# zaiisao/ConTEXTure-NeRF

Measured on AMD Instinct MI355X. Metric: UNet denoise steps/sec (CFG-batched SD2-depth UNet eval + PLMS update), higher is better.
Workload: dtype f16; 1 GPU; BASELINE configs[1]: 1 view @768^2 (latent 96^2), 50 PLMS steps (51 UNet evals), SD2-depth UNet fp16, CFG batch 2, guidance 10, random-init weights; mesh substitution napoleon.obj -> n/a for this stage (denoise loop only); latent=96, cfg_batch=2, ctx_len=77, views_per_rank=1, parallelism=view-shard x1

## Files before the change

### contexture-nerf_amd/_lib.py

```python
import ctypes as C
import os
import torch

_HERE = os.path.dirname(os.path.abspath(__file__))
LIB_PATH = os.path.join(_HERE, "libctxnerf.so")

_vp, _i32, _i64, _f32 = C.c_void_p, C.c_int32, C.c_int64, C.c_float

SIGNATURES = {
    "ctx_version": (_i32, []),
    "ctx_last_error": (C.c_char_p, []),
    "ctx_device_check": (_i32, []),
    "ctx_prepare_vertices": (_i32, [_vp, _vp, _vp, _vp, _i32, _i32, _i32, _vp, _vp, _vp, _vp, _vp]),
    "ctx_rasterize_ws_bytes": (_i64, [_i32, _i32, _i32, _i32]),
    "ctx_rasterize_fwd": (_i32, [_i32, _i32, _vp, _vp, _vp, _i32, _i32, _i32, _f32, _f32, _vp, _vp, _vp, _i64, _vp]),
    "ctx_rasterize_fused": (_i32, [_i32, _i32, _vp, _vp, _vp, _i32, _vp, _i32, _i32, _f32, _f32, _vp, _vp, _vp, _vp, _vp, _i64, _vp]),
    "ctx_normalize_depth_ws_bytes": (_i64, [_i32]),
    "ctx_normalize_depth": (_i32, [_vp, _i32, _i32, _vp, _vp, _vp, _vp]),
    "ctx_texture_mapping_fwd": (_i32, [_vp, _vp, _i32, _i32, _i32, _i32, _i32, _i32, _vp, _vp, _vp]),
    "ctx_texture_mapping_bwd": (_i32, [_vp, _vp, _i32, _i32, _i32, _i32, _vp, _vp, _vp]),
    "ctx_texmap_bwd_plan_bytes": (_i64, [_i32, _i32, _i32]),
    "ctx_texmap_bwd_plan": (_i32, [_vp, _vp, _i32, _i32, _i32, _vp, _vp]),
    "ctx_texture_mapping_bwd_binned_ws_bytes": (_i64, [_i32, _i32]),
    "ctx_texture_mapping_bwd_binned": (_i32, [_vp, _vp, _vp, _i32, _i32, _i32, _i32, _vp, _vp, _vp, _vp]),
# ... 59 lines not shown
    "ctx_hashtex_fwd": (_i32, [_vp, _vp, _i64, _i32, _vp, _i32, _i32, _i32, _vp, _vp, _vp]),
    "ctx_hashtex_bwd_ws_bytes": (_i64, [_i32, _i32, _i32]),
    "ctx_hashtex_bwd": (_i32, [_vp, _vp, _i64, _i32, _vp, _i32, _i32, _i32, _vp, _i32, _vp, _vp, _vp]),
    "ctx_texture_head_fwd": (_i32, [_vp, _vp, _i64, _i64, _i32, _vp, _vp]),
    "ctx_texture_head_bwd": (_i32, [_vp, _vp, _vp, _vp, _i64, _i64, _i32, _vp, _vp]),
    "ctx_adam_multi": (_i32, [_vp, _vp, _vp, _vp, _vp, _i32, _f32, _f32, _f32, _f32, _f32, _f32, _f32, _i32, _vp]),
    "ctx_table_adam": (_i32, [_vp, _vp, _vp, _i64, _vp, _i64, _i32, _f32, _f32, _f32, _f32, _f32, _f32, _f32, _i32, _vp]),
    "ctx_weighted_sum_packed": (_i32, [_vp, _vp, _vp, _i64, _i64, _i32, _vp, _vp]),
    "ctx_texel_rays": (_i32, [_vp, _vp, _vp, _vp, _vp, _vp, _i64, _i32, _i32, _i32, _i32, _f32, _vp, _vp, _vp, _vp]),
    "ctx_bake_resolve": (_i32, [_vp, _vp, _vp, _vp, _i64, _i32, _i32, _f32, _i32, _vp, _vp]),
    "ctx_unet_create": (_vp, [_vp]),
    "ctx_unet_destroy": (None, [_vp]),
    "ctx_unet_param_count": (_i32, [_vp]),
    "ctx_unet_param_name": (C.c_char_p, [_vp, _i32]),
    "ctx_unet_param_shape": (_i32, [_vp, _i32, _vp]),
    "ctx_unet_weight_bytes": (_i64, [_vp]),
    "ctx_unet_workspace_bytes": (_i64, [_vp, _i32, _i32, _i32, _i32]),
    "ctx_unet_bind": (_i32, [_vp, _vp, _vp, _i64]),
    "ctx_unet_derived_bytes": (_i64, [_vp]),
    "ctx_unet_bind_derived": (_i32, [_vp, _vp, _i64]),
    "ctx_unet_set_param": (_i32, [_vp, _i32, _vp, _vp]),
    "ctx_unet_forward": (_i32, [_vp, _vp, _vp, _vp, _i32, _i32, _i32, _i32, _vp, _vp]),
    "ctx_controlnet_create": (_vp, [_vp, _i32]),
    "ctx_controlnet_residual_bytes": (_i64, [_vp, _i32, _i32, _i32]),
    "ctx_controlnet_cond_cache_bytes": (_i64, [_vp, _i32, _i32, _i32]),
    "ctx_controlnet_forward": (_i32, [_vp, _vp, _vp, _vp, _vp, _vp, _i32, _i32, _i32, _i32, _i32, _vp, _vp]),
    "ctx_unet_set_residuals": (_i32, [_vp, _vp, C.c_float]),
    "ctx_unet_ref_bank_bytes": (_i64, [_vp, _i32, _i32, _i32]),
    "ctx_unet_workspace_bytes_ref": (_i64, [_vp, _i32, _i32, _i32, _i32, _i32, _i32]),
    "ctx_unet_forward_ref": (_i32, [_vp, _vp, _vp, _vp, _i32, _i32, _i32, _i32, _i32, _vp, _i32, _vp, _vp]),
    "ctx_unet_set_residual_fp32": (_i32, [_vp, _i32]),
    "ctx_unet_stats": (_i32, [_vp, _i32, _vp, _vp]),
    "ctx_unet_gn_epilogue_counts": (_i32, [_vp, _vp, _vp]),
    "ctx_unet_set_taps": (_i32, [_vp, _vp, _i64]),
    "ctx_unet_tap_count": (_i32, [_vp]),
    "ctx_unet_tap_info": (_i32, [_vp, _i32, _vp, _vp, _vp]),
    "ctx_vae_create": (_vp, [_vp]),
    "ctx_vae_destroy": (None, [_vp]),
    "ctx_vae_param_count": (_i32, [_vp]),
    "ctx_vae_param_name": (C.c_char_p, [_vp, _i32]),
    "ctx_vae_param_shape": (_i32, [_vp, _i32, _vp]),
    "ctx_vae_weight_bytes": (_i64, [_vp]),
    "ctx_vae_workspace_bytes": (_i64, [_vp, _i32, _i32, _i32]),
    "ctx_vae_bind": (_i32, [_vp, _vp, _vp, _i64]),
    "ctx_vae_derived_bytes": (_i64, [_vp]),
    "ctx_vae_bind_derived": (_i32, [_vp, _vp, _i64]),
    "ctx_vae_set_param": (_i32, [_vp, _i32, _vp, _vp]),
    "ctx_vae_decode": (_i32, [_vp, _vp, _i32, _i32, _i32, _vp, _vp]),
    "ctx_vae_decoder_param_count": (_i32, [_vp]),
    "ctx_vae_encode_workspace_bytes": (_i64, [_vp, _i32, _i32, _i32]),
    "ctx_vae_encode": (_i32, [_vp, _vp, _i32, _i32, _i32, _vp, _vp]),
    "ctx_vae_flops": (C.c_double, [_vp]),
    "ctx_vae_encode_train_workspace_bytes": (_i64, [_vp, _i32, _i32, _i32]),
    "ctx_vae_encode_train": (_i32, [_vp, _vp, _i32, _i32, _i32, _vp, _vp]),
    "ctx_vae_encode_bwd": (_i32, [_vp, _vp, _f32, _vp, _vp]),
    "ctx_gemm_f16": (_i32, [_vp, _vp, _vp, _vp, _i32, _i32, _i32, _vp, _vp]),
    "ctx_conv3x3_f16": (_i32, [_vp, _vp, _vp, _vp, _vp, _i32, _i32, _i32, _i32, _i32, _i32, _i32, _vp, _vp]),
    "ctx_conv3x3_seg_f16": (_i32, [_vp, _vp, _vp, _vp, _vp, _vp, _i32, _i32, _i32, _i32, _i32, _vp, _vp, _i32, _i32, _vp, _vp, _i32, _i32,
                                   _vp, _i32, _vp, _vp]),
    "ctx_conv3x3_gn_f16": (_i32, [_vp, _vp, _vp, _vp, _vp, _vp, _i32, _i32, _i32, _i32, _i32, _vp, _i32, _i32, _i32, _vp, _vp, _vp, _vp]),
    "ctx_gemm_last_kernel": (None, [_vp, _vp]),
    "ctx_conv3x3_geom_f16": (_i32, [_vp, _vp, _vp, _vp, _i32, _i32, _i32, _i32, _i32, _i32, _i32, _i32, _i32, _vp, _i32, _vp, _vp]),
    "ctx_pack_conv3_dgrad_f16": (_i32, [_vp, _i32, _i32, _i32, _vp, _vp]),
    "ctx_pack_conv3_phase_f16": (_i32, [_vp, _i32, _i32, _vp, _vp]),
    "ctx_conv3x3_phase_f16": (_i32, [_vp, _vp, _vp, _vp, _vp, _i32, _i32, _i32, _i32, _i32, _vp, _i32, _vp, _vp]),
    "ctx_pack_mat_dgrad_f16": (_i32, [_vp, _i32, _i32, _i32, _i32, _vp, _vp]),
    "ctx_groupnorm_bwd_ws_bytes": (_i64, [_i32, _i32]),
    "ctx_groupnorm_bwd_f16": (_i32, [_vp, _vp, _vp, _vp, _vp, _i32, _i32, _i32, _i32, _f32, _i32, _vp, _vp, _vp]),
    "ctx_softmax_rows_f16": (_i32, [_vp, _i32, _i32, _f32, _vp, _vp]),
    "ctx_softmax_bwd_rows_f16": (_i32, [_vp, _vp, _i32, _i32, _f32, _vp, _vp]),
    "ctx_quant_bwd_f16": (_i32, [_vp, _vp, _i32, _i32, _i64, _f32, _vp, _vp]),
    "ctx_conv_in_bwd_f16": (_i32, [_vp, _vp, _i32, _i32, _i32, _i32, _i32, _f32, _vp, _vp]),
    "ctx_conv_in_f16": (_i32, [_vp, _vp, _vp, _i32, _i32, _i32, _i32, _i32, _vp, _vp]),
    "ctx_conv_out_f16": (_i32, [_vp, _vp, _vp, _i32, _i32, _i32, _i32, _i32, _vp, _vp]),
    "ctx_gemv_f16": (_i32, [_vp, _vp, _vp, _i32, _i32, _i32, _i32, _i32, _vp, _vp]),
    "ctx_time_embed_f16": (_i32, [_vp, _i32, _i32, _vp, _vp]),
    "ctx_transpose_v_f16": (_i32, [_vp, _i32, _i32, _i32, _i32, _i32, _vp, _vp]),
    "ctx_concat_f16": (_i32, [_vp, _vp, _i64, _i32, _i32, _vp, _vp]),
    "ctx_concat_f32": (_i32, [_vp, _vp, _i64, _i32, _i32, _vp, _vp]),
    "ctx_f32_to_f16": (_i32, [_vp, _i64, _vp, _vp]),
    "ctx_f16_to_f32": (_i32, [_vp, _i64, _vp, _vp]),
    "ctx_conv_small_f16": (_i32, [_vp, _vp, _vp, _vp, _i32, _i32, _i32, _i32, _i32, _i32, _i32, _vp, _vp]),
    "ctx_add_scaled_f16": (_i32, [_vp, _vp, _f32, _i64, _vp]),
    "ctx_pointwise_f32": (_i32, [_vp, _vp, _vp, _i32, _i32, _i64, _i32, _vp, _vp]),
    "ctx_pack_fwd_f16": (_i32, [_vp, _i32, _i32, _i32, _vp, _vp]),
    "ctx_groupnorm_f16": (_i32, [_vp, _vp, _vp, _i32, _i32, _i32, _i32, _f32, _i32, _vp, _vp, _vp]),
    "ctx_groupnorm2_f16": (_i32, [_vp, _vp, _i32, _vp, _vp, _i32, _i32, _i32, _i32, _f32, _i32, _vp, _vp, _vp]),
    "ctx_groupnorm_apply_f16": (_i32, [_vp, _vp, _i32, _vp, _vp, _i32, _i32, _i32, _i32, _f32, _i32, _vp, _vp]),
    "ctx_groupnorm_slabs_f16": (_i32, [_vp, _i32, _vp, _vp, _vp, _i32, _vp, _vp, _i32, _i32, _i32, _i32, _f32, _i32, _vp, _vp]),
    "ctx_layernorm_f16": (_i32, [_vp, _vp, _vp, _i64, _i32, _f32, _vp, _vp]),
    "ctx_attention_ws_bytes": (_i64, [_i32, _i32, _i32]),
    "ctx_attention_f16": (_i32, [_vp, _vp, _vp, _i32, _i32, _i32, _i32, _i32, _i32, _f32, _vp, _i32, _vp, _vp]),
    "ctx_groupnorm_ws_bytes": (_i64, [_i32, _i32]),
    "ctx_geglu_f16": (_i32, [_vp, _i64, _i32, _vp, _vp]),
    "ctx_profile_begin": (_i32, []),
    "ctx_profile_end": (_i32, [_i32, _vp, _vp]),
    "ctx_bench_gemm": (C.c_float, [_vp, _vp, _vp, _vp, _i32, _i32, _i32, _vp, _i32, _i32, _i32, _i32, _i32, _i32, _vp, _i32, _i32, _vp]),
    "ctx_gemm_tune": (None, [_i32, _i32]),
    "ctx_attention_tune": (None, [_i32, _i32, _i32, _f32]),
    "ctx_probe_mfma": (_i32, [_i32, _vp, _vp, _vp, _vp]),
    "ctx_probe_stage": (C.c_float, [_i32, _i32, _i32, _i32, _i32, _vp, _vp, _vp]),
    "ctx_cfg_plms_step": (_i32, [_vp, _i64, _f32, _vp, _i32, _vp, _f32, _f32, _i32, _vp, _vp, _vp]),
}


class CtxError(RuntimeError):
    pass


# ... 48 lines not shown
```

### contexture-nerf_amd/csrc/attention.hip

```cpp
#include "gemm_common.h"
#include <math.h>

#define AT_KB 64
#define AT_KROW 72
#define AT_VROW 68


struct AttnArgs {
    const f16 *Q, *K, *V;
    f16 *O;
    int Sq, Skv, heads;
    int q_stride, kv_stride, o_stride;
    float scale_log2e;
    float lazy;
};



typedef short at_s16x4 __attribute__((__vector_size__(4 * sizeof(short))));
__device__ __forceinline__ f16x4 at_tr16(const f16 *p)
{
    at_s16x4 v = __builtin_amdgcn_ds_read_tr16_b64_v4i16((__attribute__((address_space(3))) at_s16x4 *)p);
    return __builtin_bit_cast(f16x4, v);
}
struct AtNoIssue { __device__ __forceinline__ void operator()(int) const {} };
template <bool MASK, int NISSUE = 0, class Issue = AtNoIssue>
__device__ __forceinline__ void attn_tile(const f16 *__restrict__ Ks, const f16 *__restrict__ Vs, int k0, int Skv, int r, int h,
                                          int swz, int vlane, int vfq, float c, const f16x8 (&qf)[4], f32x16 (&o)[2], f32x16 &ls,
                                          float &m_run, float lazy, Issue iss = Issue())
{
    f32x16 s[2];
#pragma unroll
    for (int kb = 0; kb < 2; ++kb) {
#pragma unroll
        for (int q = 0; q < 16; ++q) s[kb][q] = 0.f;
        const f16 *kr = Ks + (kb * 32 + r) * 64;
#pragma unroll
        for (int ks = 0; ks < 4; ++ks) {
            f16x8 kf = *(const f16x8 *)(kr + ((2 * ks + h) ^ swz) * 8);
            s[kb] = __builtin_amdgcn_mfma_f32_32x32x16_f16(kf, qf[ks], s[kb], 0, 0, 0);
            if (kb * 4 + ks < NISSUE) iss(kb * 4 + ks);
        }
    }
    if (MASK) {
#pragma unroll
        for (int kb = 0; kb < 2; ++kb)
#pragma unroll
// ... 29 lines not shown
#pragma unroll
        for (int d = 0; d < 2; ++d)
#pragma unroll
            for (int q = 0; q < 16; ++q) asm volatile("v_mul_f32 %0, %0, %1" : "+v"(o[d][q]) : "v"(alpha));
    }
    m_run = m_new;
    const f16x8 ones = {1, 1, 1, 1, 1, 1, 1, 1};
#pragma unroll
    for (int kb = 0; kb < 2; ++kb)
#pragma unroll
        for (int st = 0; st < 2; ++st) {
            f16x8 pf;
#pragma unroll
            for (int j = 0; j < 8; ++j) pf[j] = (f16)s[kb][8 * st + j];
            const f16 *vk = Vs + (32 * kb + 16 * st + 4 * h) * 64 + vlane;
#pragma unroll
            for (int d = 0; d < 2; ++d) {
                const int co = ((4 * d) ^ vfq) * 8;
                f16x4 v0 = at_tr16(vk + co), v1 = at_tr16(vk + 8 * 64 + co);
                f16x8 vf = __builtin_shufflevector(v0, v1, 0, 1, 2, 3, 4, 5, 6, 7);
                o[d] = __builtin_amdgcn_mfma_f32_32x32x16_f16(vf, pf, o[d], 0, 0, 0);
            }
            ls = __builtin_amdgcn_mfma_f32_32x32x16_f16(ones, pf, ls, 0, 0, 0);
        }
}

template <int AT_NS, int NW, bool SPREAD = true>
__global__ __launch_bounds__(64 * NW, NW == 8 ? 4 : 1) void k_attention_dma(AttnArgs a)
{
    __shared__ __attribute__((aligned(16))) f16 ring[AT_NS * 2 * 64 * 64];
    const int tid = threadIdx.x, lane = tid & 63, wave = __builtin_amdgcn_readfirstlane(tid >> 6);
    const int r = lane & 31, h = lane >> 5;
    const int b = blockIdx.z, hd = blockIdx.y;
    const int q0 = blockIdx.x * (32 * NW) + wave * 32;
    const int qrow = q0 + r;
    const bool qok = qrow < a.Sq;
    constexpr int PI = 8 / NW;
    constexpr int G = 2 * PI;

    f16x8 qf[4];
    const f16x8 zero8 = {0, 0, 0, 0, 0, 0, 0, 0};
    {
        const f16 *qp = a.Q + ((size_t)b * a.Sq + (qok ? qrow : 0)) * a.q_stride + hd * 64 + 8 * h;
#pragma unroll
        for (int ks = 0; ks < 4; ++ks) qf[ks] = qok ? *(const f16x8 *)(qp + ks * 16) : zero8;
    }
    f32x16 o[2];
#pragma unroll
    for (int d = 0; d < 2; ++d)
#pragma unroll
        for (int q = 0; q < 16; ++q) o[d][q] = 0.f;
    f32x16 ls;
#pragma unroll
    for (int q = 0; q < 16; ++q) ls[q] = 0.f;
    float m_run = -INFINITY;

    const int ntiles = (a.Skv + AT_KB - 1) / AT_KB;
    const int lr = lane >> 3, pc = lane & 7;
    const f16 *kp[PI], *vp[PI];
    int krow[PI];
#pragma unroll
    for (int i = 0; i < PI; ++i) {
        int row = 8 * (wave + NW * i) + lr;
        int lc = (pc ^ ((row >> 1) & 7)) * 8;
        krow[i] = row;
        kp[i] = a.K + ((size_t)b * a.Skv + row) * a.kv_stride + hd * 64 + lc;
// ... 53 lines not shown
            attn_tile<false>(Ks, Ks + 64 * 64, t * AT_KB, a.Skv, r, h, swz, vlane, vfq, c, qf, o, ls, m_run, a.lazy);
        }
        slot = slot + 1 == AT_NS ? 0 : slot + 1;
    }
    for (; t < nfull; ++t) {
        const int newer = issued - 1 - t;
        if (AT_NS >= 4 && newer >= 2) asm volatile("s_waitcnt vmcnt(%0)" ::"n"(2 * G) : "memory");
        else if (newer >= 1) asm volatile("s_waitcnt vmcnt(%0)" ::"n"(G) : "memory");
        else asm volatile("s_waitcnt vmcnt(0)" ::: "memory");
        __builtin_amdgcn_sched_barrier(0);
        ctx_barrier();
        if (issued < ntiles) issue(slot == 0 ? AT_NS - 1 : slot - 1);
        const f16 *Ks = ring + slot * (2 * 64 * 64);
        attn_tile<false>(Ks, Ks + 64 * 64, t * AT_KB, a.Skv, r, h, swz, vlane, vfq, c, qf, o, ls, m_run, a.lazy);
        slot = slot + 1 == AT_NS ? 0 : slot + 1;
    }
    if (nfull < ntiles) {
        asm volatile("s_waitcnt vmcnt(0)" ::: "memory");
        ctx_barrier();
        const f16 *Ks = ring + slot * (2 * 64 * 64);
        attn_tile<true>(Ks, Ks + 64 * 64, nfull * AT_KB, a.Skv, r, h, swz, vlane, vfq, c, qf, o, ls, m_run, a.lazy);
    }
    if (qok) {
        float inv = 1.0f / ls[0];
        f16 *op = a.O + ((size_t)b * a.Sq + qrow) * a.o_stride + hd * 64;
#pragma unroll
        for (int d = 0; d < 2; ++d)
#pragma unroll
            for (int g = 0; g < 4; ++g) {
                f16x4 v;
#pragma unroll
                for (int j = 0; j < 4; ++j) v[j] = (f16)(o[d][4 * g + j] * inv);
                *(f16x4 *)(op + d * 32 + 8 * g + 4 * h) = v;
            }
    }
}

template <int NS, int NW, bool SPREAD = true>
static void attn_launch(const AttnArgs &a, int B, bool report, hipStream_t s)
{
    constexpr auto kern = k_attention_dma<NS, NW, SPREAD>;
    if (report) {
        int nb = 0;
        hipFuncAttributes fa;
        (void)hipOccupancyMaxActiveBlocksPerMultiprocessor(&nb, kern, 64 * NW, 0);
        (void)hipFuncGetAttributes(&fa, (const void *)kern);
        fprintf(stderr, "[ctx] attention: %d blocks/CU by the occupancy API, %d VGPRs, %zu B static LDS\n", nb, fa.numRegs, fa.sharedSizeBytes);
    }
    ctx_launch<kern>(1, dim3(cdiv(a.Sq, 32 * NW), a.heads, B), dim3(64 * NW), 0, s, a);
}

struct AttnTune { int ns, nw8, spread; float lazy; };
static AttnTune g_attn_force = {-1, -1, -1, -1.f};
static const AttnTune &attn_tune_env()
{
    static const AttnTune env = [] {
        AttnTune t;
        t.ns = ctx_env_int("CTX_ATTN_NS", 3);
        t.nw8 = ctx_env_int("CTX_ATTN_NW8", -1);
        t.spread = ctx_env_int("CTX_ATTN_SPREAD", 1);
        const char *e = getenv("CTX_ATTN_LAZY");
        t.lazy = e ? (float)atof(e) : 8.0f;
        if (!(t.lazy >= 0.f && t.lazy <= 12.f)) t.lazy = 8.0f;
        return t;
    }();
    return env;
}

extern "C" void ctx_attention_tune(int32_t ns, int32_t nw8, int32_t spread, float lazy)
{
    g_attn_force.ns = ns; g_attn_force.nw8 = nw8; g_attn_force.spread = spread; g_attn_force.lazy = lazy;
}

int ctx_attention_core(const f16 *Q, const f16 *K, const f16 *V, int B, int Sq, int Skv, int heads, int q_stride,
                       int kv_stride, float scale, f16 *O, int o_stride, hipStream_t s)
{
    AttnArgs a;
    a.Q = Q; a.K = K; a.V = V; a.O = O; a.Sq = Sq; a.Skv = Skv; a.heads = heads;
    a.q_stride = q_stride; a.kv_stride = kv_stride; a.o_stride = o_stride;
    a.scale_log2e = scale * 1.4426950408889634f;
    const AttnTune &tu = attn_tune_env();
    const float lazy = g_attn_force.lazy >= 0.f ? g_attn_force.lazy : tu.lazy;
    a.lazy = lazy >= 0.f && lazy <= 12.f ? lazy : 8.0f;
    const int ns = g_attn_force.ns >= 0 ? g_attn_force.ns : tu.ns;
    const int nw8 = g_attn_force.nw8 >= 0 ? g_attn_force.nw8 : tu.nw8;
    const bool w8 = nw8 == 1 || (nw8 < 0 && Sq >= 1024 && Sq < 4096 && Skv >= 1024);
    const int spread = g_attn_force.spread >= 0 ? g_attn_force.spread : tu.spread;
    static int dbg = -1;
    bool report = false;
    if (dbg < 0) { dbg = ctx_env_int("CTX_ATTN_DEBUG", 0); report = dbg != 0; }
    if (w8) {
        if (ns == 2) attn_launch<2, 8>(a, B, report, s); else if (ns == 4) attn_launch<4, 8>(a, B, report, s);
        else if (spread) attn_launch<3, 8>(a, B, report, s); else attn_launch<3, 8, false>(a, B, report, s);
    } else {
        if (ns == 2) attn_launch<2, 4>(a, B, report, s); else if (ns == 4) attn_launch<4, 4>(a, B, report, s);
        else if (spread) attn_launch<3, 4>(a, B, report, s); else attn_launch<3, 4, false>(a, B, report, s);
    }
    hipError_t e = hipGetLastError();
    if (e != hipSuccess) {
        ctx_set_error("attention launch failed: %s", hipGetErrorString(e));
        return CTX_E_LAUNCH;
    }
    return CTX_OK;
}

extern "C" int64_t ctx_attention_ws_bytes(int32_t B, int32_t Skv, int32_t heads)
{
    (void)B; (void)Skv; (void)heads;
    return 256;
}
// ... 14 lines not shown
```

### contexture-nerf_amd/csrc/common.h

```cpp
#pragma once
#include <hip/hip_runtime.h>
#include <stdint.h>
#include <stdio.h>
#include <stdlib.h>
#include <stdarg.h>
#include "../../include/ctx_nerf.h"

void ctx_set_error(const char *fmt, ...);

#define CTX_REQUIRE(cond, ...)                 \
    do {                                       \
        if (!(cond)) {                         \
            ctx_set_error(__VA_ARGS__);        \
            return CTX_E_ARG;                  \
        }                                      \
    } while (0)

#define CTX_CHECK_LAUNCH(name)                                                     \
    do {                                                                           \
        hipError_t e__ = hipGetLastError();                                        \
        if (e__ != hipSuccess) {                                                   \
            ctx_set_error("%s: launch failed: %s", name, hipGetErrorString(e__)); \
            return CTX_E_LAUNCH;                                                   \
        }                                                                          \
// ... 1 lines not shown

static inline int64_t cdiv64(int64_t a, int64_t b) { return (a + b - 1) / b; }
static inline int cdiv(int a, int b) { return (a + b - 1) / b; }
static inline unsigned capped_blocks(int64_t items, int per_block, int64_t cap)
{
    const int64_t nb = cdiv64(items, per_block);
    return (unsigned)(nb < cap ? nb : cap);
}
static inline int ctx_env_int(const char *name, int dflt)
{
    const char *e = getenv(name);
    return e ? atoi(e) : dflt;
}
#define CTX_BOOL_GO(flag, B_, ...)                                 \
    do {                                                           \
        if (flag) { constexpr bool B_ = true; __VA_ARGS__; }       \
        else { constexpr bool B_ = false; __VA_ARGS__; }           \
    } while (0)

typedef _Float16 f16;
typedef f16 f16x8 __attribute__((ext_vector_type(8)));
typedef f16 f16x4 __attribute__((ext_vector_type(4)));
typedef f16 f16x2 __attribute__((ext_vector_type(2)));
typedef float f32x16 __attribute__((ext_vector_type(16)));
typedef float f32x4 __attribute__((ext_vector_type(4)));

__device__ __forceinline__ void ctx_barrier()
{
    asm volatile("" ::: "memory");
    __builtin_amdgcn_s_barrier();
    asm volatile("" ::: "memory");
}

__device__ __forceinline__ float wave_sum(float v)
{
#pragma unroll
    for (int o = 32; o > 0; o >>= 1) v += __shfl_xor(v, o, 64);
    return v;
}
__device__ __forceinline__ float sum8_dpp(float v)
{
    v += __builtin_bit_cast(float, __builtin_amdgcn_update_dpp(0, __builtin_bit_cast(int, v), 0xB1, 0xf, 0xf, true));
    v += __builtin_bit_cast(float, __builtin_amdgcn_update_dpp(0, __builtin_bit_cast(int, v), 0x4E, 0xf, 0xf, true));
    v += __builtin_bit_cast(float, __builtin_amdgcn_update_dpp(0, __builtin_bit_cast(int, v), 0x141, 0xf, 0xf, true));
    return v;
}
__device__ __forceinline__ float wave_sum_dpp(float v)
{
    v = sum8_dpp(v);
    v += __builtin_bit_cast(float, __builtin_amdgcn_update_dpp(0, __builtin_bit_cast(int, v), 0x140, 0xf, 0xf, true));
    const int vi = __builtin_bit_cast(int, v);
    float r0 = __builtin_bit_cast(float, __builtin_amdgcn_readlane(vi, 0)), r1 = __builtin_bit_cast(float, __builtin_amdgcn_readlane(vi, 16));
    float r2 = __builtin_bit_cast(float, __builtin_amdgcn_readlane(vi, 32)), r3 = __builtin_bit_cast(float, __builtin_amdgcn_readlane(vi, 48));
    return (r0 + r1) + (r2 + r3);
}
__device__ __forceinline__ float wave_max(float v)
{
#pragma unroll
    for (int o = 32; o > 0; o >>= 1) v = fmaxf(v, __shfl_xor(v, o, 64));
    return v;
}
__device__ __forceinline__ float wave_min(float v)
{
#pragma unroll
    for (int o = 32; o > 0; o >>= 1) v = fminf(v, __shfl_xor(v, o, 64));
    return v;
// ... 2 lines not shown
```

### contexture-nerf_amd/csrc/elementwise.hip

```cpp
#include "common.h"
#include "kernels.h"
#include <math.h>

__global__ __launch_bounds__(256) void k_geglu(const f16 *__restrict__ h, int64_t M, int C4, f16 *__restrict__ y)
{
    const int c8n = C4 / 8;
    const int64_t total = M * c8n;
    for (int64_t i = (int64_t)blockIdx.x * 256 + threadIdx.x; i < total; i += (int64_t)gridDim.x * 256) {
        int64_t m = i / c8n;
        int c8 = (int)(i % c8n);
        f16x8 a = *(const f16x8 *)(h + m * 2 * C4 + c8 * 8);
        f16x8 g = *(const f16x8 *)(h + m * 2 * C4 + C4 + c8 * 8);
        f16x8 o;
#pragma unroll
        for (int j = 0; j < 8; ++j) {
            float gf = (float)g[j];
            o[j] = (f16)((float)a[j] * (0.5f * gf * (1.0f + erff(gf * 0.70710678118654752f))));
        }
        *(f16x8 *)(y + m * C4 + c8 * 8) = o;
    }
}

extern "C" int32_t ctx_geglu_f16(const void *h, int64_t M, int32_t C4, void *y, ctx_stream_t stream)
{
// ... 57 lines not shown
                "transpose_v: need Sp %% 8 == 0, Sp >= S, ld %% 8 == 0, ld >= 64 heads (B=%d S=%d ld=%d heads=%d Sp=%d)", B, S, ld, heads, Sp);
    hipLaunchKernelGGL(k_transpose_v, dim3(cdiv(Sp, 64), heads, B), dim3(256), 0, s, v, S, ld, heads, Sp, vt);
    CTX_CHECK_LAUNCH("transpose_v");
    return CTX_OK;
}

__global__ __launch_bounds__(256) void k_f32_to_f16(const float *__restrict__ x, int64_t n, f16 *__restrict__ y)
{
    for (int64_t i = (int64_t)blockIdx.x * 256 + threadIdx.x; i < n; i += (int64_t)gridDim.x * 256) y[i] = (f16)x[i];
}
__global__ __launch_bounds__(256) void k_f16_to_f32(const f16 *__restrict__ x, int64_t n8, float *__restrict__ y)
{
    for (int64_t i = (int64_t)blockIdx.x * 256 + threadIdx.x; i < n8; i += (int64_t)gridDim.x * 256) {
        const f16x8 v = *(const f16x8 *)(x + i * 8);
        f32x4 a = {(float)v[0], (float)v[1], (float)v[2], (float)v[3]}, b = {(float)v[4], (float)v[5], (float)v[6], (float)v[7]};
        *(f32x4 *)(y + i * 8) = a; *(f32x4 *)(y + i * 8 + 4) = b;
    }
}
int ctx_f16_to_f32_core(const f16 *x, int64_t n, float *y, hipStream_t s)
{
    CTX_REQUIRE(x && y && n > 0 && n % 8 == 0, "f16_to_f32: n=%lld is not a positive multiple of 8", (long long)n);
    hipLaunchKernelGGL(k_f16_to_f32, dim3(capped_blocks(n / 8, 256, 4096)), dim3(256), 0, s, x, n / 8, y);
    CTX_CHECK_LAUNCH("f16_to_f32");
    return CTX_OK;
}
int ctx_f32_to_f16_core(const float *x, int64_t n, f16 *y, hipStream_t s)
{
    CTX_REQUIRE(x && y && n > 0, "f32_to_f16: null pointer or n=%lld < 1", (long long)n);
    hipLaunchKernelGGL(k_f32_to_f16, dim3(capped_blocks(n, 256, 2048)), dim3(256), 0, s, x, n, y);
    CTX_CHECK_LAUNCH("f32_to_f16");
    return CTX_OK;
}

__global__ void k_time_embed(const float *__restrict__ t, int B, int dim, f16 *__restrict__ out)
{
    int i = blockIdx.x * blockDim.x + threadIdx.x;
    int half = dim / 2;
    if (i >= half) return;
    float fr = expf(-9.210340371976184f * (float)i / (float)half);
    float a = t[0] * fr;
    float c = cosf(a), sn = sinf(a);
    for (int b = 0; b < B; ++b) {
        out[(size_t)b * dim + i] = (f16)c;
        out[(size_t)b * dim + half + i] = (f16)sn;
    }
}
int ctx_time_embed_core(const float *t, int B, int dim, f16 *out, hipStream_t s)
{
    CTX_REQUIRE(t && out && B > 0 && dim >= 2 && dim % 2 == 0, "time_embed: unsupported B=%d dim=%d", B, dim);
    hipLaunchKernelGGL(k_time_embed, dim3(cdiv(dim / 2, 64)), dim3(64), 0, s, t, B, dim, out);
    CTX_CHECK_LAUNCH("time_embed");
    return CTX_OK;
}

#define CI_SPLIT 16
template <int CP, int CX>
__global__ __launch_bounds__(256) void k_conv_in(const float *__restrict__ x, const f16 *__restrict__ w,
                                                 const f16 *__restrict__ bias, int B, int Cin, int H, int W, int Cout,
                                                 f16 *__restrict__ y)
{
    extern __shared__ __attribute__((aligned(16))) float s_w[];
    constexpr int WR = 9 * CP, WX = 9 * CX;
    const int o8n = Cout / 8;
    const int o8_per = (o8n + CI_SPLIT - 1) / CI_SPLIT;
    const int o8_0 = blockIdx.y * o8_per, o8_1 = min(o8n, o8_0 + o8_per);
    const int no = (o8_1 - o8_0) * 8;
    for (int i = threadIdx.x; i < no * WX; i += 256) {
        const int o = i / WX, r = i - o * WX, t = r / CX, c = r - t * CX;
        s_w[i] = (float)w[(size_t)(o8_0 * 8 + o) * WR + t * CP + c];
    }
    __syncthreads();
    const int64_t npix = (int64_t)B * H * W;
    const int64_t pix0 = (int64_t)blockIdx.x * 256;
    const int64_t pix = pix0 + threadIdx.x;
    const bool live = pix < npix;
    const int64_t pq = live ? pix : npix - 1;
    int b = (int)(pq / (H * W)), p = (int)(pq % (H * W));
    int oy = p / W, ox = p % W;
    float in[9][CX];
#pragma unroll
    for (int t = 0; t < 9; ++t) {
        int iy = oy + t / 3 - 1, ix = ox + t % 3 - 1;
        bool ok = iy >= 0 && iy < H && ix >= 0 && ix < W;
#pragma unroll
        for (int c = 0; c < CX; ++c)
            in[t][c] = (ok && c < Cin) ? (float)(f16)x[(((size_t)b * Cin + c) * H + iy) * W + ix] : 0.f;
    }
    f16 *patch = (f16 *)(s_w + no * WX);
    for (int g0 = o8_0; g0 < o8_1; g0 += 8) {
        const int ng = min(8, o8_1 - g0);
        for (int gi = 0; gi < ng; ++gi) {
            const int o8 = g0 + gi;
            f16x8 o;
#pragma unroll
            for (int j = 0; j < 8; ++j) {
                const float *wr = s_w + ((o8 - o8_0) * 8 + j) * WX;
                float acc = (float)bias[o8 * 8 + j];
#pragma unroll
                for (int t = 0; t < 9; ++t)
#pragma unroll
                    for (int c = 0; c < CX; ++c) acc += in[t][c] * wr[t * CX + c];
                o[j] = (f16)acc;
            }
            *(f16x8 *)(patch + threadIdx.x * 72 + gi * 8) = o;
        }
        __syncthreads();
        for (int ch = threadIdx.x; ch < 256 * ng; ch += 256) {
            const int px = ch / ng, gi = ch - px * ng;
            if (pix0 + px < npix) *(f16x8 *)(y + (pix0 + px) * Cout + (g0 + gi) * 8) = *(const f16x8 *)(patch + px * 72 + gi * 8);
        }
        __syncthreads();
    }
}
int ctx_conv_in_core(const float *x, const f16 *w, const f16 *bias, int B, int Cin, int H, int W, int Cout, f16 *y, hipStream_t s)
{
    CTX_REQUIRE(x && w && bias && y && Cout > 0 && Cout % 8 == 0, "conv_in: unsupported Cout=%d", Cout);
    CTX_REQUIRE(Cin >= 1 && Cin <= 16, "conv_in: need 1 <= Cin <= 16 (Cin=%d)", Cin);
    CTX_REQUIRE(B > 0 && H > 0 && W > 0 && (int64_t)H * W < (1ll << 31), "conv_in: unsupported grid B=%d H=%d W=%d", B, H, W);
    int64_t npix = (int64_t)B * H * W;
    int o8_per = (Cout / 8 + CI_SPLIT - 1) / CI_SPLIT;
    const int cx = Cin <= 3 ? 3 : Cin <= 5 ? Cin : Cin <= 8 ? 8 : Cin == 9 ? 9 : 16;
    CTX_REQUIRE((size_t)o8_per * 8 * 9 * cx * sizeof(float) + 256 * 72 * sizeof(f16) <= 64 * 1024,
                "conv_in: the weight slice of Cout=%d at Cin=%d does not fit the LDS", Cout, Cin);
    const dim3 grid((unsigned)cdiv64(npix, 256), CI_SPLIT);
#define CI_GO(CP_, CX_) hipLaunchKernelGGL((k_conv_in<CP_, CX_>), grid, dim3(256), (size_t)o8_per * 8 * 9 * CX_ * sizeof(float) + 256 * 72 * sizeof(f16), s, x, w, bias, B, Cin, H, W, Cout, y)
    if (Cin <= 3) CI_GO(8, 3);
    else if (Cin == 4) CI_GO(8, 4);
    else if (Cin == 5) CI_GO(8, 5);
    else if (Cin <= 8) CI_GO(8, 8);
    else if (Cin == 9) CI_GO(16, 9);
    else CI_GO(16, 16);
#undef CI_GO
    CTX_CHECK_LAUNCH("conv_in");
    return CTX_OK;
}

template <int NU, bool WF32>
__global__ __launch_bounds__(256) void k_conv_out(const f16 *__restrict__ x, const f16 *__restrict__ w,
                                                  const f16 *__restrict__ bias, int B, int H, int W, int C, int Cout,
                                                  float *__restrict__ out)
{
    extern __shared__ __attribute__((aligned(16))) char s_cw_raw[];
    f16 *s_cw = (f16 *)s_cw_raw;
    float *s_cf = (float *)s_cw_raw;
    const int nwt = Cout * 9 * C;
    if (WF32) {
        for (int i = threadIdx.x * 8; i < nwt; i += 256 * 8) {
            const f16x8 v = *(const f16x8 *)(w + i);
#pragma unroll
            for (int j = 0; j < 8; ++j) s_cf[i + j] = (float)v[j];
        }
    } else {
        for (int i = threadIdx.x * 8; i < nwt; i += 256 * 8) *(f16x8 *)(s_cw + i) = *(const f16x8 *)(w + i);
    }
    __syncthreads();
    const int lane = threadIdx.x & 63;
    const int c8n = C / 8, nitems = 9 * c8n;
    const int64_t npix = (int64_t)B * H * W;
// ... 112 lines not shown
                                     const float *coef4, float sample_coeff, float eps_coeff, int32_t mode,
                                     float *cur_sample_ws, float *x, ctx_stream_t stream)
{
    CTX_REQUIRE(eps_pair && ets && coef4 && x && n > 0 && head >= 0 && head < 4, "cfg_plms_step: bad args");
    CTX_REQUIRE(mode == 0 || cur_sample_ws, "cfg_plms_step: mode %d needs cur_sample_ws", mode);
    hipLaunchKernelGGL(k_cfg_plms, dim3(capped_blocks(n, 256, 2048)), dim3(256), 0, (hipStream_t)stream, eps_pair, n, guidance, ets, head,
                       coef4[0], coef4[1], coef4[2], coef4[3], sample_coeff, eps_coeff, mode, cur_sample_ws, x);
    CTX_CHECK_LAUNCH("cfg_plms_step");
    return CTX_OK;
}

extern "C" int32_t ctx_concat_f16(const void *a, const void *b, int64_t M, int32_t Ca, int32_t Cb, void *y, ctx_stream_t stream)
{
    return ctx_concat_core((const f16 *)a, (const f16 *)b, M, Ca, Cb, (f16 *)y, (hipStream_t)stream);
}
extern "C" int32_t ctx_concat_f32(const float *a, const float *b, int64_t M, int32_t Ca, int32_t Cb, float *y, ctx_stream_t stream)
{
    CTX_REQUIRE(Ca > 0 && Cb > 0 && Ca <= (1 << 29) && Cb <= (1 << 29), "concat_f32: unsupported Ca=%d Cb=%d", Ca, Cb);
    return ctx_concat32_core(a, b, M, Ca, Cb, y, (hipStream_t)stream);
}
extern "C" int32_t ctx_transpose_v_f16(const void *v, int32_t B, int32_t S, int32_t ld, int32_t heads, int32_t Sp, void *vt, ctx_stream_t stream)
{
    CTX_REQUIRE(B <= 65535 && heads <= 65535, "transpose_v: B=%d / heads=%d exceed the grid", B, heads);
    return ctx_transpose_v_core((const f16 *)v, B, S, ld, heads, Sp, (f16 *)vt, (hipStream_t)stream);
}
extern "C" int32_t ctx_f32_to_f16(const float *x, int64_t n, void *y, ctx_stream_t stream)
{
    return ctx_f32_to_f16_core(x, n, (f16 *)y, (hipStream_t)stream);
}
extern "C" int32_t ctx_f16_to_f32(const void *x, int64_t n, float *y, ctx_stream_t stream)
{
    return ctx_f16_to_f32_core((const f16 *)x, n, y, (hipStream_t)stream);
}
extern "C" int32_t ctx_time_embed_f16(const float *t, int32_t B, int32_t dim, void *out, ctx_stream_t stream)
{
    return ctx_time_embed_core(t, B, dim, (f16 *)out, (hipStream_t)stream);
}
extern "C" int32_t ctx_conv_in_f16(const float *x, const void *w_pack, const void *bias, int32_t B, int32_t Cin, int32_t H, int32_t W, int32_t Cout,
                                   void *y, ctx_stream_t stream)
{
    return ctx_conv_in_core(x, (const f16 *)w_pack, (const f16 *)bias, B, Cin, H, W, Cout, (f16 *)y, (hipStream_t)stream);
}
extern "C" int32_t ctx_conv_out_f16(const void *x, const void *w, const void *bias, int32_t B, int32_t H, int32_t W, int32_t C, int32_t Cout,
                                    float *out, ctx_stream_t stream)
{
    return ctx_conv_out_core((const f16 *)x, (const f16 *)w, (const f16 *)bias, B, H, W, C, Cout, out, (hipStream_t)stream);
}
```

### contexture-nerf_amd/csrc/engine.h

```cpp
#pragma once
#include "common.h"
#include "kernels.h"
#include <string>
#include <vector>

enum PackKind { PK_COPY = 0, PK_CONV3 = 1, PK_CONVIN = 2, PK_GEGLU_W = 3, PK_GEGLU_B = 4 };

struct Param {
    std::string name;
    int ndim;
    int64_t shape[4];
    int kind;
    size_t dst;
    int a, b;
    int kind2 = 0; size_t dst2 = 0; int pad2 = 0, ld2 = 0, col2 = 0;
    int kind3 = 0; size_t dst3 = 0;
};

struct Engine {
    const char *tag = "";
    std::vector<Param> params;
    size_t wtop = 0;
    size_t dtop = 0;
    f16 *D = nullptr;
    f16 *W = nullptr;
    char *ws = nullptr;
    size_t ws_cap = 0;
    size_t top = 0, peak = 0;
    bool dry = false;
    hipStream_t s = nullptr;
    int rc = 0;
    int64_t launches[3] = {0, 0, 0};
    double flops[3] = {0, 0, 0};

    struct GnTag { const void *x = nullptr; int B = 0, HW = 0, C = 0, groups = 0, NS = 0; } gn_tag;
    int64_t gn_from_producer = 0, gn_from_slabs = 0;

    size_t walloc(size_t n) { size_t o = wtop; wtop += (n + 127) / 128 * 128; return o; }
    size_t add(const std::string &name, std::vector<int64_t> shp, int kind, size_t dst, int a = 0, int b = 0)
    {
        Param p; p.name = name; p.ndim = (int)shp.size(); p.kind = kind; p.dst = dst; p.a = a; p.b = b;
        for (int i = 0; i < 4; ++i) p.shape[i] = i < p.ndim ? shp[i] : 1;
        params.push_back(p);
        return dst;
    }
    void derive_phase()
    {
        Param &p = params.back();
        if (!ctx_conv3_phase_ok(p.b, p.a, 1, 1, 0, 0)) return;
        p.kind3 = 1; p.dst3 = dtop; dtop += ((size_t)16 * p.a * p.b + 127) / 128 * 128;
    }
    const f16 *phase_pack(const f16 *Wt) const
    {
        if (!D || !W) return nullptr;
        for (const Param &p : params)
            if (p.kind3 == 1 && W + p.dst == Wt) return D + p.dst3;
        return nullptr;
    }
    size_t vec(const std::string &name, int n) { return add(name, {n}, PK_COPY, walloc(n)); }
    size_t lin(const std::string &name, int out, int in) { return add(name, {out, in}, PK_COPY, walloc((size_t)out * in)); }

    void *alloc(size_t bytes)
    {
        size_t o = (top + 255) / 256 * 256;
        top = o + bytes;
        if (top > peak) peak = top;
        if (!dry && top > ws_cap) { rc = CTX_E_STATE; ctx_set_error("%s: workspace too small (%zu > %zu)", tag, top, ws_cap); return ws; }
        return dry ? nullptr : (void *)(ws + o);
    }
    f16 *allocH(size_t n) { return (f16 *)alloc(n * 2); }

    void begin()
    {
        top = 0; peak = 0; rc = 0; gn_tag = GnTag(); gn_from_producer = 0; gn_from_slabs = 0;
        for (int k = 0; k < 3; ++k) { launches[k] = 0; flops[k] = 0; }
    }
    void note(int klass, double fl, int n = 1) { launches[klass] += n; flops[klass] += fl; }
    bool live() const { return !dry && rc == 0; }
    void copy(void *dst, const void *src, size_t bytes) { if (live()) (void)hipMemcpyAsync(dst, src, bytes, hipMemcpyDeviceToDevice, s); }
    void copy2d(void *dst, size_t dpitch, const void *src, size_t spitch, size_t width, size_t rows)
    { if (live()) (void)hipMemcpy2DAsync(dst, dpitch, src, spitch, width, rows, hipMemcpyDeviceToDevice, s); }
};

#define ENGINE_RUN(e, expr) do { if ((e)->live()) { int r__ = (expr); if (r__ != 0) (e)->rc = r__; } } while (0)
#define ENGINE_LAUNCH(e, kernel, grid, block, lds, ...) do { if ((e)->live()) hipLaunchKernelGGL(kernel, grid, block, lds, (e)->s, __VA_ARGS__); } while (0)

struct GnReq { float *part = nullptr; int groups = 0, HW = 0; };
void engine_linear(Engine &e, const f16 *X, const f16 *Wt, const f16 *bias, const void *res, int M, int N, int K, void *out, int ldc = 0,
                   int epi = 0, bool res32 = false, bool out32 = false, const GnReq *gn = nullptr);
struct ConvGeom { int stride = 1, ups = 0, poff = 0, zins = 0; };
struct ConvSegs { int n = 0; const f16 *x[2] = {nullptr, nullptr}; const f16 *w[2] = {nullptr, nullptr}; int C[2] = {0, 0}, ldw[2] = {0, 0}; const f16 *bias2 = nullptr; };
void engine_conv3(Engine &e, const f16 *x, const f16 *Wt, const f16 *bias, const void *res, int B, int H, int W, int Cin, int Cout, void *out,
                  ConvGeom g = ConvGeom(), const f16 *rowbias = nullptr, int ldrb = 0, bool res32 = false, bool out32 = false,
                  const ConvSegs *segs = nullptr, const GnReq *gn = nullptr, GnSlabs *slabs = nullptr);
int engine_conv3_split(int B, int H, int W, int Cin, int Cout);

template <class F> int engine_dry_run(Engine *e, F run)
{
    const bool was = e->dry;
    e->dry = true; const int rc = run(); e->dry = was;
    return rc;
}
inline int64_t engine_workspace_need(const Engine *e) { return (int64_t)e->peak + 4096; }
int engine_finish(Engine *e, const char *who);

int32_t engine_param_count(const Engine *e);
const char *engine_param_name(const Engine *e, int32_t i);
// ... 8 lines not shown
```

### contexture-nerf_amd/csrc/engine.hip

```cpp
#include "engine.h"

int32_t engine_param_count(const Engine *e) { return e ? (int32_t)e->params.size() : 0; }
const char *engine_param_name(const Engine *e, int32_t i)
{
    return (e && i >= 0 && i < (int)e->params.size()) ? e->params[i].name.c_str() : "";
}
int32_t engine_param_shape(const Engine *e, int32_t i, int64_t shape4[4])
{
    if (!e || i < 0 || i >= (int)e->params.size()) return 0;
    for (int k = 0; k < 4; ++k) shape4[k] = e->params[i].shape[k];
    return e->params[i].ndim;
}
int64_t engine_weight_bytes(const Engine *e) { return e ? (int64_t)e->wtop * 2 + 256 : 0; }

int32_t engine_bind(Engine *e, void *weights, void *workspace, int64_t workspace_bytes, const char *who)
{
    CTX_REQUIRE(e && weights && workspace && workspace_bytes > 0, "%s: bad args", who);
    CTX_REQUIRE(((uintptr_t)weights & 255) == 0 && ((uintptr_t)workspace & 255) == 0, "%s: blobs must be 256-byte aligned", who);
    e->W = (f16 *)weights; e->ws = (char *)workspace; e->ws_cap = (size_t)workspace_bytes;
    return CTX_OK;
}

int64_t engine_derived_bytes(const Engine *e) { return e && e->dtop ? (int64_t)e->dtop * 2 + 256 : 0; }
int32_t engine_bind_derived(Engine *e, void *derived, int64_t bytes, const char *who)
{
    CTX_REQUIRE(e, "%s: bad args", who);
    if (!derived) { e->D = nullptr; return CTX_OK; }
    CTX_REQUIRE(e->dtop > 0, "%s: this engine derives nothing", who);
    CTX_REQUIRE(bytes >= engine_derived_bytes(e) && ((uintptr_t)derived & 255) == 0, "%s: the derived blob needs %lld bytes, 256-byte aligned", who,
                (long long)engine_derived_bytes(e));
    e->D = (f16 *)derived;
    return CTX_OK;
}

static void engine_gemm(Engine &e, GemmArgs &a, bool conv, const ConvSegs *segs = nullptr, const GnReq *gn = nullptr, GnSlabs *slabs = nullptr,
                        const f16 *phase = nullptr)
{
    e.note(0, 2.0 * a.M * a.N * a.K);
    size_t mark = e.top;
    if (phase) ctx_conv3_phase(a, phase);
    ctx_gemm_plan(a, conv);
    if (segs && segs->n) {
        int kseg = 0;
        a.nseg = segs->n; a.bias2 = segs->bias2;
        for (int i = 0; i < segs->n; ++i) {
            a.segX[i] = segs->x[i]; a.segW[i] = segs->w[i]; a.segC[i] = segs->C[i]; a.segLdw[i] = segs->ldw[i];
            kseg += segs->C[i];
        }
        a.K += kseg;
        e.note(0, 2.0 * a.M * a.N * kseg);
    }
    if (a.zins) a.use8 = 0;
    if (a.splitk > 1) a.part = (float *)e.alloc((size_t)a.splitk * a.M * a.N * 4);
    if (gn && gn->part && gn->groups > 0 && a.N % gn->groups == 0) { a.gn_part = gn->part; a.gn_cg = a.N / gn->groups; a.gn_hw = gn->HW; }
    if (slabs) {
        a.keep_slabs = 1;
        *slabs = GnSlabs{a.part, a.splitk, (size_t)a.M * a.N, a.bias, a.bias2, a.rowbias, a.ldrb};
    }
    ENGINE_RUN(&e, ctx_gemm_dispatch(a, conv, e.s));
    if (e.live() && a.gn_part) e.gn_tag = Engine::GnTag{a.out, a.M / a.gn_hw, a.gn_hw, a.N, gn->groups, a.gn_ns};
    if (!slabs) e.top = mark;
}

int engine_conv3_split(int B, int H, int W, int Cin, int Cout)
{
    GemmArgs a = {};
    a.Ho = H; a.Wo = W; a.M = B * H * W; a.N = Cout; a.K = 9 * Cin; a.H = H; a.W = W; a.Cin = Cin; a.stride = 1;
    ctx_gemm_plan(a, true);
    return (a.splitk > 1 && a.splitk <= a.K / 64) ? a.splitk : 1;
}

void engine_linear(Engine &e, const f16 *X, const f16 *Wt, const f16 *bias, const void *res, int M, int N, int K, void *out, int ldc, int epi,
                   bool res32, bool out32, const GnReq *gn)
{
    GemmArgs a = {};
    a.X = X; a.Wt = Wt; a.bias = bias; a.residual = (const f16 *)res; a.out = (f16 *)out;
    a.M = M; a.N = N; a.K = K; a.ldc = ldc ? ldc : epi == 1 ? N / 2 : N; a.ldr = N; a.rows_per_batch = 1; a.ldrb = N; a.epi = epi;
    a.res32 = res32; a.out32 = out32;
    engine_gemm(e, a, false, nullptr, gn);
}

void engine_conv3(Engine &e, const f16 *x, const f16 *Wt, const f16 *bias, const void *res, int B, int H, int W, int Cin, int Cout, void *out,
                  ConvGeom g, const f16 *rowbias, int ldrb, bool res32, bool out32, const ConvSegs *segs, const GnReq *gn, GnSlabs *slabs)
{
    GemmArgs a = {};
    ctx_conv3_problem(a, B, H, W, Cin, Cout, g.stride, g.ups, g.poff, g.zins);
    a.X = x; a.Wt = Wt; a.bias = bias; a.rowbias = rowbias; a.residual = (const f16 *)res; a.out = (f16 *)out;
    a.ldrb = ldrb;
    a.res32 = res32; a.out32 = out32;
    const f16 *phase = nullptr;
    if (g.ups && ctx_conv3_phase_ok(Cin, Cout, g.stride, g.ups, g.poff, g.zins) && !res && !rowbias && !segs && !gn && !slabs && !res32 && !out32 &&
        !ctx_conv3_phase_loses(a.M, Cout, Cin))
// ... 157 lines not shown
```

### contexture-nerf_amd/csrc/gemm.hip

```cpp
#include "gemm_common.h"

template <int MI, int NI, bool PH = false>
__device__ __forceinline__ void gemm_epilogue(const GemmArgs &a, f32x16 (&acc)[MI][NI], int mw, int nw, int r, int h, const ConvPhase &ph)
{
#pragma unroll
    for (int mi = 0; mi < MI; ++mi) {
        int m = mw + mi * 32 + r;
        if (m >= ph.M) continue;
        const int mo = PH ? conv_phase_row(a, ph, m) : m;
        int bidx = a.rowbias ? m / a.rows_per_batch : 0;
        if (a.epi == 1) {
            if constexpr (NI == 2) {
                int fbase = nw / 2;
#pragma unroll
                for (int g = 0; g < 4; ++g) {
                    int nn = nw + 8 * g + 4 * h;
                    if (nn >= a.N) continue;
                    f16x4 o;
#pragma unroll
                    for (int j = 0; j < 4; ++j) {
                        float xv = acc[mi][0][4 * g + j], gv = acc[mi][1][4 * g + j];
                        if (a.bias) { xv += (float)a.bias[nn + j]; gv += (float)a.bias[nn + 32 + j]; }
                        o[j] = geglu(xv, gv);
                    }
// ... 33 lines not shown
            for (int g = 0; g < 4; ++g)
                *(f32x4 *)(stage + r * RS + ni * 32 + 8 * g + 4 * h) = acc4(acc[mi][ni], g);
#pragma unroll
        for (int p = 0; p < 32 / RPP; ++p) {
            const int row = RPP * p + prow;
            const int m = mw + mi * 32 + row;
            f32x4 v0 = *(const f32x4 *)(stage + row * RS + c8), v1 = *(const f32x4 *)(stage + row * RS + c8 + 4);
            if (m < ph.M && n < a.N) {
                float v[8] = {v0[0], v0[1], v0[2], v0[3], v1[0], v1[1], v1[2], v1[3]};
                add8(v, bs);
                if (a.bias2) add8(v, *(const f16x8 *)(a.bias2 + n));
                store8<true>(a, v, PH ? conv_phase_row(a, ph, m) : m, n);
            }
        }
    }
}

template <int WM, int WN, int MI, int NI, bool CONV, int NS, int PKT, bool PH = false>
__global__ __launch_bounds__(64 * WM * WN) void k_gemm_pipe(GemmArgs a)
{
    constexpr int BM = 32 * MI * WM, BN = 32 * NI * WN, NW = WM * WN;
    constexpr int RP = 512 / PKT;
    constexpr int LPR = PKT / 8;
    constexpr int XI = BM / (RP * NW), WI = BN / (RP * NW);
    static_assert(XI >= 1 && WI >= 1, "tile too small for the wave count");
    constexpr int G = XI + WI;
    constexpr int STAGE = (BM + BN) * PKT;
    extern __shared__ __attribute__((aligned(16))) f16 smem[];

    const int tid = threadIdx.x, lane = tid & 63, wave = __builtin_amdgcn_readfirstlane(tid >> 6);
    const int r = lane & 31, h = lane >> 5;
    const int wm = wave / WN, wn = wave % WN;
    const GemmTile t = gemm_tile(a, blockIdx.x, PKT, BM, BN);
    static_assert(!PH || CONV, "the phase form is a convolution");
    const ConvPhase ph = PH ? conv_phase_tile(a, t.tile_m, BM) : ConvPhase{0, 0, 0, t.m0, a.M};
    const int slice = t.slice, tile_m = t.tile_m, tile_n = t.tile_n, m0 = ph.m0, n0 = t.n0, kbeg = t.kbeg, nk = t.nk;
    const int ldw = CONV ? (PH ? 4 : 9) * a.Cin : a.K;
    const f16 *const Wt = PH ? a.Wt + (size_t)ph.ph * a.N * ldw : a.Wt;
    const int lr = lane / LPR, pc = lane % LPR;

    const f16 *xp[XI], *wp[WI];
    int xst[XI], wst[WI];
    int xoff[XI], xoy[XI], xox[XI];
    bool xok[XI];
#pragma unroll
    for (int i = 0; i < XI; ++i) {
        int row = RP * (wave + NW * i) + lr;
        int m = m0 + row;
        const int lc = (pc ^ (PKT == 32 ? ((row >> 2) & 3) : ((row >> 1) & 7))) * 8;
        xok[i] = m < ph.M;
        if (CONV) {
            conv_pixel(a, m, lc, xoy[i], xox[i], xoff[i]);
            xp[i] = ctx_zero_page; xst[i] = 0;
        } else {
            xoff[i] = 0; xoy[i] = 0; xox[i] = 0;
            xp[i] = xok[i] ? a.X + (size_t)m * a.K + kbeg * PKT + lc : ctx_zero_page;
            xst[i] = xok[i] ? PKT : 0;
        }
    }
#pragma unroll
    for (int i = 0; i < WI; ++i) {
        int row = RP * (wave + NW * i) + lr;
        bool ok = (n0 + row) < a.N;
        wp[i] = ok ? Wt + (size_t)(n0 + row) * ldw + kbeg * PKT + ((pc ^ (PKT == 32 ? ((row >> 2) & 3) : ((row >> 1) & 7))) * 8) : ctx_zero_page;
        wst[i] = ok ? PKT : 0;
    }
// ... 703 lines not shown
```

### contexture-nerf_amd/csrc/gemm144.hip

```cpp
#include "gemm_common.h"
#include <type_traits>

#define G144_BM 144
#define G144_BN 160
#define G144_STAGE ((G144_BM + G144_BN) * 64)

template <int WM, int WN, bool CONV, int NS, int VAR, int UPS = 0, int BMB = 9, bool GNP = false>
__global__ __launch_bounds__(64 * WM * WN) void k_gemm144(GemmArgs a)
{
    constexpr int NW = WM * WN, MI = BMB / WM, NI = 10 / WN;
    constexpr int BM = 16 * BMB, NPX = BM / 8;
    constexpr int NP = NPX + 20;
    constexpr int STAGE = (BM + G144_BN) * 64;
    static_assert(NPX % 2 == 0, "the K segments' chunk swizzle takes a weight piece's parity from its slot");
    static_assert(BMB % WM == 0 && (BMB == 9 || (BMB == 18 && VAR == 0)), "288-row tiles: lockstep schedule only");
    constexpr int SL = (NP + NW - 1) / NW;
    static_assert(9 % WM == 0 && 10 % WN == 0, "wave grid must divide 9 x 10 blocks");
    extern __shared__ __attribute__((aligned(16))) f16 smem[];
    const int tid = threadIdx.x, lane = tid & 63, wave = __builtin_amdgcn_readfirstlane(tid >> 6);
    const int wm = wave / WN, wn = wave % WN;
    const int r16 = lane & 15, kg = lane >> 4;

    const GemmTile tl = gemm_tile(a, blockIdx.x, 64, BM, G144_BN);
    constexpr bool PH = UPS == 2;
    static_assert(!PH || (CONV && !GNP), "the phase form is a convolution without GroupNorm partials");
    const ConvPhase ph = PH ? conv_phase_tile(a, tl.tile_m, BM) : ConvPhase{0, 0, 0, tl.m0, a.M};
    const int slice = tl.slice, m0 = ph.m0, n0 = tl.n0, kbeg = tl.kbeg, nk = tl.nk;
    const int ldw = CONV ? (PH ? 4 : 9) * a.Cin : a.K;
    const f16 *const Wt = PH ? a.Wt + (size_t)ph.ph * a.N * ldw : a.Wt;

    const int prow = lane >> 3, pc = lane & 7;
    constexpr bool FAST = CONV && UPS != 1;
    constexpr int NTAP = PH ? 4 : 9;
    const f16 *pp[SL], *xcen[SL];
    int pst[SL], xoff[SL], xoy[SL], xox[SL], xlc[SL], xval[SL];
    bool xok[SL];
    const f16 *const zp = ctx_zero_page;
    const bool full = wave + NW * (SL - 1) < NP;
#pragma unroll
    for (int i = 0; i < SL; ++i) {
        const int p = wave + NW * i;
        const bool isx = p < NPX, live = p < NP;
        const int s = isx ? 8 * p + prow : 8 * (p - NPX) + prow;
        xlc[i] = (pc ^ ((s >> 1) & 7)) * 8;
        xoff[i] = 0; xoy[i] = 0; xox[i] = 0;
        if (isx) {
            const int m = m0 + s;
            xok[i] = m < ph.M;
            if (CONV) {
                conv_pixel(a, xok[i] ? m : 0, xlc[i], xoy[i], xox[i], xoff[i]);
                pp[i] = zp; pst[i] = 0;
                if (FAST) {
                    xcen[i] = a.X + (size_t)xoff[i] + (size_t)(xoy[i] * a.W + xox[i]) * a.Cin;
                    int v = 0;
#pragma unroll
                    for (int t = 0; t < NTAP; ++t) {
                        const int iy = xoy[i] + (PH ? conv_phase_dy(ph, t) : t / 3 - 1 + a.poff), ix = xox[i] + (PH ? conv_phase_dx(ph, t) : t % 3 - 1 + a.poff);
// ... 458 lines not shown
```

### contexture-nerf_amd/csrc/kernels.h

```cpp
#pragma once
#include "common.h"

struct GemmArgs {
    const f16 *X;
    const f16 *Wt;
    const f16 *bias;
    const f16 *rowbias;
    const f16 *residual;
    f16 *out;
    int M, N, K;
    int ldc, ldr;
    int rows_per_batch;
    int ldrb;
    int epi;
    int H, W, Cin, Ho, Wo, stride, ups;
    int poff;
    int res32, out32;
    int zins;
    int phase;
    int ntm, ntn;
    int splitk;
    float *part;
    int pk;
    int krot;
    int tile, use8;
    int stage_epi;
    int mfast;
    int nseg;
    const f16 *segX[2];
    const f16 *segW[2];
    int segC[2], segLdw[2];
    const f16 *bias2;
    float *gn_part;
    int gn_cg, gn_hw;
    int gn_ns;
    int keep_slabs;
};
#define CTX_GN_MAX_SLOTS 128
#define CTX_GEMM_MAX_SEG 2

static inline void ctx_conv3_problem(GemmArgs &a, int B, int H, int W, int Cin, int Cout, int stride, int ups, int poff, int zins)
{
    a.Ho = ((H << ups) - 1) / stride + 1; a.Wo = ((W << ups) - 1) / stride + 1;
    a.M = B * a.Ho * a.Wo; a.N = Cout; a.K = 9 * Cin; a.ldc = Cout; a.ldr = Cout; a.rows_per_batch = a.Ho * a.Wo;
    a.H = H; a.W = W; a.Cin = Cin; a.stride = stride; a.ups = ups; a.poff = poff; a.zins = zins;
}

static inline void ctx_conv3_phase(GemmArgs &a, const f16 *wp)
{
    a.phase = 1; a.Wt = wp; a.K = 4 * a.Cin;
}
static inline int ctx_conv3_phase_ok(int Cin, int Cout, int stride, int ups, int poff, int zins)
{
    return ups == 1 && stride == 1 && poff == 0 && !zins && Cin % 64 == 0 && Cout % 8 == 0;
}
static inline int ctx_conv3_phase_loses(int M, int Cout, int Cin) { return 0; }

int ctx_gemm_dispatch(GemmArgs &a, bool conv, hipStream_t s);
int ctx_gemm8_try(GemmArgs &a, bool conv, bool force, hipStream_t s);
int ctx_conv_halo_try(GemmArgs &a, int ni, hipStream_t s);
int ctx_gemm144_try(GemmArgs &a, bool conv, int form, hipStream_t s);
int ctx_gemm_pick_split(int M, int N, int K, int epi);
void ctx_gemm_plan(GemmArgs &a, bool conv);
int ctx_gemv_core(const f16 *x, const f16 *w, const f16 *bias, int Bm, int N, int K, int silu_in, int silu_out, f16 *out, hipStream_t s);
int ctx_concat_core(const f16 *a, const f16 *b, int64_t M, int Ca, int Cb, f16 *y, hipStream_t s);
int ctx_transpose_v_core(const f16 *v, int B, int S, int ld, int heads, int Sp, f16 *vt, hipStream_t s);
int ctx_f32_to_f16_core(const float *x, int64_t n, f16 *y, hipStream_t s);
int ctx_time_embed_core(const float *t, int B, int dim, f16 *out, hipStream_t s);
int ctx_conv_in_core(const float *x, const f16 *w, const f16 *bias, int B, int Cin, int H, int W, int Cout, f16 *y, hipStream_t s);
int ctx_conv_out_core(const f16 *x, const f16 *w, const f16 *bias, int B, int H, int W, int C, int Cout, float *out, hipStream_t s);
int ctx_attention_core(const f16 *Q, const f16 *K, const f16 *V, int B, int Sq, int Skv, int heads, int q_stride,
                       int kv_stride, float scale, f16 *O, int o_stride, hipStream_t s);
extern "C" int64_t ctx_groupnorm_ws_bytes(int32_t B, int32_t groups);
int ctx_groupnorm_any(const void *x, int x32, const void *gamma, const void *beta, int B, int HW, int C, int groups, float eps, int silu,
                      void *y, void *stats_ws, hipStream_t stream, const void *x2 = nullptr, int Ca = 0);
int ctx_groupnorm_two_pass(int HW, int C, int groups);
int ctx_groupnorm_apply(const void *x, const float *part, int NS, const void *gamma, const void *beta, int B, int HW, int C, int groups, float eps,
                        int silu, void *y, hipStream_t stream);
struct GnSlabs { const float *part; int S; size_t MN; const f16 *bias, *bias2, *rowbias; int ldrb; };
int ctx_groupnorm_slabs(const GnSlabs &sl, const void *gamma, const void *beta, int B, int HW, int C, int groups, float eps, int silu, void *y,
                        hipStream_t stream);
int ctx_layernorm_any(const void *x, int x32, const void *gamma, const void *beta, int64_t rows, int C, float eps, void *y, hipStream_t stream);
int ctx_concat32_core(const float *a, const float *b, int64_t M, int Ca, int Cb, float *y, hipStream_t s);
int ctx_f16_to_f32_core(const f16 *x, int64_t n, float *y, hipStream_t s);
int ctx_conv_small_core(const float *x32, const f16 *x16, const f16 *w, const f16 *bias, int B, int H, int W, int Cin, int Cout, int stride, int silu,
                        f16 *y, hipStream_t s);
int ctx_add_scaled_core(f16 *dst, const f16 *src, float scale, int64_t n, hipStream_t s);
int ctx_pointwise_core(const void *x, const f16 *w, const f16 *b, int B, int C, int64_t HW, bool nhwc16, float *y, hipStream_t s);

bool ctx_prof_on(void);
void ctx_prof_events(int klass, hipEvent_t *a, hipEvent_t *b);
```

### contexture-nerf_amd/csrc/norm.hip

```cpp
#include "common.h"
#include "kernels.h"
#include <math.h>


struct Wide8 {
    float v[8];
    __device__ __forceinline__ float get(int j) const { return v[j]; }
};
template <bool X32> struct Raw8;
template <> struct Raw8<false> {
    f16x8 a;
    __device__ __forceinline__ float get(int j) const { return (float)a[j]; }
    __device__ __forceinline__ Wide8 widen() const
    {
        Wide8 r;
#pragma unroll
        for (int j = 0; j < 8; ++j) r.v[j] = (float)a[j];
        return r;
    }
};
template <> struct Raw8<true> {
    f32x4 a, b;
    __device__ __forceinline__ float get(int j) const { return j < 4 ? a[j] : b[j - 4]; }
    __device__ __forceinline__ Wide8 widen() const
    {
        Wide8 r;
#pragma unroll
        for (int j = 0; j < 4; ++j) { r.v[j] = a[j]; r.v[4 + j] = b[j]; }
        return r;
    }
};
template <bool X32>
__device__ __forceinline__ Raw8<X32> ldraw(const void *base, size_t elem)
{
    Raw8<X32> r;
    if constexpr (X32) { r.a = *(const f32x4 *)((const float *)base + elem); r.b = *(const f32x4 *)((const float *)base + elem + 4); }
    else r.a = *(const f16x8 *)((const f16 *)base + elem);
    return r;
}

struct GnSrc { const void *p; int cs, col; };
__device__ __forceinline__ GnSrc gn_src(const void *x, const void *x2, int Ca, int C, int ch)
{
    if (!x2) return {x, C, ch};
    return ch < Ca ? GnSrc{x, Ca, ch} : GnSrc{x2, C - Ca, ch - Ca};
}

#define GN_MAX_GROUPS 64
#define GN_MAX_SPLITS CTX_GN_MAX_SLOTS
#define GN_MAX_C 4096
#define GN_U 4
#define GN_AU 6
#define GN_FOLD 8

template <bool X32>
__global__ __launch_bounds__(1024) void k_gn_stats(const void *__restrict__ x, const void *__restrict__ x2, int Ca, int HW, int C, int G,
                                                   int NS, int PL, float *__restrict__ part)
{
    extern __shared__ float s_part[];
    const int c8n = C / 8;
    const int b = blockIdx.y, sp = blockIdx.x;
    const int c8 = threadIdx.x % c8n, pl = threadIdx.x / c8n;
    const int per = (HW + NS - 1) / NS;
    const int p0 = sp * per, p1 = min(HW, p0 + per);
    float s[8], q[8];
#pragma unroll
    for (int j = 0; j < 8; ++j) { s[j] = 0.f; q[j] = 0.f; }
    const GnSrc src = gn_src(x, x2, Ca, C, c8 * 8);
    const size_t base = ((size_t)b * HW) * src.cs + src.col;
    for (int p = p0 + pl; p < p1; p += PL * GN_U) {
        Wide8 v[GN_U];
#pragma unroll
        for (int u = 0; u < GN_U; ++u) v[u] = ldraw<X32>(src.p, base + (size_t)min(p + u * PL, p1 - 1) * src.cs).widen();
#pragma unroll
        for (int u = 0; u < GN_U; ++u) {
            const bool live = p + u * PL < p1;
#pragma unroll
            for (int j = 0; j < 8; ++j) { float f = live ? v[u].get(j) : 0.f; s[j] += f; q[j] += f * f; }
        }
    }
#pragma unroll
    for (int j = 0; j < 8; ++j) {
        s_part[((size_t)pl * C + c8 * 8 + j) * 2 + 0] = s[j];
        s_part[((size_t)pl * C + c8 * 8 + j) * 2 + 1] = q[j];
    }
    __syncthreads();
    float *s_ch = s_part + (size_t)PL * C * 2;
    const int na = max(1, (int)blockDim.x / C);
    for (int it = threadIdx.x; it < C * na; it += blockDim.x) {
        const int a = it / C, c = it - a * C;
        float ss = 0.f, qq = 0.f;
// ... 28 lines not shown
}

__device__ __forceinline__ float2 gn_mean_rstd(float sum, float sumsq, float n, float eps)
{
    const float mean = sum / n;
    return make_float2(mean, rsqrtf(fmaxf(sumsq / n - mean * mean, 0.f) + eps));
}
template <class MR>
__device__ __forceinline__ void gn_scale_shift(MR mr, f16x8 ga, f16x8 be, float (&sa)[8], float (&sh)[8])
{
#pragma unroll
    for (int j = 0; j < 8; ++j) {
        const float2 m = mr(j);
        sa[j] = m.y * (float)ga[j];
        sh[j] = (float)be[j] - m.x * sa[j];
    }
}
template <class V8>
__device__ __forceinline__ void gn_store(const V8 &v, const float (&sa)[8], const float (&sh)[8], int silu, f16 *dst)
{
    f16x8 o;
#pragma unroll
    for (int j = 0; j < 8; ++j) {
        float t = v.get(j) * sa[j] + sh[j];
        if (silu) t = t * __builtin_amdgcn_rcpf(1.0f + __builtin_amdgcn_exp2f(-1.4426950408889634f * t));
        o[j] = (f16)t;
    }
    *(f16x8 *)dst = o;
}

template <bool X32>
__global__ __launch_bounds__(512) void k_gn_apply(const void *__restrict__ x, const void *__restrict__ x2, int Ca, const float *__restrict__ part,
                                                  const f16 *__restrict__ gamma, const f16 *__restrict__ beta, int HW, int C,
                                                  int G, int NS, int PL, float eps, int silu, f16 *__restrict__ y)
{
    constexpr int AU = GN_AU;
    __shared__ float s_mean[GN_MAX_GROUPS], s_rstd[GN_MAX_GROUPS];
    const int b = blockIdx.y;
    const int c8n = C / 8;
    const int c8 = threadIdx.x % c8n, pl = threadIdx.x / c8n;
    const int p0 = blockIdx.x * (PL * AU);
    const GnSrc src = gn_src(x, x2, Ca, C, c8 * 8);
    const size_t xb = (size_t)b * HW * src.cs + src.col;
    f16 *yb = y + (size_t)b * HW * C + c8 * 8;
    Raw8<X32> v[AU];
#pragma unroll
    for (int u = 0; u < AU; ++u) v[u] = ldraw<X32>(src.p, xb + (size_t)min(p0 + u * PL + pl, HW - 1) * src.cs);
    const f16x8 ga = *(const f16x8 *)(gamma + c8 * 8), be = *(const f16x8 *)(beta + c8 * 8);
    if (threadIdx.x < 256) {
        const int lpg = min(256 / G, 64);
        const int gi = threadIdx.x / lpg, l = threadIdx.x % lpg;
        const int g = min(gi, G - 1);
        float s = 0.f, q = 0.f;
        for (int k0 = 0; k0 < NS; k0 += GN_FOLD * lpg) {
            float2 pv[GN_FOLD];
#pragma unroll
            for (int k = 0; k < GN_FOLD; ++k)
                pv[k] = *(const float2 *)(part + (((size_t)b * NS + min(k0 + k * lpg + l, NS - 1)) * G + g) * 2);
#pragma unroll
            for (int k = 0; k < GN_FOLD; ++k)
                if (k0 + k * lpg + l < NS) { s += pv[k].x; q += pv[k].y; }
        }
        for (int o = lpg >> 1; o > 0; o >>= 1) { s += __shfl_xor(s, o, 64); q += __shfl_xor(q, o, 64); }
        if (l == 0 && gi < G) {
            const float2 m = gn_mean_rstd(s, q, (float)HW * (float)(C / G), eps);
            s_mean[g] = m.x;
            s_rstd[g] = m.y;
        }
    }
    __syncthreads();
    const int cg = C / G;
    float sa[8], sh[8];
    gn_scale_shift([&](int j) { const int gg = (c8 * 8 + j) / cg; return make_float2(s_mean[gg], s_rstd[gg]); }, ga, be, sa, sh);
#pragma unroll
    for (int u = 0; u < AU; ++u) {
        const int p = p0 + u * PL + pl;
        if (p < HW) gn_store(v[u], sa, sh, silu, yb + (size_t)p * C);
    }
}

#define GN_FT 512
#define GN_FU 12
__device__ __forceinline__ Wide8 gn_slab_chunk(const GnSlabs &sl, size_t m, int b, int C, int ch)
{
    const float *row = sl.part + m * C + ch;
    f32x4 lo = *(const f32x4 *)row, hi = *(const f32x4 *)(row + 4);
    for (int s = 1; s < sl.S; ++s) { lo += *(const f32x4 *)(row + s * sl.MN); hi += *(const f32x4 *)(row + s * sl.MN + 4); }
    Wide8 r;
#pragma unroll
    for (int j = 0; j < 4; ++j) { r.v[j] = lo[j]; r.v[4 + j] = hi[j]; }
    if (sl.bias) { const f16x8 t = *(const f16x8 *)(sl.bias + ch);
#pragma unroll
        for (int j = 0; j < 8; ++j) r.v[j] += (float)t[j]; }
    if (sl.bias2) { const f16x8 t = *(const f16x8 *)(sl.bias2 + ch);
#pragma unroll
        for (int j = 0; j < 8; ++j) r.v[j] += (float)t[j]; }
    if (sl.rowbias) { const f16x8 t = *(const f16x8 *)(sl.rowbias + (size_t)b * sl.ldrb + ch);
#pragma unroll
        for (int j = 0; j < 8; ++j) r.v[j] += (float)t[j]; }
#pragma unroll
    for (int j = 0; j < 8; ++j) r.v[j] = (float)(f16)r.v[j];
    return r;
}
template <bool X32, bool SLAB = false>
__global__ __launch_bounds__(GN_FT) void k_gn_fused(const void *__restrict__ x, const void *__restrict__ x2, int Ca, const f16 *__restrict__ gamma,
                                                    const f16 *__restrict__ beta, int HW, int C, int G, int PLF, float eps, int silu,
                                                    f16 *__restrict__ y, GnSlabs sl)
{
    __shared__ float s_red[2][GN_FT / 64];
    const int g = blockIdx.x, b = blockIdx.y;
    const int cg = C / G, cpg = cg / 8;
    const int c = threadIdx.x % cpg, pl = threadIdx.x / cpg;
    const bool act = pl < PLF;
    const GnSrc src = gn_src(x, x2, Ca, C, g * cg + c * 8);
    const size_t xb = (size_t)b * HW * src.cs + src.col;
    f16 *yb = y + (size_t)b * HW * C + g * cg + c * 8;
    const f16x8 ga = *(const f16x8 *)(gamma + g * cg + c * 8), be = *(const f16x8 *)(beta + g * cg + c * 8);
    Wide8 v[GN_FU];
#pragma unroll
    for (int u = 0; u < GN_FU; ++u) {
        if constexpr (SLAB) v[u] = gn_slab_chunk(sl, (size_t)b * HW + min(pl + PLF * u, HW - 1), b, C, g * cg + c * 8);
        else v[u] = ldraw<X32>(src.p, xb + (size_t)min(pl + PLF * u, HW - 1) * src.cs).widen();
    }
    float s = 0.f, q = 0.f;
#pragma unroll
    for (int u = 0; u < GN_FU; ++u)
        if (act && pl + PLF * u < HW) {
#pragma unroll
            for (int j = 0; j < 8; ++j) { float f = v[u].get(j); s += f; q += f * f; }
        }
    s = wave_sum_dpp(s); q = wave_sum_dpp(q);
    const int wave = threadIdx.x >> 6;
    if ((threadIdx.x & 63) == 0) { s_red[0][wave] = s; s_red[1][wave] = q; }
    __syncthreads();
    float ss = 0.f, qq = 0.f;
    const int nw = ((int)blockDim.x + 63) >> 6;
    for (int w = 0; w < nw; ++w) { ss += s_red[0][w]; qq += s_red[1][w]; }
    const float2 m = gn_mean_rstd(ss, qq, (float)HW * (float)cg, eps);
    float sa[8], sh[8];
    gn_scale_shift([&](int) { return m; }, ga, be, sa, sh);
#pragma unroll
    for (int u = 0; u < GN_FU; ++u) {
        const int p = pl + PLF * u;
        if (act && p < HW) gn_store(v[u], sa, sh, silu, yb + (size_t)p * C);
    }
}

static bool gn_shape_ok(int B, int HW, int C, int groups)
{
    return B > 0 && HW > 0 && groups > 0 && C % 8 == 0 && C % groups == 0 && groups <= GN_MAX_GROUPS && C <= GN_MAX_C && 256 % groups == 0 &&
           (256 / groups & (256 / groups - 1)) == 0;
}
static int gn_one_kernel_lanes(int HW, int C, int groups)
{
    static const int fuse = ctx_env_int("CTX_GN_FUSED", 1);
    const int cg = C / groups, cpg = cg / 8;
    const int plf = cg % 8 == 0 ? GN_FT / cpg : 0;
    return (fuse && plf > 0 && cpg <= GN_FT && (HW + plf - 1) / plf <= GN_FU) ? plf : 0;
}
static void gn_launch_apply(const void *x, int x32, const void *x2, int Ca, const float *part, int NS, const void *gamma, const void *beta, int B, int HW,
                            int C, int groups, float eps, int silu, void *y, hipStream_t stream)
{
    const int c8n = C / 8;
    const int apl = (256 + c8n - 1) / c8n;
    const int athreads = c8n * apl;
    const int nb = (HW + apl * GN_AU - 1) / (apl * GN_AU);
    CTX_BOOL_GO(x32, X, hipLaunchKernelGGL(k_gn_apply<X>, dim3(nb, B), dim3(athreads), 0, stream, x, x2, Ca, part, (const f16 *)gamma, (const f16 *)beta, HW, C,
                                           groups, NS, apl, eps, silu, (f16 *)y));
}

extern "C" int64_t ctx_groupnorm_ws_bytes(int32_t B, int32_t groups)
{
    return ((int64_t)B * GN_MAX_SPLITS * groups * 2 + (int64_t)B * 2 * GN_MAX_C) * 4;
}

extern "C" int32_t ctx_groupnorm_f16(const void *x, const void *gamma, const void *beta, int32_t B, int32_t HW, int32_t C,
                                     int32_t groups, float eps, int32_t silu, void *y, void *stats_ws, ctx_stream_t stream)
{
    return ctx_groupnorm_any(x, 0, gamma, beta, B, HW, C, groups, eps, silu, y, stats_ws, (hipStream_t)stream);
}

extern "C" int32_t ctx_groupnorm2_f16(const void *xa, const void *xb, int32_t Ca, const void *gamma, const void *beta, int32_t B, int32_t HW,
                                      int32_t C, int32_t groups, float eps, int32_t silu, void *y, void *stats_ws, ctx_stream_t stream)
{
    CTX_REQUIRE(xb, "groupnorm2: null pointer");
    return ctx_groupnorm_any(xa, 0, gamma, beta, B, HW, C, groups, eps, silu, y, stats_ws, (hipStream_t)stream, xb, Ca);
}

extern "C" int32_t ctx_groupnorm_apply_f16(const void *x, const void *part, int32_t slots, const void *gamma, const void *beta, int32_t B, int32_t HW,
                                           int32_t C, int32_t groups, float eps, int32_t silu, void *y, ctx_stream_t stream)
{
    return ctx_groupnorm_apply(x, (const float *)part, slots, gamma, beta, B, HW, C, groups, eps, silu, y, (hipStream_t)stream);
}

extern "C" int32_t ctx_groupnorm_slabs_f16(const void *part, int32_t splitk, const void *bias, const void *bias2, const void *rowbias, int32_t ldrb,
                                           const void *gamma, const void *beta, int32_t B, int32_t HW, int32_t C, int32_t groups, float eps,
                                           int32_t silu, void *y, ctx_stream_t stream)
{
    const GnSlabs sl = {(const float *)part, splitk, (size_t)B * HW * C, (const f16 *)bias, (const f16 *)bias2, (const f16 *)rowbias, ldrb};
    return ctx_groupnorm_slabs(sl, gamma, beta, B, HW, C, groups, eps, silu, y, (hipStream_t)stream);
}

int ctx_groupnorm_any(const void *x, int x32, const void *gamma, const void *beta, int B, int HW, int C, int groups, float eps, int silu,
                      void *y, void *stats_ws, hipStream_t stream, const void *x2, int Ca)
{
    CTX_REQUIRE(x && gamma && beta && y && stats_ws, "groupnorm: null pointer");
    CTX_REQUIRE(!x2 || (Ca > 0 && Ca < C && Ca % 8 == 0), "groupnorm: two sources need 0 < Ca < C in whole 8-channel columns (Ca=%d C=%d)", Ca, C);
    CTX_REQUIRE(gn_shape_ok(B, HW, C, groups), "groupnorm: unsupported B=%d HW=%d C=%d groups=%d", B, HW, C, groups);
    if (const int plf = gn_one_kernel_lanes(HW, C, groups); plf && (!x2 || Ca % (C / groups) == 0)) {
        const int thr = (C / groups / 8 * plf + 63) / 64 * 64;
        CTX_BOOL_GO(x32, X, hipLaunchKernelGGL(k_gn_fused<X>, dim3(groups, B), dim3(thr), 0, stream, x, x2, Ca, (const f16 *)gamma, (const f16 *)beta, HW, C,
                                               groups, plf, eps, silu, (f16 *)y, GnSlabs{}));
        CTX_CHECK_LAUNCH("groupnorm");
        return CTX_OK;
    }
    int c8n = C / 8;
    int PL = 1024 / c8n;
    if (PL < 1) PL = 1;
    if (PL > HW) PL = HW;
    int threads = c8n * PL;
    int NS = min(GN_MAX_SPLITS, max(1, HW / PL));
    {
        static const int ns_env = ctx_env_int("CTX_GN_NS", 0);
        const int64_t sample_bytes = (int64_t)HW * C * (x32 ? 4 : 2);
        const int by_size = (int)min((int64_t)GN_MAX_SPLITS, sample_bytes / (384 * 1024));
        const int want = ns_env > 0 ? ns_env : max(16, max(by_size, (64 + B - 1) / B));
        NS = min(NS, want);
    }
    float *part = (float *)stats_ws;
    const int na = threads / C > 1 ? threads / C : 1;
    size_t lds = (size_t)(PL + na) * C * 2 * sizeof(float);
    static bool attr = false;
    if (!attr) {
        (void)hipFuncSetAttribute((const void *)k_gn_stats<false>, hipFuncAttributeMaxDynamicSharedMemorySize, 80 * 1024);
        (void)hipFuncSetAttribute((const void *)k_gn_stats<true>, hipFuncAttributeMaxDynamicSharedMemorySize, 80 * 1024);
        attr = true;
    }
    CTX_BOOL_GO(x32, X, hipLaunchKernelGGL(k_gn_stats<X>, dim3(NS, B), dim3(threads), lds, stream, x, x2, Ca, HW, C, groups, NS, PL, part));
    gn_launch_apply(x, x32, x2, Ca, part, NS, gamma, beta, B, HW, C, groups, eps, silu, y, stream);
    CTX_CHECK_LAUNCH("groupnorm");
    return CTX_OK;
}

int ctx_groupnorm_two_pass(int HW, int C, int groups) { return gn_one_kernel_lanes(HW, C, groups) == 0; }

int ctx_groupnorm_apply(const void *x, const float *part, int NS, const void *gamma, const void *beta, int B, int HW, int C, int groups, float eps,
                        int silu, void *y, hipStream_t stream)
{
    CTX_REQUIRE(x && part && gamma && beta && y, "groupnorm apply: null pointer");
    CTX_REQUIRE(gn_shape_ok(B, HW, C, groups) && NS >= 1 && NS <= GN_MAX_SPLITS, "groupnorm apply: unsupported B=%d HW=%d C=%d groups=%d NS=%d", B, HW, C, groups, NS);
    gn_launch_apply(x, 0, nullptr, 0, part, NS, gamma, beta, B, HW, C, groups, eps, silu, y, stream);
    CTX_CHECK_LAUNCH("groupnorm apply");
    return CTX_OK;
}

int ctx_groupnorm_slabs(const GnSlabs &sl, const void *gamma, const void *beta, int B, int HW, int C, int groups, float eps, int silu, void *y,
                        hipStream_t stream)
{
    CTX_REQUIRE(sl.part && sl.S >= 1 && gamma && beta && y, "groupnorm slabs: bad arguments");
    const int plf = gn_shape_ok(B, HW, C, groups) ? gn_one_kernel_lanes(HW, C, groups) : 0;
    CTX_REQUIRE(plf > 0 && (!sl.rowbias || sl.ldrb % 8 == 0), "groupnorm slabs: B=%d HW=%d C=%d groups=%d does not take the one-kernel form", B, HW, C, groups);
    const int thr = (C / groups / 8 * plf + 63) / 64 * 64;
    hipLaunchKernelGGL((k_gn_fused<false, true>), dim3(groups, B), dim3(thr), 0, stream, (const void *)nullptr, (const void *)nullptr, 0, (const f16 *)gamma,
                       (const f16 *)beta, HW, C, groups, plf, eps, silu, (f16 *)y, sl);
    CTX_CHECK_LAUNCH("groupnorm slabs");
    return CTX_OK;
}

#define GNB_MAX_SPLITS 128

__device__ __forceinline__ float gnb_du(float dy, float u, float gamma, int silu)
{
    if (silu) { const float sg = 1.0f / (1.0f + __expf(-u)); dy *= sg * (1.0f + u * (1.0f - sg)); }
    return dy * gamma;
}
template <int MODE>
__global__ __launch_bounds__(256) void k_gnb_reduce(const f16 *__restrict__ x, const f16 *__restrict__ dy, const f16 *__restrict__ gamma,
                                                    const f16 *__restrict__ beta, const float *__restrict__ mr, int HW, int C, int G, int NS,
                                                    int silu, float *__restrict__ part)
{
    extern __shared__ float sm[];
    const int c8n = C / 8, PL = 256 / c8n;
    const int b = blockIdx.y, sp = blockIdx.x;
    const int c8 = threadIdx.x % c8n, pl = threadIdx.x / c8n;
    const int per = (HW + NS - 1) / NS, p0 = sp * per, p1 = min(HW, p0 + per), cg = C / G;
    float s[8], q[8], a[8], b0[8], ga[8], mu[8], rs[8];
#pragma unroll
    for (int j = 0; j < 8; ++j) {
        s[j] = 0.f; q[j] = 0.f;
        if (MODE == 1) {
            const int c = c8 * 8 + j, g = c / cg;
            mu[j] = mr[((size_t)b * G + g) * 2]; rs[j] = mr[((size_t)b * G + g) * 2 + 1];
            ga[j] = (float)gamma[c]; a[j] = rs[j] * ga[j]; b0[j] = (float)beta[c] - mu[j] * a[j];
        }
    }
    if (pl < PL)
        for (int p = p0 + pl; p < p1; p += PL) {
// ... 70 lines not shown
extern "C" int64_t ctx_groupnorm_bwd_ws_bytes(int32_t B, int32_t groups)
{
    return ((int64_t)B * GNB_MAX_SPLITS * groups * 2 + (int64_t)B * groups * 4) * 4;
}

extern "C" int32_t ctx_groupnorm_bwd_f16(const void *xv, const void *dyv, const void *gammav, const void *betav, const void *addv, int32_t B,
                                         int32_t HW, int32_t C, int32_t groups, float eps, int32_t silu, void *dxv, void *ws, ctx_stream_t stream)
{
    const f16 *x = (const f16 *)xv, *dy = (const f16 *)dyv, *gamma = (const f16 *)gammav, *beta = (const f16 *)betav, *add = (const f16 *)addv;
    f16 *dx = (f16 *)dxv;
    hipStream_t s = (hipStream_t)stream;
    CTX_REQUIRE(x && dy && gamma && beta && dx && ws, "groupnorm backward: null pointer");
    CTX_REQUIRE(B > 0 && HW > 0 && C >= 8 && groups > 0, "groupnorm backward: B=%d HW=%d C=%d groups=%d", B, HW, C, groups);
    const int G = groups, c8n = C / 8;
    CTX_REQUIRE(C % 8 == 0 && 256 % c8n == 0 && C % G == 0, "groupnorm backward: C=%d groups=%d is outside the kernel's envelope", C, G);
    const int PL = 256 / c8n;
    int NS = HW / (PL * 4); if (NS < 1) NS = 1; if (NS > GNB_MAX_SPLITS) NS = GNB_MAX_SPLITS;
    float *part = (float *)ws, *mr = part + (size_t)B * GNB_MAX_SPLITS * G * 2, *cc = mr + (size_t)B * G * 2;
    const size_t lds = ((size_t)PL * C * 2 + (size_t)C * 2) * sizeof(float);
    const float n = (float)HW * (float)(C / G);
    hipLaunchKernelGGL(k_gnb_reduce<0>, dim3(NS, B), dim3(256), lds, s, x, (const f16 *)nullptr, gamma, beta, (const float *)nullptr, HW, C, G, NS, silu, part);
    hipLaunchKernelGGL(k_gnb_finalize<0>, dim3(B), dim3(64), 0, s, part, G, NS, n, eps, mr);
    hipLaunchKernelGGL(k_gnb_reduce<1>, dim3(NS, B), dim3(256), lds, s, x, dy, gamma, beta, mr, HW, C, G, NS, silu, part);
    hipLaunchKernelGGL(k_gnb_finalize<1>, dim3(B), dim3(64), 0, s, part, G, NS, n, 0.f, cc);
    hipLaunchKernelGGL(k_gnb_apply, dim3(capped_blocks((int64_t)HW * c8n, 256, 2048), B), dim3(256), 0, s, x, dy, gamma, beta, mr, cc, add, HW, C, G, silu, dx);
    CTX_CHECK_LAUNCH("groupnorm backward");
    return CTX_OK;
}

__device__ __forceinline__ f16 ln_norm(float x, float mean, float rstd, f16 ga, f16 be) { return (f16)((x - mean) * rstd * (float)ga + (float)be); }
template <int KC, int R, bool X32>
__global__ __launch_bounds__(256) void k_layernorm(const void *__restrict__ x, const f16 *__restrict__ gamma,
                                                   const f16 *__restrict__ beta, int64_t rows, int C, float eps,
                                                   f16 *__restrict__ y)
{
    const int lane = threadIdx.x & 63;
    const int c8n = C / 8;
    const int64_t wave = ((int64_t)blockIdx.x * 256 + threadIdx.x) >> 6;
    const int64_t row0 = wave * R;
    if (row0 >= rows) return;
    Wide8 v[R][KC];
#pragma unroll
    for (int rr = 0; rr < R; ++rr)
#pragma unroll
        for (int k = 0; k < KC; ++k) {
            int c8 = lane + 64 * k;
            const int64_t rw = row0 + rr < rows ? row0 + rr : rows - 1;
            v[rr][k] = ldraw<X32>(x, (size_t)(rw * C + min(c8, c8n - 1) * 8)).widen();
            if (c8 >= c8n) v[rr][k] = Wide8{};
        }
    f16x8 ga[KC], be[KC];
#pragma unroll
    for (int k = 0; k < KC; ++k) {
        int c8 = lane + 64 * k;
        ga[k] = *(const f16x8 *)(gamma + min(c8, c8n - 1) * 8);
        be[k] = *(const f16x8 *)(beta + min(c8, c8n - 1) * 8);
    }
#pragma unroll
    for (int rr = 0; rr < R; ++rr) {
        if (row0 + rr >= rows) break;
        float s = 0.f;
#pragma unroll
        for (int k = 0; k < KC; ++k)
#pragma unroll
            for (int j = 0; j < 8; ++j) s += v[rr][k].get(j);
        float mean = wave_sum_dpp(s) / (float)C;
        float q = 0.f;
#pragma unroll
        for (int k = 0; k < KC; ++k) {
            int c8 = lane + 64 * k;
            if (c8 < c8n) {
#pragma unroll
                for (int j = 0; j < 8; ++j) { float d = v[rr][k].get(j) - mean; q += d * d; }
            }
        }
        float rstd = rsqrtf(wave_sum_dpp(q) / (float)C + eps);
        f16 *yr = y + (row0 + rr) * C;
#pragma unroll
        for (int k = 0; k < KC; ++k) {
            int c8 = lane + 64 * k;
            if (c8 < c8n) {
                f16x8 o;
#pragma unroll
                for (int j = 0; j < 8; ++j) o[j] = ln_norm(v[rr][k].get(j), mean, rstd, ga[k][j], be[k][j]);
                *(f16x8 *)(yr + c8 * 8) = o;
            }
        }
    }
}

template <int KC>
__global__ __launch_bounds__(256) void k_layernorm_g8(const f16 *__restrict__ x, const f16 *__restrict__ gamma, const f16 *__restrict__ beta,
                                                      int64_t rows, float eps, f16 *__restrict__ y)
{
    constexpr int C = 64 * KC;
    const int lane = threadIdx.x & 63, s = lane & 7, rw = lane >> 3;
    const int64_t wave = ((int64_t)blockIdx.x * 256 + threadIdx.x) >> 6;
    const int64_t row = wave * 8 + rw;
    const bool live = row < rows;
    const f16 *xr = x + (live ? row : rows - 1) * C + s * 8;
    Raw8<false> v[KC];
#pragma unroll
    for (int k = 0; k < KC; ++k) v[k] = ldraw<false>(xr, k * 64);
    f16x8 ga[KC], be[KC];
#pragma unroll
    for (int k = 0; k < KC; ++k) {
        ga[k] = *(const f16x8 *)(gamma + k * 64 + s * 8);
        be[k] = *(const f16x8 *)(beta + k * 64 + s * 8);
    }
    float sum = 0.f;
#pragma unroll
    for (int k = 0; k < KC; ++k)
#pragma unroll
        for (int j = 0; j < 8; ++j) sum += v[k].get(j);
    const float mean = sum8_dpp(sum) / (float)C;
    float q = 0.f;
#pragma unroll
    for (int k = 0; k < KC; ++k)
#pragma unroll
        for (int j = 0; j < 8; ++j) { const float d = v[k].get(j) - mean; q += d * d; }
    const float rstd = rsqrtf(sum8_dpp(q) / (float)C + eps);
    if (!live) return;
    f16 *yr = y + row * C + s * 8;
#pragma unroll
    for (int k = 0; k < KC; ++k) {
        f16x8 o;
#pragma unroll
        for (int j = 0; j < 8; ++j) o[j] = ln_norm(v[k].get(j), mean, rstd, ga[k][j], be[k][j]);
        *(f16x8 *)(yr + k * 64) = o;
    }
}

extern "C" int32_t ctx_layernorm_f16(const void *x, const void *gamma, const void *beta, int64_t rows, int32_t C, float eps,
                                     void *y, ctx_stream_t stream)
{
    return ctx_layernorm_any(x, 0, gamma, beta, rows, C, eps, y, (hipStream_t)stream);
}

int ctx_layernorm_any(const void *x, int x32, const void *gamma, const void *beta, int64_t rows, int C, float eps, void *y, hipStream_t stream)
{
    CTX_REQUIRE(x && gamma && beta && y && rows > 0 && C % 8 == 0 && C <= 2048, "layernorm: unsupported rows=%lld C=%d", (long long)rows, C);
    {
        static const int g8 = ctx_env_int("CTX_LN_G8", 1);
        if (g8 && !x32 && C % 64 == 0 && C <= 640 && rows >= 64) {
            const unsigned nb = (unsigned)cdiv64(cdiv64(rows, 8), 4);
#define LN_G8(KC_) case KC_: hipLaunchKernelGGL(k_layernorm_g8<KC_>, dim3(nb), dim3(256), 0, stream, (const f16 *)x, (const f16 *)gamma, (const f16 *)beta, rows, eps, (f16 *)y); break
            switch (C / 64) {
                LN_G8(1); LN_G8(2); LN_G8(3); LN_G8(4); LN_G8(5); LN_G8(6); LN_G8(7); LN_G8(8); LN_G8(9); LN_G8(10);
            }
#undef LN_G8
            CTX_CHECK_LAUNCH("layernorm");
            return CTX_OK;
        }
    }
    const int kc = (C / 8 + 63) / 64;
#define LN_GO(KC_, R_) CTX_BOOL_GO(x32, X, hipLaunchKernelGGL((k_layernorm<KC_, R_, X>), dim3((unsigned)cdiv64(cdiv64(rows, R_), 4)), dim3(256), 0, stream, x, \
                                                          (const f16 *)gamma, (const f16 *)beta, rows, C, eps, (f16 *)y))
    const bool many = rows >= 8192;
    if (kc == 1) { if (many) LN_GO(1, 4); else LN_GO(1, 1); }
    else if (kc == 2) { if (many) LN_GO(2, 2); else LN_GO(2, 1); }
    else if (kc == 3) LN_GO(3, 1);
    else LN_GO(4, 1);
#undef LN_GO
    CTX_CHECK_LAUNCH("layernorm");
    return CTX_OK;
}
```

### contexture-nerf_amd/csrc/unet.hip

```cpp
#include "engine.h"
#include <string.h>

struct ResP {
    int cin, cout;
    size_t n1g, n1b, c1w, c1b, n2g, n2b, c2w, c2b, scw, scb;
    int temb_row;
};
struct TrP {
    int C, heads;
    size_t ng, nb, piw, pib, l1g, l1b, qkv, o1w, o1b, l2g, l2b, q2, kv2, o2w, o2b, l3g, l3b, f1w, f1b, f2w, f2b, pow_, pob;
    int kv_row;
};
struct LevelP {
    std::vector<ResP> res;
    std::vector<TrP> tr;
    bool has_attn = false, has_sampler = false;
    size_t sw = 0, sb = 0;
    int sc = 0;
};

struct ctx_unet : Engine {
    ctx_unet_config_t cfg;
    size_t ciw, cib, t1w, t1b, t2w, t2b, tpw, tpb, cng, cnb, cow, cob;
    int temb_dim = 0, temb_rows = 0;
    size_t kvw = 0;
    int kv_rows_total = 0, kv_rows = 0;
    std::vector<LevelP> down, up;
    LevelP mid;
    struct RefSlot { size_t off; int tokens, C, rows; };
    int ref_mode = 0;
    f16 *ref_bank = nullptr;
    size_t ref_cursor = 0;
    int ref_k = 0, ref_row0 = 0;
    std::vector<RefSlot> ref_slots;
    bool is_controlnet = false;
    int cond_channels = 3;
    struct CondConv { size_t w, b; int cin, cout, stride; };
    std::vector<CondConv> cond_convs;
    std::vector<size_t> zc_w, zc_b;
    std::vector<int> zc_c;
    size_t zm_w = 0, zm_b = 0;
    const float *cn_cond = nullptr;
    f16 *cn_cache = nullptr;
    bool cn_cache_valid = false;
    f16 *cn_out = nullptr;
    const f16 *add_res = nullptr;
    float add_scale = 1.0f;
    bool res32 = false;
    void *allocS(size_t n) { return alloc(n * (res32 ? 4 : 2)); }
    struct Tap { size_t off; int rows, C; };
    f16 *tap_buf = nullptr;
    size_t tap_cap = 0, tap_cursor = 0;
    std::vector<Tap> taps;
    void tap(const void *x, int rows, int C)
    {
        if (!tap_buf || res32) return;
        const size_t n = (size_t)rows * C;
        Tap t = {tap_cursor, rows, C};
        taps.push_back(t);
        if (tap_cursor + n <= tap_cap) copy(tap_buf + tap_cursor, x, n * 2);
        tap_cursor += n;
    }
};

static void add_resnet(ctx_unet *u, const std::string &p, int cin, int cout, ResP &r)
{
    r.cin = cin; r.cout = cout;
    r.n1g = u->vec(p + ".norm1.weight", cin); r.n1b = u->vec(p + ".norm1.bias", cin);
    r.c1w = u->add(p + ".conv1.weight", {cout, cin, 3, 3}, PK_CONV3, u->walloc((size_t)cout * cin * 9), cout, cin);
    r.c1b = u->vec(p + ".conv1.bias", cout);
    r.temb_row = u->temb_rows;
    u->add(p + ".time_emb_proj.weight", {cout, u->temb_dim}, PK_COPY, u->tpw + (size_t)u->temb_rows * u->temb_dim);
    u->add(p + ".time_emb_proj.bias", {cout}, PK_COPY, u->tpb + u->temb_rows);
    u->temb_rows += cout;
    r.n2g = u->vec(p + ".norm2.weight", cout); r.n2b = u->vec(p + ".norm2.bias", cout);
    r.c2w = u->add(p + ".conv2.weight", {cout, cout, 3, 3}, PK_CONV3, u->walloc((size_t)cout * cout * 9), cout, cout);
    r.c2b = u->vec(p + ".conv2.bias", cout);
    if (cin != cout) {
        r.scw = u->add(p + ".conv_shortcut.weight", {cout, cin, 1, 1}, PK_COPY, u->walloc((size_t)cout * cin));
        r.scb = u->vec(p + ".conv_shortcut.bias", cout);
    } else r.scw = r.scb = 0;
}

static void add_transformer(ctx_unet *u, const std::string &p, int C, int heads, TrP &t)
{
    int cd = u->cfg.cross_attention_dim;
    t.C = C; t.heads = heads;
    t.ng = u->vec(p + ".norm.weight", C); t.nb = u->vec(p + ".norm.bias", C);
    t.piw = u->lin(p + ".proj_in.weight", C, C); t.pib = u->vec(p + ".proj_in.bias", C);
    std::string b = p + ".transformer_blocks.0";
    t.l1g = u->vec(b + ".norm1.weight", C); t.l1b = u->vec(b + ".norm1.bias", C);
    t.qkv = u->walloc((size_t)3 * C * C);
    u->add(b + ".attn1.to_q.weight", {C, C}, PK_COPY, t.qkv);
    u->add(b + ".attn1.to_k.weight", {C, C}, PK_COPY, t.qkv + (size_t)C * C);
    u->add(b + ".attn1.to_v.weight", {C, C}, PK_COPY, t.qkv + (size_t)2 * C * C);
    t.o1w = u->lin(b + ".attn1.to_out.0.weight", C, C); t.o1b = u->vec(b + ".attn1.to_out.0.bias", C);
    t.l2g = u->vec(b + ".norm2.weight", C); t.l2b = u->vec(b + ".norm2.bias", C);
    t.q2 = u->lin(b + ".attn2.to_q.weight", C, C);
    t.kv_row = u->kv_rows;
    t.kv2 = u->kvw + (size_t)u->kv_rows * cd;
    u->kv_rows += 2 * C;
    u->add(b + ".attn2.to_k.weight", {C, cd}, PK_COPY, t.kv2);
    u->add(b + ".attn2.to_v.weight", {C, cd}, PK_COPY, t.kv2 + (size_t)C * cd);
    t.o2w = u->lin(b + ".attn2.to_out.0.weight", C, C); t.o2b = u->vec(b + ".attn2.to_out.0.bias", C);
    t.l3g = u->vec(b + ".norm3.weight", C); t.l3b = u->vec(b + ".norm3.bias", C);
    t.f1w = u->add(b + ".ff.net.0.proj.weight", {8 * C, C}, PK_GEGLU_W, u->walloc((size_t)8 * C * C), 4 * C, C);
    t.f1b = u->add(b + ".ff.net.0.proj.bias", {8 * C}, PK_GEGLU_B, u->walloc((size_t)8 * C), 4 * C, 0);
    t.f2w = u->lin(b + ".ff.net.2.weight", C, 4 * C); t.f2b = u->vec(b + ".ff.net.2.bias", C);
    t.pow_ = u->lin(p + ".proj_out.weight", C, C); t.pob = u->vec(p + ".proj_out.bias", C);
}

static ctx_unet_t *unet_create_impl(const ctx_unet_config_t *cfg, bool controlnet, int cond_channels)
{
    if (!cfg || cfg->n_levels < 1 || cfg->n_levels > 4 || cfg->in_channels > 16 || cfg->out_channels > 4 ||
        cfg->groups > 64 || cfg->layers_per_block < 1 || cfg->layers_per_block > 4 || cfg->cross_attention_dim % 64) {
        ctx_set_error("unet_create: unsupported config");
        return nullptr;
    }
    for (int i = 0; i < cfg->n_levels; ++i)
        if (cfg->block_out_channels[i] % 64 || cfg->block_out_channels[i] % cfg->groups || cfg->heads[i] * 64 != cfg->block_out_channels[i]) {
            ctx_set_error("unet_create: level %d: channels %d must be a multiple of 64 and of groups, with head_dim 64 (heads=%d)",
                          i, cfg->block_out_channels[i], cfg->heads[i]);
            return nullptr;
        }
    ctx_unet *u = new ctx_unet();
    u->tag = "unet";
    u->cfg = *cfg;
    const int n = cfg->n_levels, lpb = cfg->layers_per_block;
    const int *ch = cfg->block_out_channels;
    u->temb_dim = ch[0] * 4;
    int rows = 0;
    u->is_controlnet = controlnet; u->cond_channels = cond_channels;
    for (int i = 0; i < n; ++i) rows += lpb * ch[i];
    rows += 2 * ch[n - 1];
    if (!controlnet)
        for (int i = 0; i < n; ++i) rows += (lpb + 1) * ch[n - 1 - i];
    u->tpw = u->walloc((size_t)rows * u->temb_dim);
    u->tpb = u->walloc(rows);
    {
        int kvr = 2 * ch[n - 1];
        for (int i = 0; i < n; ++i) {
            if (cfg->down_attn[i]) kvr += lpb * 2 * ch[i];
            if (cfg->up_attn[i] && !controlnet) kvr += (lpb + 1) * 2 * ch[n - 1 - i];
        }
        u->kv_rows_total = kvr;
        u->kvw = u->walloc((size_t)kvr * cfg->cross_attention_dim);
    }

    u->ciw = u->add("conv_in.weight", {ch[0], cfg->in_channels, 3, 3}, PK_CONVIN, u->walloc((size_t)ch[0] * 9 * (cfg->in_channels > 8 ? 16 : 8)), ch[0],
                    cfg->in_channels);
    u->cib = u->vec("conv_in.bias", ch[0]);
    u->t1w = u->lin("time_embedding.linear_1.weight", u->temb_dim, ch[0]); u->t1b = u->vec("time_embedding.linear_1.bias", u->temb_dim);
    u->t2w = u->lin("time_embedding.linear_2.weight", u->temb_dim, u->temb_dim); u->t2b = u->vec("time_embedding.linear_2.bias", u->temb_dim);
    u->down.resize(n);
    int out = ch[0];
    for (int i = 0; i < n; ++i) {
        LevelP &L = u->down[i];
        int cin = out; out = ch[i];
        std::string p = "down_blocks." + std::to_string(i);
// ... 206 lines not shown

static int gn_epi_mode(void)
{
    static const int m = ctx_env_int("CTX_GN_EPI", 2);
    return m;
}
static GnReq gn_request(ctx_unet *u, void *stats, int HW, int C, bool want)
{
    GnReq r;
    if (want && (gn_epi_mode() == 1 || gn_epi_mode() == 2) && !u->res32 && C % u->cfg.groups == 0 && ctx_groupnorm_two_pass(HW, C, u->cfg.groups)) {
        r.part = (float *)stats; r.groups = u->cfg.groups; r.HW = HW;
    }
    return r;
}

static void op_gemm(ctx_unet *u, const f16 *X, size_t w, size_t bias, bool has_bias, const void *res, int M, int N, int K, void *out,
                    int epi = 0, bool res_s = false, bool out_s = false, const GnReq *gn = nullptr)
{
    engine_linear(*u, X, u->W + w, has_bias ? u->W + bias : nullptr, res, M, N, K, out, 0, epi, u->res32 && res_s && res, u->res32 && out_s, gn);
}
static void op_conv(ctx_unet *u, const f16 *x, size_t w, size_t bias, const f16 *rowbias, int ldrb, const void *res, int B, int H,
                    int W, int Cin, int Cout, int stride, int ups, void *out, bool res_s = false, bool out_s = false, const ConvSegs *segs = nullptr,
                    const GnReq *gn = nullptr, GnSlabs *slabs = nullptr)
{
    engine_conv3(*u, x, u->W + w, u->W + bias, res, B, H, W, Cin, Cout, out, ConvGeom{stride, ups}, rowbias, ldrb, u->res32 && res_s && res,
                 u->res32 && out_s, segs, gn, slabs);
}
static void op_gn(ctx_unet *u, const void *x, size_t g, size_t b, int B, int HW, int C, float eps, int silu, f16 *y, void *stats, bool x_s = true,
                  const void *x2 = nullptr, int Ca = 0)
{
    u->note(2, 0, 2);
    const Engine::GnTag t = u->gn_tag;
    u->gn_tag = Engine::GnTag();
    if (t.x && t.x == x && !x2 && !(u->res32 && x_s) && t.B == B && t.HW == HW && t.C == C && t.groups == u->cfg.groups) {
        ++u->gn_from_producer;
        RUN(ctx_groupnorm_apply(x, (const float *)stats, t.NS, u->W + g, u->W + b, B, HW, C, u->cfg.groups, eps, silu, y, u->s));
        return;
    }
    RUN(ctx_groupnorm_any(x, (u->res32 && x_s) ? 1 : 0, u->W + g, u->W + b, B, HW, C, u->cfg.groups, eps, silu, y, stats, u->s, x2, Ca));
}
static void op_ln(ctx_unet *u, const void *x, size_t g, size_t b, int64_t rows, int C, f16 *y)
{
    u->note(2, 0);
    RUN(ctx_layernorm_any(x, u->res32 ? 1 : 0, u->W + g, u->W + b, rows, C, 1e-5f, y, u->s));
}
static const f16 *op_as16(ctx_unet *u, const void *x, size_t n)
{
    if (!u->res32) return (const f16 *)x;
    f16 *c = u->allocH(n);
    u->note(2, 0);
    RUN(ctx_f32_to_f16_core((const float *)x, (int64_t)n, c, u->s));
    return c;
}
static void op_attn(ctx_unet *u, const f16 *Q, const f16 *K, const f16 *V, int B, int Sq, int Skv, int heads, int qs, int kvs, f16 *O)
{
    u->note(1, 4.0 * B * heads * (double)Sq * Skv * 64);
    RUN(ctx_attention_core(Q, K, V, B, Sq, Skv, heads, qs, kvs, 0.125f, O, heads * 64, u->s));
}

struct FwdCtx {
    int B, L;
    const f16 *tproj;
    const f16 *ctx16;
    const f16 *kv_all;
    void *gn_stats;
};

static int resnet_fold_mode(void)
{
    static const int m = ctx_env_int("CTX_RESNET_FOLD", 1);
    return m;
}
static bool resnet_fold_loses(int M, int cin, int cout) { return M == 4608 && cin == 320 && cout == 640; }

static void *run_resnet(ctx_unet *u, const FwdCtx &f, const ResP &r, const void *x, int H, int W, void *out, bool gn_next, const void *x2 = nullptr,
                        int Ca = 0)
{
    const int B = f.B, HW = H * W, M = B * HW;
    size_t mark = u->top;
    const int mode = u->res32 ? 0 : resnet_fold_mode();
    const bool pair = Ca > 0;
    const int Cb = r.cin - Ca;
    const bool segs_ok = r.cout % 32 == 0 && (pair ? (Ca % 32 == 0 && Cb % 32 == 0) : r.cin % 32 == 0);
    const bool fold = mode == 1 && r.cin != r.cout && segs_ok && !resnet_fold_loses(M, r.cin, r.cout);
    const bool gn_pair = pair && mode != 0 && Ca % 8 == 0;
    const void *xin = x;
    if (pair) {
        u->note(2, 0);
        if (!gn_pair || !fold) {
            void *cat = u->allocS((size_t)M * r.cin);
// ... 22 lines not shown
    } else {
        f16 *h = u->allocH((size_t)M * r.cout);
        const GnReq rq = gn_request(u, f.gn_stats, HW, r.cout, true);
        op_conv(u, t1, r.c1w, r.c1b, trow, u->temb_rows, nullptr, B, H, W, r.cin, r.cout, 1, 0, h, false, false, nullptr, &rq);
        t2 = u->allocH((size_t)M * r.cout);
        op_gn(u, h, r.n2g, r.n2b, B, HW, r.cout, u->cfg.norm_eps, 1, t2, f.gn_stats, false);
    }
    const GnReq rq2 = gn_request(u, f.gn_stats, HW, r.cout, gn_next);
    if (fold) {
        ConvSegs sg;
        sg.n = pair ? 2 : 1; sg.bias2 = u->W + r.scb;
        sg.x[0] = (const f16 *)x; sg.w[0] = u->W + r.scw; sg.C[0] = pair ? Ca : r.cin; sg.ldw[0] = r.cin;
        if (pair) { sg.x[1] = (const f16 *)x2; sg.w[1] = u->W + r.scw + Ca; sg.C[1] = Cb; sg.ldw[1] = r.cin; }
        op_conv(u, t2, r.c2w, r.c2b, nullptr, 0, nullptr, B, H, W, r.cout, r.cout, 1, 0, out, true, true, &sg, &rq2);
        u->top = mark;
        return out;
    }
    const void *sc = xin;
    if (r.cin != r.cout) {
        void *s2 = u->allocS((size_t)M * r.cout);
        op_gemm(u, op_as16(u, xin, (size_t)M * r.cin), r.scw, r.scb, true, nullptr, M, r.cout, r.cin, s2, 0, false, true);
        sc = s2;
    }
    op_conv(u, t2, r.c2w, r.c2b, nullptr, 0, sc, B, H, W, r.cout, r.cout, 1, 0, out, true, true, nullptr, &rq2);
    u->top = mark;
    return out;
}

static void *run_transformer(ctx_unet *u, const FwdCtx &f, const TrP &t, const void *x, int H, int W, void *out, bool gn_next)
{
    const int B = f.B, S = H * W, M = B * S, C = t.C, cd = u->cfg.cross_attention_dim;
    size_t mark = u->top;
    f16 *g = u->allocH((size_t)M * C);
    op_gn(u, x, t.ng, t.nb, B, S, C, 1e-6f, 0, g, f.gn_stats);
    void *h0 = u->allocS((size_t)M * C);
    op_gemm(u, g, t.piw, t.pib, true, nullptr, M, C, C, h0, 0, false, true);
    f16 *l = g;
    op_ln(u, h0, t.l1g, t.l1b, M, C, l);
    f16 *a = nullptr;
    if (u->ref_mode == 2) {
        if (u->ref_k >= (int)u->ref_slots.size() || u->ref_slots[u->ref_k].C != C ||
            u->ref_slots[u->ref_k].rows != B - u->ref_row0) {
            u->rc = CTX_E_STATE;
            ctx_set_error("unet: the reference bank does not match this pass (run the 'w' pass on the condition latent first; layer %d)", u->ref_k);
            u->top = mark;
            return out;
        }
        const ctx_unet::RefSlot sl = u->ref_slots[u->ref_k++];
        f16 *q = u->allocH((size_t)M * C);
        op_gemm(u, l, t.qkv, 0, false, nullptr, M, C, C, q);
        a = u->allocH((size_t)M * C);
        f16 *kv = u->allocH((size_t)(S + sl.tokens) * 2 * C);
        for (int b = 0; b < B; ++b) {
            const int Sr = b >= u->ref_row0 ? sl.tokens : 0;
            op_gemm(u, l ? l + (size_t)b * S * C : nullptr, t.qkv + (size_t)C * C, 0, false, nullptr, S, 2 * C, C, kv);
            if (Sr)
                op_gemm(u, u->ref_bank ? u->ref_bank + sl.off + (size_t)(b - u->ref_row0) * sl.tokens * C : nullptr,
                        t.qkv + (size_t)C * C, 0, false, nullptr, Sr, 2 * C, C, kv ? kv + (size_t)S * 2 * C : nullptr);
            op_attn(u, q ? q + (size_t)b * S * C : nullptr, kv, kv ? kv + C : nullptr, 1, S, S + Sr, t.heads, C, 2 * C,
                    a ? a + (size_t)b * S * C : nullptr);
        }
    } else {
        if (u->ref_mode == 1) {
            ctx_unet::RefSlot sl; sl.off = u->ref_cursor; sl.tokens = S; sl.C = C; sl.rows = B;
            u->ref_slots.push_back(sl);
            u->ref_cursor += (size_t)M * C;
            if (u->ref_bank) u->copy(u->ref_bank + sl.off, l, (size_t)M * C * 2);
        }
        f16 *qkv = u->allocH((size_t)M * 3 * C);
        op_gemm(u, l, t.qkv, 0, false, nullptr, M, 3 * C, C, qkv);
        a = u->allocH((size_t)M * C);
        op_attn(u, qkv, qkv + C, qkv + 2 * C, B, S, S, t.heads, 3 * C, 3 * C, a);
    }
    void *h1 = u->allocS((size_t)M * C);
    op_gemm(u, a, t.o1w, t.o1b, true, h0, M, C, C, h1, 0, true, true);
    op_ln(u, h1, t.l2g, t.l2b, M, C, l);
    f16 *q = a;
    op_gemm(u, l, t.q2, 0, false, nullptr, M, C, C, q);
    const f16 *kv = f.kv_all + t.kv_row;
    f16 *a2 = u->allocH((size_t)M * C);
    op_attn(u, q, kv, kv + C, B, S, f.L, t.heads, C, u->kv_rows_total, a2);
    void *h2 = h0;
    op_gemm(u, a2, t.o2w, t.o2b, true, h1, M, C, C, h2, 0, true, true);
    op_ln(u, h2, t.l3g, t.l3b, M, C, l);
    f16 *ff = u->allocH((size_t)M * 4 * C);
    op_gemm(u, l, t.f1w, t.f1b, true, nullptr, M, 8 * C, C, ff, 1);
    void *h3 = h1;
    op_gemm(u, ff, t.f2w, t.f2b, true, h2, M, C, 4 * C, h3, 0, true, true);
    const GnReq rq = gn_request(u, f.gn_stats, S, C, gn_next);
    op_gemm(u, op_as16(u, h3, (size_t)M * C), t.pow_, t.pob, true, x, M, C, C, out, 0, true, true, &rq);
    u->top = mark;
    return out;
}

static int unet_run(ctx_unet *u, const float *sample, const float *timestep, const float *ctx, int B, int H, int W, int L, float *out)
{
    const ctx_unet_config_t &c = u->cfg;
    const int n = c.n_levels, lpb = c.layers_per_block;
    const int *ch = c.block_out_channels;
    u->begin();
    u->ref_k = 0; u->ref_cursor = 0;
    u->taps.clear(); u->tap_cursor = 0;
    if (u->ref_mode == 1) u->ref_slots.clear();
    FwdCtx f; f.B = B; f.L = L;
    f.gn_stats = u->alloc((size_t)ctx_groupnorm_ws_bytes(B, c.groups));
    f16 *te0 = u->allocH((size_t)B * ch[0]);
    u->note(2, 0); RUN(ctx_time_embed_core(timestep, B, ch[0], te0, u->s));
    f16 *te1 = u->allocH((size_t)B * u->temb_dim);
    u->note(2, 2.0 * B * ch[0] * u->temb_dim); RUN(ctx_gemv_core(te0, u->W + u->t1w, u->W + u->t1b, B, u->temb_dim, ch[0], 0, 1, te1, u->s));
    f16 *te2 = u->allocH((size_t)B * u->temb_dim);
    u->note(2, 2.0 * B * u->temb_dim * u->temb_dim); RUN(ctx_gemv_core(te1, u->W + u->t2w, u->W + u->t2b, B, u->temb_dim, u->temb_dim, 0, 1, te2, u->s));
    f16 *tproj = u->allocH((size_t)B * u->temb_rows);
    u->note(2, 2.0 * B * u->temb_rows * u->temb_dim); RUN(ctx_gemv_core(te2, u->W + u->tpw, u->W + u->tpb, B, u->temb_rows, u->temb_dim, 0, 0, tproj, u->s));
    f.tproj = tproj;
    f16 *ctx16 = u->allocH((size_t)B * L * c.cross_attention_dim);
    u->note(2, 0); RUN(ctx_f32_to_f16_core(ctx, (int64_t)B * L * c.cross_attention_dim, ctx16, u->s));
    f.ctx16 = ctx16;
    f16 *kv_all = u->allocH((size_t)B * L * u->kv_rows_total);
    op_gemm(u, ctx16, u->kvw, 0, false, nullptr, B * L, u->kv_rows_total, c.cross_attention_dim, kv_all);
    f.kv_all = kv_all;

    int h = H, w = W;
    if (u->res32 && (u->is_controlnet || u->add_res || u->ref_mode)) {
        ctx_set_error("unet: the fp32 residual-stream mode covers the plain UNet forward only");
        return CTX_E_STATE;
    }
    void *x = u->allocS((size_t)B * h * w * ch[0]);
    {
        size_t m0 = u->top;
        f16 *x16 = u->res32 ? u->allocH((size_t)B * h * w * ch[0]) : (f16 *)x;
        u->note(2, 2.0 * B * h * w * ch[0] * c.in_channels * 9); RUN(ctx_conv_in_core(sample, u->W + u->ciw, u->W + u->cib, B, c.in_channels, h, w, ch[0], x16, u->s));
        if (u->res32) { u->note(2, 0); RUN(ctx_f16_to_f32_core(x16, (int64_t)B * h * w * ch[0], (float *)x, u->s)); u->top = m0; }
    }

    auto add_scaled = [&](f16 *dst, const f16 *src, float scale, size_t n) {
        u->note(2, 0);
        RUN(ctx_add_scaled_core(dst, src, scale, (int64_t)n, u->s));
    };
    if (u->is_controlnet) {
        size_t mark = u->top;
        int eh = 8 * H, ew = 8 * W;
        const f16 *cur16 = nullptr;
        const size_t nconv = u->cond_convs.size();
        for (size_t k = 0; k + 1 < nconv; ++k) {
            const ctx_unet::CondConv &cc = u->cond_convs[k];
            int oh = (eh - 1) / cc.stride + 1, ow = (ew - 1) / cc.stride + 1;
            const bool last = k + 2 == nconv;
            f16 *o = (last && u->cn_cache) ? u->cn_cache : u->allocH((size_t)B * oh * ow * cc.cout);
            if (!u->cn_cache_valid) {
                u->note(2, 2.0 * B * oh * ow * cc.cout * cc.cin * 9);
                RUN(ctx_conv_small_core(k == 0 ? u->cn_cond : nullptr, cur16, u->W + cc.w, u->W + cc.b, B, eh, ew, cc.cin, cc.cout, cc.stride, 1, o, u->s));
            }
            cur16 = o; eh = oh; ew = ow;
        }
        if (eh != h || ew != w) { ctx_set_error("controlnet: conditioning embedding grid %dx%d != latent grid %dx%d", eh, ew, h, w); return CTX_E_ARG; }
        const ctx_unet::CondConv &co = u->cond_convs.back();
        f16 *emb = u->allocH((size_t)B * h * w * ch[0]);
        op_conv(u, cur16, co.w, co.b, nullptr, 0, x, B, h, w, co.cin, ch[0], 1, 0, emb);
        u->copy(x, emb, (size_t)B * h * w * ch[0] * 2);
        u->top = mark;
    }
    struct Skip { void *p; int C, h, w; };
    std::vector<Skip> skips;
    skips.push_back({x, ch[0], h, w});
// ... 71 lines not shown
    for (int i = 0; i < n; ++i) {
        LevelP &Lv = u->up[i];
        for (int j = 0; j <= lpb; ++j) {
            Skip sk = skips.back(); skips.pop_back();
            if (sk.h != h || sk.w != w) { ctx_set_error("unet: skip size mismatch (H, W must be multiples of %d)", 1 << (n - 1)); return CTX_E_ARG; }
            int cin = cur + sk.C, cout = Lv.res[j].cout;
            void *o = u->allocS((size_t)B * h * w * cout);
            size_t mark = u->top;
            if (cin != Lv.res[j].cin) { ctx_set_error("unet: up block input has %d channels, its resnet expects %d", cin, Lv.res[j].cin); return CTX_E_STATE; }
            const bool last = i == n - 1 && j == lpb && !Lv.has_sampler;
            if (Lv.has_attn) {
                void *t = u->allocS((size_t)B * h * w * cout);
                run_resnet(u, f, Lv.res[j], x, h, w, t, true, sk.p, cur);
                u->tap(t, B * h * w, cout);
                run_transformer(u, f, Lv.tr[j], t, h, w, o, last);
            } else run_resnet(u, f, Lv.res[j], x, h, w, o, last, sk.p, cur);
            u->tap(o, B * h * w, cout);
            u->top = mark;
            x = o; cur = cout;
        }
        if (Lv.has_sampler) {
            void *o = u->allocS((size_t)B * (2 * h) * (2 * w) * cur);
            size_t m0 = u->top;
            op_conv(u, op_as16(u, x, (size_t)B * h * w * cur), Lv.sw, Lv.sb, nullptr, 0, nullptr, B, h, w, cur, cur, 1, 1, o, false, true);
            u->top = m0;
            x = o; h *= 2; w *= 2;
            u->tap(x, B * h * w, cur);
        }
    }
    f16 *y = u->allocH((size_t)B * h * w * cur);
    op_gn(u, x, u->cng, u->cnb, B, h * w, cur, c.norm_eps, 1, y, f.gn_stats);
    u->note(2, 2.0 * B * h * w * cur * c.out_channels * 9);
    RUN(ctx_conv_out_core(y, u->W + u->cow, u->W + u->cob, B, h, w, cur, c.out_channels, out, u->s));
    return engine_finish(u, "unet_forward");
}

static int unet_dry(ctx_unet *u, int B, int H, int W, int L)
{
    return engine_dry_run(u, [&] { return unet_run(u, nullptr, nullptr, nullptr, B, H, W, L, nullptr); });
}

static int check_dims(const ctx_unet *u, int B, int H, int W, int L)
{
    int div = 1 << (u->cfg.n_levels - 1);
    if (B < 1 || B > 16 || H < div || W < div || H % div || W % div || L < 1) {
        ctx_set_error("unet: need 1<=B<=16, H,W multiples of %d, ctx_len>=1 (B=%d H=%d W=%d L=%d)", div, B, H, W, L);
        return CTX_E_ARG;
    }
    return 0;
}

extern "C" int64_t ctx_unet_workspace_bytes(const ctx_unet_t *cu, int32_t B, int32_t H, int32_t W, int32_t ctx_len)
{
    ctx_unet *u = const_cast<ctx_unet *>(cu);
    if (!u || check_dims(u, B, H, W, ctx_len)) return -1;
    unet_dry(u, B, H, W, ctx_len);
    return engine_workspace_need(u);
}

extern "C" int32_t ctx_unet_forward(ctx_unet_t *u, const float *sample, const float *timestep, const float *ctx, int32_t B,
                                    int32_t H, int32_t W, int32_t ctx_len, float *out, ctx_stream_t stream)
{
    CTX_REQUIRE(u && sample && timestep && ctx && out, "unet_forward: null pointer");
    CTX_REQUIRE(u->W && u->ws, "unet_forward: ctx_unet_bind() first");
    if (check_dims(u, B, H, W, ctx_len)) return CTX_E_ARG;
    u->s = (hipStream_t)stream;
// ... 71 lines not shown
    CTX_REQUIRE(u->W && u->ws, "unet_forward_ref: ctx_unet_bind() first");
    CTX_REQUIRE(mode == 1 || mode == 2, "unet_forward_ref: mode %d (1 = 'w' park the attn1 inputs, 2 = 'r' attend to them)", mode);
    CTX_REQUIRE(ref_row0 >= 0 && ref_row0 < B, "unet_forward_ref: ref_row0=%d outside [0, B)", ref_row0);
    if (check_dims(u, B, H, W, ctx_len)) return CTX_E_ARG;
    u->s = (hipStream_t)stream;
    u->dry = false;
    u->ref_mode = mode; u->ref_bank = (f16 *)bank; u->ref_row0 = mode == 2 ? ref_row0 : 0;
    int rc = unet_run(u, sample, timestep, ctx, B, H, W, ctx_len, out);
    u->ref_mode = 0; u->ref_bank = nullptr; u->ref_row0 = 0;
    return rc;
}

extern "C" int32_t ctx_unet_set_residual_fp32(ctx_unet_t *u, int32_t on)
{
    CTX_REQUIRE(u, "unet_set_residual_fp32: null handle");
    u->res32 = on != 0;
    return CTX_OK;
}

extern "C" int32_t ctx_unet_set_taps(ctx_unet_t *u, void *buf, int64_t capacity)
{
    CTX_REQUIRE(u && capacity >= 0, "unet_set_taps: bad args");
    u->tap_buf = (f16 *)buf; u->tap_cap = buf ? (size_t)capacity : 0;
    return CTX_OK;
}
extern "C" int32_t ctx_unet_tap_count(const ctx_unet_t *u) { return u ? (int32_t)u->taps.size() : -1; }
extern "C" int32_t ctx_unet_tap_info(const ctx_unet_t *u, int32_t i, int64_t *offset, int32_t *rows, int32_t *channels)
{
    CTX_REQUIRE(u && offset && rows && channels && i >= 0 && i < (int32_t)u->taps.size(), "unet_tap_info: bad args");
    *offset = (int64_t)u->taps[i].off; *rows = u->taps[i].rows; *channels = u->taps[i].C;
    return CTX_OK;
}

extern "C" int32_t ctx_unet_gn_epilogue_counts(const ctx_unet_t *u, int64_t *from_producer, int64_t *from_slabs)
{
    CTX_REQUIRE(u && from_producer && from_slabs, "unet_gn_epilogue_counts: bad args");
    *from_producer = u->gn_from_producer;
    *from_slabs = u->gn_from_slabs;
    return CTX_OK;
}

extern "C" int32_t ctx_unet_stats(const ctx_unet_t *u, int32_t klass, int64_t *launches, double *flops)
{
    CTX_REQUIRE(u && klass >= 0 && klass < 3 && launches && flops, "unet_stats: bad args");
    *launches = u->launches[klass];
    *flops = u->flops[klass];
    return CTX_OK;
}
```

### contexture-nerf_amd/unet.py

```python
import ctypes as C
import math
import torch
from . import _lib as L
from .engine import HipEngine


class UNetConfig(C.Structure):
    _fields_ = [("in_channels", C.c_int32), ("out_channels", C.c_int32), ("n_levels", C.c_int32),
                ("block_out_channels", C.c_int32 * 4), ("heads", C.c_int32 * 4),
                ("down_attn", C.c_int32 * 4), ("up_attn", C.c_int32 * 4), ("layers_per_block", C.c_int32),
                ("cross_attention_dim", C.c_int32), ("groups", C.c_int32), ("norm_eps", C.c_float)]


SD2_DEPTH = dict(in_channels=5, out_channels=4, block_out_channels=(320, 640, 1280, 1280), layers_per_block=2,
                 down_attn=(True, True, True, False), up_attn=(False, True, True, True),
                 cross_attention_dim=1024, heads=(5, 10, 20, 20), groups=32, norm_eps=1e-5)


def _pad4(xs):
    xs = [int(x) for x in xs]
    return (C.c_int32 * 4)(*(xs + [0] * (4 - len(xs))))


class UNet2DConditionModel(HipEngine):
    _prefix = 'ctx_unet'

    def __init__(self, config=None, device="cuda:0", seed=0, init=True):
        super().__init__(dict(SD2_DEPTH if config is None else config), device=device, seed=seed, init=init)

    def _config_struct(self):
        cfg = self.config
        return UNetConfig(cfg['in_channels'], cfg['out_channels'], len(cfg['block_out_channels']),
                          _pad4(cfg['block_out_channels']), _pad4(cfg['heads']), _pad4(cfg['down_attn']),
                          _pad4(cfg['up_attn']), cfg['layers_per_block'], cfg['cross_attention_dim'], cfg['groups'],
                          cfg['norm_eps'])

    def _create_handle(self):
        h = self._lib.ctx_unet_create(C.byref(self._config_struct()))
        if not h:
            raise L.CtxError("ctx_unet_create: " + self._lib.ctx_last_error().decode())
        return h

    def _init_state(self, src=None):
        self.in_channels = self.config['in_channels']
        self._res32 = False
        if src is not None and src._res32:
            self.set_residual_fp32(True)

    def load_state_dict(self, sd, strict=True):
        missing = [n for n in self._names if n not in sd]
        extra = [k for k in sd if k not in self._index]
        if strict and (missing or extra):
            raise L.CtxError(f"load_state_dict: missing {missing[:5]}... ({len(missing)}), unexpected {extra[:5]}... ({len(extra)})")
        self._load(sd)
        return missing, extra

    @staticmethod
    def _init_scale(u, fan):
        b = 1.0 / math.sqrt(fan)
        return u * b

    def workspace_bytes(self, B, H, W, ctx_len):
        n = self._lib.ctx_unet_workspace_bytes(self._h, B, H, W, ctx_len)
        if n < 0:
            raise L.CtxError(self._lib.ctx_last_error().decode())
        return n

    def flops(self, B, H, W, ctx_len):
        self.workspace_bytes(B, H, W, ctx_len)
        out = {}
        for k, name in enumerate(('gemm_conv', 'attention', 'other')):
            n, f = C.c_int64(), C.c_double()
            L.check(self._lib.ctx_unet_stats(self._h, k, C.byref(n), C.byref(f)))
            out[name] = (n.value, f.value)
        return out

    def __call__(self, sample, timestep, encoder_hidden_states=None, down_block_additional_residuals=None,
                 mid_block_additional_residual=None, **kw):
        if down_block_additional_residuals is None:
            return self.forward(sample, timestep, encoder_hidden_states)
        with self.residuals(down_block_additional_residuals):
            return self.forward(sample, timestep, encoder_hidden_states)

    def residuals(self, res):
        unet = self

        class _Scope:
            def __enter__(s):
                if not isinstance(res, ControlResiduals):
                    raise L.CtxError("unet: additional residuals must come from contexture_nerf_amd.unet.ControlNetModel")
                L.check(unet._lib.ctx_unet_set_residuals(unet._h, L.ptr(res.buffer), float(res.scale)))
                unet._ws_key = None

            def __exit__(s, *a):
                L.check(unet._lib.ctx_unet_set_residuals(unet._h, None, 1.0))
                unet._ws_key = None
                return False
        return _Scope()

    def set_residual_fp32(self, on=True):
        L.check(self._lib.ctx_unet_set_residual_fp32(self._h, int(bool(on))))
        self._res32 = bool(on)
        self._ws_key = None
        return self

    def forward_ref(self, sample, timestep, encoder_hidden_states, mode, bank=None, ref_row0=0):
        m = {'w': 1, 'r': 2}.get(mode)
        if m is None:
            raise L.CtxError(f"unet.forward_ref: mode {mode!r} (expected 'w' or 'r')")
        x = L.f32c(sample, self.device)
        ctx = L.f32c(encoder_hidden_states, self.device)
        B, Cin, H, W = x.shape
        if Cin != self.in_channels or ctx.shape[0] != B or ctx.shape[2] != self.config['cross_attention_dim']:
            raise L.CtxError(f"unet.forward_ref: sample {tuple(x.shape)} / encoder_hidden_states {tuple(ctx.shape)} do not fit")
        Lc = ctx.shape[1]
        if m == 1:
            nb = self._lib.ctx_unet_ref_bank_bytes(self._h, B, H, W)
            if nb < 0:
                raise L.CtxError(self._lib.ctx_last_error().decode())
            if bank is None or bank.numel() < nb:
                bank = torch.empty(nb, dtype=torch.uint8, device=self.device)
        elif bank is None:
            raise L.CtxError("unet.forward_ref: mode 'r' needs the bank of a 'w' pass")
        self._reserve(self._lib.ctx_unet_workspace_bytes_ref(self._h, B, H, W, Lc, m, ref_row0 if m == 2 else 0))
        self._ws_key = None
        t = self._timestep(timestep)
        out = torch.empty(B, self.config['out_channels'], H, W, device=self.device)
        L.check(self._lib.ctx_unet_forward_ref(self._h, L.ptr(x, torch.float32, "sample"), L.ptr(t), L.ptr(ctx), B, H, W, Lc, m,
                                               L.ptr(bank), ref_row0, L.ptr(out), L.stream()))
        return {'sample': out}, bank

    def forward(self, sample, timestep, encoder_hidden_states):
        x = L.f32c(sample, self.device)
        ctx = L.f32c(encoder_hidden_states, self.device)
        B, Cin, H, W = x.shape
        if Cin != self.in_channels:
            raise L.CtxError(f"unet: expected {self.in_channels} input channels, got {Cin}")
# ... 80 lines not shown
```

### include/ctx_nerf.h

```cpp
#ifndef CTX_NERF_H
#define CTX_NERF_H
#include <stdint.h>
#ifdef __cplusplus
extern "C" {
#endif

#define CTX_OK 0
#define CTX_E_ARG (-1)
#define CTX_E_LAUNCH (-2)
#define CTX_E_STATE (-3)

typedef void *ctx_stream_t;

int32_t ctx_version(void);
const char *ctx_last_error(void);
int32_t ctx_device_check(void);

int32_t ctx_prepare_vertices(const float *verts, const int64_t *faces, const float *cam,
                             const float *proj3, int32_t B, int32_t V, int32_t F,
                             float *fv_cam, float *fv_img, float *fnorm,
                             void *ws , ctx_stream_t stream);

int64_t ctx_rasterize_ws_bytes(int32_t H, int32_t W, int32_t B, int32_t F);
int32_t ctx_rasterize_fwd(int32_t H, int32_t W, const float *face_z, const float *face_xy,
// ... 197 lines not shown
    int32_t groups;
    float norm_eps;
} ctx_unet_config_t;

ctx_unet_t *ctx_unet_create(const ctx_unet_config_t *cfg);
void ctx_unet_destroy(ctx_unet_t *u);
int32_t ctx_unet_param_count(const ctx_unet_t *u);
const char *ctx_unet_param_name(const ctx_unet_t *u, int32_t i);
int32_t ctx_unet_param_shape(const ctx_unet_t *u, int32_t i, int64_t shape4[4]);
int64_t ctx_unet_weight_bytes(const ctx_unet_t *u);
int64_t ctx_unet_workspace_bytes(const ctx_unet_t *u, int32_t B, int32_t H, int32_t W, int32_t ctx_len);
int32_t ctx_unet_bind(ctx_unet_t *u, void *weights, void *workspace, int64_t workspace_bytes);
int64_t ctx_unet_derived_bytes(const ctx_unet_t *u);
int32_t ctx_unet_bind_derived(ctx_unet_t *u, void *derived, int64_t bytes);
int32_t ctx_unet_set_param(ctx_unet_t *u, int32_t i, const float *src, ctx_stream_t stream);
int32_t ctx_unet_forward(ctx_unet_t *u, const float *sample, const float *timestep, const float *ctx,
                         int32_t B, int32_t H, int32_t W, int32_t ctx_len, float *out, ctx_stream_t stream);
int64_t ctx_unet_ref_bank_bytes(const ctx_unet_t *u, int32_t B, int32_t H, int32_t W);
int64_t ctx_unet_workspace_bytes_ref(const ctx_unet_t *u, int32_t B, int32_t H, int32_t W, int32_t ctx_len, int32_t mode,
                                     int32_t ref_row0);
int32_t ctx_unet_forward_ref(ctx_unet_t *u, const float *sample, const float *timestep, const float *ctx,
                             int32_t B, int32_t H, int32_t W, int32_t ctx_len, int32_t mode, void *bank, int32_t ref_row0,
                             float *out, ctx_stream_t stream);
ctx_unet_t *ctx_controlnet_create(const ctx_unet_config_t *cfg, int32_t cond_channels);
int64_t ctx_controlnet_residual_bytes(const ctx_unet_t *cn, int32_t B, int32_t H, int32_t W);
int64_t ctx_controlnet_cond_cache_bytes(const ctx_unet_t *cn, int32_t B, int32_t H, int32_t W);
int32_t ctx_controlnet_forward(ctx_unet_t *cn, const float *sample, const float *timestep, const float *ctx,
                               const float *cond , void *cond_cache, int32_t cache_valid,
                               int32_t B, int32_t H, int32_t W, int32_t ctx_len, void *residuals, ctx_stream_t stream);
int32_t ctx_unet_set_residuals(ctx_unet_t *u, const void *residuals , float scale);
int32_t ctx_unet_set_residual_fp32(ctx_unet_t *u, int32_t on);
int32_t ctx_unet_stats(const ctx_unet_t *u, int32_t klass, int64_t *launches, double *flops);
int32_t ctx_unet_gn_epilogue_counts(const ctx_unet_t *u, int64_t *from_producer, int64_t *from_slabs);
int32_t ctx_unet_set_taps(ctx_unet_t *u, void *buf, int64_t capacity);
int32_t ctx_unet_tap_count(const ctx_unet_t *u);
int32_t ctx_unet_tap_info(const ctx_unet_t *u, int32_t i, int64_t *offset, int32_t *rows, int32_t *channels);

typedef struct ctx_vae ctx_vae_t;
typedef struct {
    int32_t latent_channels, out_channels;
    int32_t n_levels;
    int32_t block_out_channels[4];
    int32_t layers_per_block;
    int32_t groups;
} ctx_vae_config_t;
ctx_vae_t *ctx_vae_create(const ctx_vae_config_t *cfg);
void ctx_vae_destroy(ctx_vae_t *v);
int32_t ctx_vae_param_count(const ctx_vae_t *v);
const char *ctx_vae_param_name(const ctx_vae_t *v, int32_t i);
int32_t ctx_vae_param_shape(const ctx_vae_t *v, int32_t i, int64_t shape4[4]);
int64_t ctx_vae_weight_bytes(const ctx_vae_t *v);
int64_t ctx_vae_workspace_bytes(const ctx_vae_t *v, int32_t B, int32_t H, int32_t W);
int32_t ctx_vae_bind(ctx_vae_t *v, void *weights, void *workspace, int64_t workspace_bytes);
int64_t ctx_vae_derived_bytes(const ctx_vae_t *v);
int32_t ctx_vae_bind_derived(ctx_vae_t *v, void *derived, int64_t bytes);
int32_t ctx_vae_set_param(ctx_vae_t *v, int32_t i, const float *src, ctx_stream_t stream);
int32_t ctx_vae_decode(ctx_vae_t *v, const float *latents, int32_t B, int32_t H, int32_t W, float *image, ctx_stream_t stream);
int32_t ctx_vae_decoder_param_count(const ctx_vae_t *v);
int64_t ctx_vae_encode_workspace_bytes(const ctx_vae_t *v, int32_t B, int32_t H, int32_t W);
int32_t ctx_vae_encode(ctx_vae_t *v, const float *image, int32_t B, int32_t H, int32_t W, float *moments, ctx_stream_t stream);
double ctx_vae_flops(const ctx_vae_t *v);
int64_t ctx_vae_encode_train_workspace_bytes(const ctx_vae_t *v, int32_t B, int32_t H, int32_t W);
int32_t ctx_vae_encode_train(ctx_vae_t *v, const float *image, int32_t B, int32_t H, int32_t W, float *moments, ctx_stream_t stream);
int32_t ctx_vae_encode_bwd(ctx_vae_t *v, const float *grad_moments, float gscale, float *grad_image, ctx_stream_t stream);

int32_t ctx_gemm_f16(const void *A, const void *Wt, const void *bias, const void *residual,
// ... 3 lines not shown
                        int32_t Cout, int32_t stride, int32_t upsample, void *y, ctx_stream_t stream);
int32_t ctx_conv3x3_seg_f16(const void *x, const void *w, const void *bias, const void *bias2, const void *rowbias,
                            const void *residual, int32_t B, int32_t H, int32_t W, int32_t Cin, int32_t Cout,
                            const void *xa, const void *wa, int32_t Ca, int32_t ldwa, const void *xb, const void *wb,
                            int32_t Cb, int32_t ldwb, void *part, int32_t splitk, void *y, ctx_stream_t stream);
int32_t ctx_conv3x3_gn_f16(const void *x, const void *w, const void *bias, const void *bias2, const void *rowbias,
                           const void *residual, int32_t B, int32_t H, int32_t W, int32_t Cin, int32_t Cout, void *part,
                           int32_t splitk, int32_t keep_slabs, int32_t groups, void *gn_part, int32_t *slots, void *y,
                           ctx_stream_t stream);
void ctx_gemm_last_kernel(int32_t *tile, int32_t *use8);
int32_t ctx_conv3x3_geom_f16(const void *x, const void *w, const void *bias, const void *residual, int32_t B, int32_t H, int32_t W,
                             int32_t Cin, int32_t Cout, int32_t stride, int32_t upsample, int32_t poff, int32_t zins, void *part,
                             int32_t splitk, void *y, ctx_stream_t stream);
int32_t ctx_pack_conv3_phase_f16(const float *src, int32_t Cout, int32_t Cin, void *dst, ctx_stream_t stream);
int32_t ctx_conv3x3_phase_f16(const void *x, const void *wp, const void *bias, const void *rowbias, const void *residual, int32_t B,
                              int32_t H, int32_t W, int32_t Cin, int32_t Cout, void *part, int32_t splitk, void *y, ctx_stream_t stream);
int32_t ctx_pack_conv3_dgrad_f16(const float *src, int32_t Cout, int32_t Cin, int32_t pad, void *dst, ctx_stream_t stream);
int32_t ctx_pack_mat_dgrad_f16(const float *src, int32_t out, int32_t in, int32_t ld, int32_t col, void *dst, ctx_stream_t stream);
int64_t ctx_groupnorm_bwd_ws_bytes(int32_t B, int32_t groups);
int32_t ctx_groupnorm_bwd_f16(const void *x, const void *dy, const void *gamma, const void *beta, const void *add, int32_t B, int32_t HW,
                              int32_t C, int32_t groups, float eps, int32_t silu, void *dx, void *ws, ctx_stream_t stream);
int32_t ctx_softmax_rows_f16(const void *s, int32_t rows, int32_t n, float scale, void *p, ctx_stream_t stream);
int32_t ctx_softmax_bwd_rows_f16(const void *P, const void *dP, int32_t rows, int32_t n, float scale, void *dS, ctx_stream_t stream);
int32_t ctx_quant_bwd_f16(const float *g, const void *w, int32_t B, int32_t C, int64_t HW, float gscale, void *d, ctx_stream_t stream);
int32_t ctx_conv_in_bwd_f16(const void *dy, const void *w_pack, int32_t B, int32_t H, int32_t W, int32_t C, int32_t Cimg, float inv_gscale,
                            float *dimg, ctx_stream_t stream);
int32_t ctx_conv_in_f16(const float *x, const void *w_pack, const void *bias, int32_t B, int32_t Cin, int32_t H, int32_t W, int32_t Cout,
                        void *y, ctx_stream_t stream);
int32_t ctx_conv_out_f16(const void *x, const void *w, const void *bias, int32_t B, int32_t H, int32_t W, int32_t C, int32_t Cout,
                         float *out, ctx_stream_t stream);
int32_t ctx_gemv_f16(const void *x, const void *w, const void *bias, int32_t Bm, int32_t N, int32_t K, int32_t silu_in, int32_t silu_out,
                     void *out, ctx_stream_t stream);
int32_t ctx_time_embed_f16(const float *t, int32_t B, int32_t dim, void *out, ctx_stream_t stream);
int32_t ctx_transpose_v_f16(const void *v, int32_t B, int32_t S, int32_t ld, int32_t heads, int32_t Sp, void *vt, ctx_stream_t stream);
int32_t ctx_concat_f16(const void *a, const void *b, int64_t M, int32_t Ca, int32_t Cb, void *y, ctx_stream_t stream);
int32_t ctx_concat_f32(const float *a, const float *b, int64_t M, int32_t Ca, int32_t Cb, float *y, ctx_stream_t stream);
int32_t ctx_f32_to_f16(const float *x, int64_t n, void *y, ctx_stream_t stream);
int32_t ctx_f16_to_f32(const void *x, int64_t n, float *y, ctx_stream_t stream);
int32_t ctx_conv_small_f16(const float *x32, const void *x16, const void *w, const void *bias, int32_t B, int32_t H, int32_t W, int32_t Cin,
                           int32_t Cout, int32_t stride, int32_t silu, void *y, ctx_stream_t stream);
int32_t ctx_add_scaled_f16(void *dst, const void *src, float scale, int64_t n, ctx_stream_t stream);
int32_t ctx_pointwise_f32(const void *x, const void *w, const void *b, int32_t B, int32_t C, int64_t HW, int32_t nhwc16, float *y,
                          ctx_stream_t stream);
int32_t ctx_pack_fwd_f16(const float *src, int32_t kind, int32_t a, int32_t b, void *dst, ctx_stream_t stream);
int64_t ctx_groupnorm_ws_bytes(int32_t B, int32_t groups);
int32_t ctx_groupnorm_f16(const void *x, const void *gamma, const void *beta, int32_t B, int32_t HW,
                          int32_t C, int32_t groups, float eps, int32_t silu, void *y, void *stats_ws,
                          ctx_stream_t stream);
int32_t ctx_groupnorm2_f16(const void *xa, const void *xb, int32_t Ca, const void *gamma, const void *beta, int32_t B,
                           int32_t HW, int32_t C, int32_t groups, float eps, int32_t silu, void *y, void *stats_ws,
                           ctx_stream_t stream);
int32_t ctx_groupnorm_apply_f16(const void *x, const void *part, int32_t slots, const void *gamma, const void *beta, int32_t B,
                                int32_t HW, int32_t C, int32_t groups, float eps, int32_t silu, void *y, ctx_stream_t stream);
int32_t ctx_groupnorm_slabs_f16(const void *part, int32_t splitk, const void *bias, const void *bias2, const void *rowbias,
                                int32_t ldrb, const void *gamma, const void *beta, int32_t B, int32_t HW, int32_t C,
                                int32_t groups, float eps, int32_t silu, void *y, ctx_stream_t stream);
int32_t ctx_layernorm_f16(const void *x, const void *gamma, const void *beta, int64_t rows, int32_t C,
                          float eps, void *y, ctx_stream_t stream);
int64_t ctx_attention_ws_bytes(int32_t B, int32_t Skv, int32_t heads);
int32_t ctx_attention_f16(const void *Q, const void *K, const void *V, int32_t B, int32_t Sq, int32_t Skv,
                          int32_t heads, int32_t q_stride, int32_t kv_stride, float scale, void *O,
                          int32_t o_stride, void *vt_ws, ctx_stream_t stream);
int32_t ctx_geglu_f16(const void *h, int64_t M, int32_t C4, void *y, ctx_stream_t stream);

int32_t ctx_cfg_plms_step(const float *eps_pair, int64_t n, float guidance, float *ets, int32_t head,
                          const float *coef4, float sample_coeff, float eps_coeff, int32_t mode,
// ... 23 lines not shown
```

Before: 120.7 steps/s.

## Share identical CFG pair rows up to first cross-attention, computing once and duplicating

```diff
diff --git a/contexture-nerf_amd/_lib.py b/contexture-nerf_amd/_lib.py
--- a/contexture-nerf_amd/_lib.py
+++ b/contexture-nerf_amd/_lib.py
@@ -115,6 +115,8 @@
     "ctx_unet_set_residual_fp32": (_i32, [_vp, _i32]),
     "ctx_unet_stats": (_i32, [_vp, _i32, _vp, _vp]),
     "ctx_unet_gn_epilogue_counts": (_i32, [_vp, _vp, _vp]),
+    "ctx_unet_set_pair_share": (_i32, [_vp, _i32]),
+    "ctx_unet_pair_share_ops": (_i32, [_vp]),
     "ctx_unet_set_taps": (_i32, [_vp, _vp, _i64]),
     "ctx_unet_tap_count": (_i32, [_vp]),
     "ctx_unet_tap_info": (_i32, [_vp, _i32, _vp, _vp, _vp]),
@@ -158,6 +160,7 @@
     "ctx_conv_out_f16": (_i32, [_vp, _vp, _vp, _i32, _i32, _i32, _i32, _i32, _vp, _vp]),
     "ctx_gemv_f16": (_i32, [_vp, _vp, _vp, _i32, _i32, _i32, _i32, _i32, _vp, _vp]),
     "ctx_time_embed_f16": (_i32, [_vp, _i32, _i32, _vp, _vp]),
+    "ctx_time_embed_pairs_f16": (_i32, [_vp, _i32, _i32, _vp, _vp, _i64, _vp, _i32, _i32, _vp]),
     "ctx_transpose_v_f16": (_i32, [_vp, _i32, _i32, _i32, _i32, _i32, _vp, _vp]),
     "ctx_concat_f16": (_i32, [_vp, _vp, _i64, _i32, _i32, _vp, _vp]),
     "ctx_concat_f32": (_i32, [_vp, _vp, _i64, _i32, _i32, _vp, _vp]),
diff --git a/contexture-nerf_amd/csrc/attention.hip b/contexture-nerf_amd/csrc/attention.hip
--- a/contexture-nerf_amd/csrc/attention.hip
+++ b/contexture-nerf_amd/csrc/attention.hip
@@ -13,6 +13,8 @@
     int q_stride, kv_stride, o_stride;
     float scale_log2e;
     float lazy;
+    const int *pair;
+    int pair_epoch;
 };
 
 
@@ -108,6 +110,11 @@
     const int tid = threadIdx.x, lane = tid & 63, wave = __builtin_amdgcn_readfirstlane(tid >> 6);
     const int r = lane & 31, h = lane >> 5;
     const int b = blockIdx.z, hd = blockIdx.y;
+    size_t o_twin = 0;
+    if (a.pair && pair_shared(a.pair, a.pair_epoch, b)) {
+        if (b & 1) return;
+        o_twin = (size_t)a.Sq * a.o_stride;
+    }
     const int q0 = blockIdx.x * (32 * NW) + wave * 32;
     const int qrow = q0 + r;
     const bool qok = qrow < a.Sq;
@@ -227,6 +234,7 @@
 #pragma unroll
                 for (int j = 0; j < 4; ++j) v[j] = (f16)(o[d][4 * g + j] * inv);
                 *(f16x4 *)(op + d * 32 + 8 * g + 4 * h) = v;
+                if (o_twin) *(f16x4 *)(op + o_twin + d * 32 + 8 * g + 4 * h) = v;
             }
     }
 }
@@ -268,9 +276,10 @@
 }
 
 int ctx_attention_core(const f16 *Q, const f16 *K, const f16 *V, int B, int Sq, int Skv, int heads, int q_stride,
-                       int kv_stride, float scale, f16 *O, int o_stride, hipStream_t s)
+                       int kv_stride, float scale, f16 *O, int o_stride, hipStream_t s, const PairShare *pair)
 {
     AttnArgs a;
+    a.pair = pair ? pair->mism : nullptr; a.pair_epoch = pair ? pair->epoch : 0;
     a.Q = Q; a.K = K; a.V = V; a.O = O; a.Sq = Sq; a.Skv = Skv; a.heads = heads;
     a.q_stride = q_stride; a.kv_stride = kv_stride; a.o_stride = o_stride;
     a.scale_log2e = scale * 1.4426950408889634f;
diff --git a/contexture-nerf_amd/csrc/common.h b/contexture-nerf_amd/csrc/common.h
--- a/contexture-nerf_amd/csrc/common.h
+++ b/contexture-nerf_amd/csrc/common.h
@@ -57,6 +57,15 @@
     asm volatile("" ::: "memory");
 }
 
+struct PairShare { const int *mism = nullptr; int epoch = 0; int rows = 0; int dup = 0; };
+__device__ __forceinline__ bool pair_shared(const int *mism, int epoch, int b) { return mism[b >> 1] != epoch; }
+__device__ __forceinline__ bool pair_rows_dead(const int *mism, int epoch, unsigned rows, unsigned first, unsigned last)
+{
+    if (!mism) return false;
+    const unsigned b = first / rows;
+    return (b & 1) && last / rows == b && pair_shared(mism, epoch, (int)b);
+}
+
 __device__ __forceinline__ float wave_sum(float v)
 {
 #pragma unroll
diff --git a/contexture-nerf_amd/csrc/elementwise.hip b/contexture-nerf_amd/csrc/elementwise.hip
--- a/contexture-nerf_amd/csrc/elementwise.hip
+++ b/contexture-nerf_amd/csrc/elementwise.hip
@@ -113,9 +113,8 @@
     return CTX_OK;
 }
 
-__global__ void k_time_embed(const float *__restrict__ t, int B, int dim, f16 *__restrict__ out)
-{
-    int i = blockIdx.x * blockDim.x + threadIdx.x;
+__device__ __forceinline__ void time_embed_item(const float *__restrict__ t, int B, int dim, f16 *__restrict__ out, int i)
+{
     int half = dim / 2;
     if (i >= half) return;
     float fr = expf(-9.210340371976184f * (float)i / (float)half);
@@ -126,10 +125,52 @@
         out[(size_t)b * dim + half + i] = (f16)sn;
     }
 }
+__global__ void k_time_embed(const float *__restrict__ t, int B, int dim, f16 *__restrict__ out)
+{
+    time_embed_item(t, B, dim, out, blockIdx.x * blockDim.x + threadIdx.x);
+}
 int ctx_time_embed_core(const float *t, int B, int dim, f16 *out, hipStream_t s)
 {
     CTX_REQUIRE(t && out && B > 0 && dim >= 2 && dim % 2 == 0, "time_embed: unsupported B=%d dim=%d", B, dim);
     hipLaunchKernelGGL(k_time_embed, dim3(cdiv(dim / 2, 64)), dim3(64), 0, s, t, B, dim, out);
+    CTX_CHECK_LAUNCH("time_embed");
+    return CTX_OK;
+}
+
+#define PS_CHUNK 2048
+__global__ __launch_bounds__(64) void k_time_embed_pairs(const float *__restrict__ t, int B, int dim, f16 *__restrict__ out, int nte,
+                                                         const unsigned *__restrict__ sample, int64_t per, int chunks, int *__restrict__ mism,
+                                                         int epoch)
+{
+    if ((int)blockIdx.x < nte) { time_embed_item(t, B, dim, out, blockIdx.x * 64 + threadIdx.x); return; }
+    const int k = blockIdx.x - nte;
+    if (k == 0) {
+        if (threadIdx.x == 0) {
+            if (B & 1) mism[B >> 1] = epoch;
+            if (!chunks)
+                for (int p = 0; p < B / 2; ++p) mism[p] = epoch - 1;
+        }
+        return;
+    }
+    const int p = (k - 1) / chunks, ch = (k - 1) - p * chunks;
+    const unsigned *xa = sample + (int64_t)(2 * p) * per, *xb = xa + per;
+    const int64_t i0 = (int64_t)ch * PS_CHUNK + threadIdx.x;
+    bool ne = false;
+#pragma unroll 8
+    for (int j = 0; j < PS_CHUNK / 64; ++j) {
+        const int64_t i = i0 + 64 * j;
+        if (i < per) ne |= xa[i] != xb[i];
+    }
+    if (__any(ne) && threadIdx.x == 0) mism[p] = epoch;
+}
+int ctx_time_embed_pairs_core(const float *t, int B, int dim, f16 *out, const float *sample, int64_t per, int *mism, int epoch, int forced,
+                              hipStream_t s)
+{
+    CTX_REQUIRE(t && out && B > 0 && dim >= 2 && dim % 2 == 0, "time_embed: unsupported B=%d dim=%d", B, dim);
+    CTX_REQUIRE(sample && mism && per > 0, "time_embed: the pair-sharing words need the sample and a buffer of (B + 1) / 2 words");
+    const int nte = cdiv(dim / 2, 64), chunks = forced ? 0 : (int)cdiv64(per, PS_CHUNK);
+    hipLaunchKernelGGL(k_time_embed_pairs, dim3(nte + 1 + (B / 2) * chunks), dim3(64), 0, s, t, B, dim, out, nte, (const unsigned *)sample, per,
+                       chunks, mism, epoch);
     CTX_CHECK_LAUNCH("time_embed");
     return CTX_OK;
 }
@@ -138,8 +179,9 @@
 template <int CP, int CX>
 __global__ __launch_bounds__(256) void k_conv_in(const float *__restrict__ x, const f16 *__restrict__ w,
                                                  const f16 *__restrict__ bias, int B, int Cin, int H, int W, int Cout,
-                                                 f16 *__restrict__ y)
-{
+                                                 f16 *__restrict__ y, PairShare ps)
+{
+    if (pair_rows_dead(ps.mism, ps.epoch, H * W, blockIdx.x * 256, min((int64_t)(blockIdx.x + 1) * 256, (int64_t)B * H * W) - 1)) return;
     extern __shared__ __attribute__((aligned(16))) float s_w[];
     constexpr int WR = 9 * CP, WX = 9 * CX;
     const int o8n = Cout / 8;
@@ -188,13 +230,28 @@
         __syncthreads();
         for (int ch = threadIdx.x; ch < 256 * ng; ch += 256) {
             const int px = ch / ng, gi = ch - px * ng;
-            if (pix0 + px < npix) *(f16x8 *)(y + (pix0 + px) * Cout + (g0 + gi) * 8) = *(const f16x8 *)(patch + px * 72 + gi * 8);
+            if (pix0 + px < npix) {
+                const int64_t m = pix0 + px;
+                const f16x8 v = *(const f16x8 *)(patch + px * 72 + gi * 8);
+                int64_t twin = 0;
+                bool own = true;
+                if (ps.mism) {
+                    const int sb = (int)(m / (H * W));
+                    if (pair_shared(ps.mism, ps.epoch, sb)) { own = !(sb & 1); twin = (int64_t)H * W; }
+                }
+                if (own) {
+                    *(f16x8 *)(y + m * Cout + (g0 + gi) * 8) = v;
+                    if (twin) *(f16x8 *)(y + (m + twin) * Cout + (g0 + gi) * 8) = v;
+                }
+            }
         }
         __syncthreads();
     }
 }
-int ctx_conv_in_core(const float *x, const f16 *w, const f16 *bias, int B, int Cin, int H, int W, int Cout, f16 *y, hipStream_t s)
-{
+int ctx_conv_in_core(const float *x, const f16 *w, const f16 *bias, int B, int Cin, int H, int W, int Cout, f16 *y, hipStream_t s,
+                     const PairShare *pair)
+{
+    const PairShare ps = pair ? *pair : PairShare();
     CTX_REQUIRE(x && w && bias && y && Cout > 0 && Cout % 8 == 0, "conv_in: unsupported Cout=%d", Cout);
     CTX_REQUIRE(Cin >= 1 && Cin <= 16, "conv_in: need 1 <= Cin <= 16 (Cin=%d)", Cin);
     CTX_REQUIRE(B > 0 && H > 0 && W > 0 && (int64_t)H * W < (1ll << 31), "conv_in: unsupported grid B=%d H=%d W=%d", B, H, W);
@@ -204,7 +261,7 @@
     CTX_REQUIRE((size_t)o8_per * 8 * 9 * cx * sizeof(float) + 256 * 72 * sizeof(f16) <= 64 * 1024,
                 "conv_in: the weight slice of Cout=%d at Cin=%d does not fit the LDS", Cout, Cin);
     const dim3 grid((unsigned)cdiv64(npix, 256), CI_SPLIT);
-#define CI_GO(CP_, CX_) hipLaunchKernelGGL((k_conv_in<CP_, CX_>), grid, dim3(256), (size_t)o8_per * 8 * 9 * CX_ * sizeof(float) + 256 * 72 * sizeof(f16), s, x, w, bias, B, Cin, H, W, Cout, y)
+#define CI_GO(CP_, CX_) hipLaunchKernelGGL((k_conv_in<CP_, CX_>), grid, dim3(256), (size_t)o8_per * 8 * 9 * CX_ * sizeof(float) + 256 * 72 * sizeof(f16), s, x, w, bias, B, Cin, H, W, Cout, y, ps)
     if (Cin <= 3) CI_GO(8, 3);
     else if (Cin == 4) CI_GO(8, 4);
     else if (Cin == 5) CI_GO(8, 5);
@@ -383,6 +440,11 @@
 {
     return ctx_f16_to_f32_core((const f16 *)x, n, y, (hipStream_t)stream);
 }
+extern "C" int32_t ctx_time_embed_pairs_f16(const float *t, int32_t B, int32_t dim, void *out, const float *sample, int64_t per, void *mism,
+                                            int32_t epoch, int32_t forced, ctx_stream_t stream)
+{
+    return ctx_time_embed_pairs_core(t, B, dim, (f16 *)out, sample, per, (int *)mism, epoch, forced, (hipStream_t)stream);
+}
 extern "C" int32_t ctx_time_embed_f16(const float *t, int32_t B, int32_t dim, void *out, ctx_stream_t stream)
 {
     return ctx_time_embed_core(t, B, dim, (f16 *)out, (hipStream_t)stream);
diff --git a/contexture-nerf_amd/csrc/engine.h b/contexture-nerf_amd/csrc/engine.h
--- a/contexture-nerf_amd/csrc/engine.h
+++ b/contexture-nerf_amd/csrc/engine.h
@@ -35,6 +35,8 @@
 
     struct GnTag { const void *x = nullptr; int B = 0, HW = 0, C = 0, groups = 0, NS = 0; } gn_tag;
     int64_t gn_from_producer = 0, gn_from_slabs = 0;
+    PairShare pair;
+    int pair_ops = 0;
 
     size_t walloc(size_t n) { size_t o = wtop; wtop += (n + 127) / 128 * 128; return o; }
     size_t add(const std::string &name, std::vector<int64_t> shp, int kind, size_t dst, int a = 0, int b = 0)
@@ -72,7 +74,7 @@
 
     void begin()
     {
-        top = 0; peak = 0; rc = 0; gn_tag = GnTag(); gn_from_producer = 0; gn_from_slabs = 0;
+        top = 0; peak = 0; rc = 0; gn_tag = GnTag(); gn_from_producer = 0; gn_from_slabs = 0; pair = PairShare(); pair_ops = 0;
         for (int k = 0; k < 3; ++k) { launches[k] = 0; flops[k] = 0; }
     }
     void note(int klass, double fl, int n = 1) { launches[klass] += n; flops[klass] += fl; }
diff --git a/contexture-nerf_amd/csrc/engine.hip b/contexture-nerf_amd/csrc/engine.hip
--- a/contexture-nerf_amd/csrc/engine.hip
+++ b/contexture-nerf_amd/csrc/engine.hip
@@ -53,11 +53,18 @@
     if (a.zins) a.use8 = 0;
     if (a.splitk > 1) a.part = (float *)e.alloc((size_t)a.splitk * a.M * a.N * 4);
     if (gn && gn->part && gn->groups > 0 && a.N % gn->groups == 0) { a.gn_part = gn->part; a.gn_cg = a.N / gn->groups; a.gn_hw = gn->HW; }
+    const bool paired = e.pair.mism && a.splitk <= 1 && !a.phase && e.pair.rows > 0 && a.M % e.pair.rows == 0;
+    if (paired) { a.pair = e.pair.mism; a.pair_epoch = e.pair.epoch; a.pair_rows = e.pair.rows; }
     if (slabs) {
         a.keep_slabs = 1;
         *slabs = GnSlabs{a.part, a.splitk, (size_t)a.M * a.N, a.bias, a.bias2, a.rowbias, a.ldrb};
     }
     ENGINE_RUN(&e, ctx_gemm_dispatch(a, conv, e.s));
+    if (e.live() && paired) {
+        int32_t tile = -1, use8 = -1;
+        ctx_gemm_last_kernel(&tile, &use8);
+        if (use8 == 0 || (use8 >= 4 && use8 <= 8)) ++e.pair_ops;
+    }
     if (e.live() && a.gn_part) e.gn_tag = Engine::GnTag{a.out, a.M / a.gn_hw, a.gn_hw, a.N, gn->groups, a.gn_ns};
     if (!slabs) e.top = mark;
 }
diff --git a/contexture-nerf_amd/csrc/gemm.hip b/contexture-nerf_amd/csrc/gemm.hip
--- a/contexture-nerf_amd/csrc/gemm.hip
+++ b/contexture-nerf_amd/csrc/gemm.hip
@@ -89,6 +89,7 @@
     const int r = lane & 31, h = lane >> 5;
     const int wm = wave / WN, wn = wave % WN;
     const GemmTile t = gemm_tile(a, blockIdx.x, PKT, BM, BN);
+    if (!PH && pair_rows_dead(a.pair, a.pair_epoch, a.pair_rows, t.m0, min(t.m0 + BM, a.M) - 1)) return;
     static_assert(!PH || CONV, "the phase form is a convolution");
     const ConvPhase ph = PH ? conv_phase_tile(a, t.tile_m, BM) : ConvPhase{0, 0, 0, t.m0, a.M};
     const int slice = t.slice, tile_m = t.tile_m, tile_n = t.tile_n, m0 = ph.m0, n0 = t.n0, kbeg = t.kbeg, nk = t.nk;
diff --git a/contexture-nerf_amd/csrc/gemm144.hip b/contexture-nerf_amd/csrc/gemm144.hip
--- a/contexture-nerf_amd/csrc/gemm144.hip
+++ b/contexture-nerf_amd/csrc/gemm144.hip
@@ -23,6 +23,7 @@
 
     const GemmTile tl = gemm_tile(a, blockIdx.x, 64, BM, G144_BN);
     constexpr bool PH = UPS == 2;
+    if (!PH && pair_rows_dead(a.pair, a.pair_epoch, a.pair_rows, tl.m0, min(tl.m0 + BM, a.M) - 1)) return;
     static_assert(!PH || (CONV && !GNP), "the phase form is a convolution without GroupNorm partials");
     const ConvPhase ph = PH ? conv_phase_tile(a, tl.tile_m, BM) : ConvPhase{0, 0, 0, tl.m0, a.M};
     const int slice = tl.slice, m0 = ph.m0, n0 = tl.n0, kbeg = tl.kbeg, nk = tl.nk;
diff --git a/contexture-nerf_amd/csrc/kernels.h b/contexture-nerf_amd/csrc/kernels.h
--- a/contexture-nerf_amd/csrc/kernels.h
+++ b/contexture-nerf_amd/csrc/kernels.h
@@ -35,6 +35,8 @@
     int gn_cg, gn_hw;
     int gn_ns;
     int keep_slabs;
+    const int *pair;
+    int pair_epoch, pair_rows;
 };
 #define CTX_GN_MAX_SLOTS 128
 #define CTX_GEMM_MAX_SEG 2
@@ -67,20 +69,24 @@
 int ctx_transpose_v_core(const f16 *v, int B, int S, int ld, int heads, int Sp, f16 *vt, hipStream_t s);
 int ctx_f32_to_f16_core(const float *x, int64_t n, f16 *y, hipStream_t s);
 int ctx_time_embed_core(const float *t, int B, int dim, f16 *out, hipStream_t s);
-int ctx_conv_in_core(const float *x, const f16 *w, const f16 *bias, int B, int Cin, int H, int W, int Cout, f16 *y, hipStream_t s);
+int ctx_time_embed_pairs_core(const float *t, int B, int dim, f16 *out, const float *sample, int64_t per, int *mism, int epoch, int forced,
+                              hipStream_t s);
+int ctx_conv_in_core(const float *x, const f16 *w, const f16 *bias, int B, int Cin, int H, int W, int Cout, f16 *y, hipStream_t s,
+                     const PairShare *pair = nullptr);
 int ctx_conv_out_core(const f16 *x, const f16 *w, const f16 *bias, int B, int H, int W, int C, int Cout, float *out, hipStream_t s);
 int ctx_attention_core(const f16 *Q, const f16 *K, const f16 *V, int B, int Sq, int Skv, int heads, int q_stride,
-                       int kv_stride, float scale, f16 *O, int o_stride, hipStream_t s);
+                       int kv_stride, float scale, f16 *O, int o_stride, hipStream_t s, const PairShare *pair = nullptr);
 extern "C" int64_t ctx_groupnorm_ws_bytes(int32_t B, int32_t groups);
 int ctx_groupnorm_any(const void *x, int x32, const void *gamma, const void *beta, int B, int HW, int C, int groups, float eps, int silu,
-                      void *y, void *stats_ws, hipStream_t stream, const void *x2 = nullptr, int Ca = 0);
+                      void *y, void *stats_ws, hipStream_t stream, const void *x2 = nullptr, int Ca = 0, const PairShare *pair = nullptr);
 int ctx_groupnorm_two_pass(int HW, int C, int groups);
 int ctx_groupnorm_apply(const void *x, const float *part, int NS, const void *gamma, const void *beta, int B, int HW, int C, int groups, float eps,
-                        int silu, void *y, hipStream_t stream);
+                        int silu, void *y, hipStream_t stream, const PairShare *pair = nullptr);
 struct GnSlabs { const float *part; int S; size_t MN; const f16 *bias, *bias2, *rowbias; int ldrb; };
 int ctx_groupnorm_slabs(const GnSlabs &sl, const void *gamma, const void *beta, int B, int HW, int C, int groups, float eps, int silu, void *y,
                         hipStream_t stream);
-int ctx_layernorm_any(const void *x, int x32, const void *gamma, const void *beta, int64_t rows, int C, float eps, void *y, hipStream_t stream);
+int ctx_layernorm_any(const void *x, int x32, const void *gamma, const void *beta, int64_t rows, int C, float eps, void *y, hipStream_t stream,
+                      const PairShare *pair = nullptr);
 int ctx_concat32_core(const float *a, const float *b, int64_t M, int Ca, int Cb, float *y, hipStream_t s);
 int ctx_f16_to_f32_core(const f16 *x, int64_t n, float *y, hipStream_t s);
 int ctx_conv_small_core(const float *x32, const f16 *x16, const f16 *w, const f16 *bias, int B, int H, int W, int Cin, int Cout, int stride, int silu,
diff --git a/contexture-nerf_amd/csrc/norm.hip b/contexture-nerf_amd/csrc/norm.hip
--- a/contexture-nerf_amd/csrc/norm.hip
+++ b/contexture-nerf_amd/csrc/norm.hip
@@ -39,6 +39,15 @@
     return r;
 }
 
+template <class V8>
+__device__ __forceinline__ void pair_copy(const V8 &v, f16 *dst)
+{
+    f16x8 o;
+#pragma unroll
+    for (int j = 0; j < 8; ++j) o[j] = (f16)v.get(j);
+    *(f16x8 *)dst = o;
+}
+
 struct GnSrc { const void *p; int cs, col; };
 __device__ __forceinline__ GnSrc gn_src(const void *x, const void *x2, int Ca, int C, int ch)
 {
@@ -55,8 +64,9 @@
 
 template <bool X32>
 __global__ __launch_bounds__(1024) void k_gn_stats(const void *__restrict__ x, const void *__restrict__ x2, int Ca, int HW, int C, int G,
-                                                   int NS, int PL, float *__restrict__ part)
-{
+                                                   int NS, int PL, float *__restrict__ part, PairShare ps)
+{
+    if (ps.mism && (blockIdx.y & 1) && pair_shared(ps.mism, ps.epoch, blockIdx.y)) return;
     extern __shared__ float s_part[];
     const int c8n = C / 8;
     const int b = blockIdx.y, sp = blockIdx.x;
@@ -151,8 +161,9 @@
 template <bool X32>
 __global__ __launch_bounds__(512) void k_gn_apply(const void *__restrict__ x, const void *__restrict__ x2, int Ca, const float *__restrict__ part,
                                                   const f16 *__restrict__ gamma, const f16 *__restrict__ beta, int HW, int C,
-                                                  int G, int NS, int PL, float eps, int silu, f16 *__restrict__ y)
-{
+                                                  int G, int NS, int PL, float eps, int silu, f16 *__restrict__ y, PairShare ps)
+{
+    if (ps.mism && (blockIdx.y & 1) && pair_shared(ps.mism, ps.epoch, blockIdx.y)) return;
     constexpr int AU = GN_AU;
     __shared__ float s_mean[GN_MAX_GROUPS], s_rstd[GN_MAX_GROUPS];
     const int b = blockIdx.y;
@@ -162,6 +173,7 @@
     const GnSrc src = gn_src(x, x2, Ca, C, c8 * 8);
     const size_t xb = (size_t)b * HW * src.cs + src.col;
     f16 *yb = y + (size_t)b * HW * C + c8 * 8;
+    f16 *const twin = (!X32 && ps.dup && ps.mism && pair_shared(ps.mism, ps.epoch, b)) ? (f16 *)const_cast<void *>(x) + (size_t)(b + 1) * HW * C + c8 * 8 : nullptr;
     Raw8<X32> v[AU];
 #pragma unroll
     for (int u = 0; u < AU; ++u) v[u] = ldraw<X32>(src.p, xb + (size_t)min(p0 + u * PL + pl, HW - 1) * src.cs);
@@ -194,7 +206,10 @@
 #pragma unroll
     for (int u = 0; u < AU; ++u) {
         const int p = p0 + u * PL + pl;
-        if (p < HW) gn_store(v[u], sa, sh, silu, yb + (size_t)p * C);
+        if (p < HW) {
+            gn_store(v[u], sa, sh, silu, yb + (size_t)p * C);
+            if (twin) pair_copy(v[u], twin + (size_t)p * C);
+        }
     }
 }
 
@@ -224,8 +239,9 @@
 template <bool X32, bool SLAB = false>
 __global__ __launch_bounds__(GN_FT) void k_gn_fused(const void *__restrict__ x, const void *__restrict__ x2, int Ca, const f16 *__restrict__ gamma,
                                                     const f16 *__restrict__ beta, int HW, int C, int G, int PLF, float eps, int silu,
-                                                    f16 *__restrict__ y, GnSlabs sl)
-{
+                                                    f16 *__restrict__ y, GnSlabs sl, PairShare ps)
+{
+    if (ps.mism && (blockIdx.y & 1) && pair_shared(ps.mism, ps.epoch, blockIdx.y)) return;
     __shared__ float s_red[2][GN_FT / 64];
     const int g = blockIdx.x, b = blockIdx.y;
     const int cg = C / G, cpg = cg / 8;
@@ -234,6 +250,7 @@
     const GnSrc src = gn_src(x, x2, Ca, C, g * cg + c * 8);
     const size_t xb = (size_t)b * HW * src.cs + src.col;
     f16 *yb = y + (size_t)b * HW * C + g * cg + c * 8;
+    f16 *const twin = (!X32 && !SLAB && ps.dup && ps.mism && pair_shared(ps.mism, ps.epoch, b)) ? (f16 *)const_cast<void *>(x) + (size_t)(b + 1) * HW * C + g * cg + c * 8 : nullptr;
     const f16x8 ga = *(const f16x8 *)(gamma + g * cg + c * 8), be = *(const f16x8 *)(beta + g * cg + c * 8);
     Wide8 v[GN_FU];
 #pragma unroll
@@ -261,7 +278,10 @@
 #pragma unroll
     for (int u = 0; u < GN_FU; ++u) {
         const int p = pl + PLF * u;
-        if (act && p < HW) gn_store(v[u], sa, sh, silu, yb + (size_t)p * C);
+        if (act && p < HW) {
+            gn_store(v[u], sa, sh, silu, yb + (size_t)p * C);
+            if (twin) pair_copy(v[u], twin + (size_t)p * C);
+        }
     }
 }
 
@@ -278,14 +298,14 @@
     return (fuse && plf > 0 && cpg <= GN_FT && (HW + plf - 1) / plf <= GN_FU) ? plf : 0;
 }
 static void gn_launch_apply(const void *x, int x32, const void *x2, int Ca, const float *part, int NS, const void *gamma, const void *beta, int B, int HW,
-                            int C, int groups, float eps, int silu, void *y, hipStream_t stream)
+                            int C, int groups, float eps, int silu, void *y, hipStream_t stream, const PairShare &ps)
 {
     const int c8n = C / 8;
     const int apl = (256 + c8n - 1) / c8n;
     const int athreads = c8n * apl;
     const int nb = (HW + apl * GN_AU - 1) / (apl * GN_AU);
     CTX_BOOL_GO(x32, X, hipLaunchKernelGGL(k_gn_apply<X>, dim3(nb, B), dim3(athreads), 0, stream, x, x2, Ca, part, (const f16 *)gamma, (const f16 *)beta, HW, C,
-                                           groups, NS, apl, eps, silu, (f16 *)y));
+                                           groups, NS, apl, eps, silu, (f16 *)y, ps));
 }
 
 extern "C" int64_t ctx_groupnorm_ws_bytes(int32_t B, int32_t groups)
@@ -321,15 +341,17 @@
 }
 
 int ctx_groupnorm_any(const void *x, int x32, const void *gamma, const void *beta, int B, int HW, int C, int groups, float eps, int silu,
-                      void *y, void *stats_ws, hipStream_t stream, const void *x2, int Ca)
-{
+                      void *y, void *stats_ws, hipStream_t stream, const void *x2, int Ca, const PairShare *pair)
+{
+    const PairShare ps = pair ? *pair : PairShare();
     CTX_REQUIRE(x && gamma && beta && y && stats_ws, "groupnorm: null pointer");
+    CTX_REQUIRE(!(ps.mism && ps.dup) || (!x32 && !x2), "groupnorm: the odd sample's copy of the input needs one fp16 source");
     CTX_REQUIRE(!x2 || (Ca > 0 && Ca < C && Ca % 8 == 0), "groupnorm: two sources need 0 < Ca < C in whole 8-channel columns (Ca=%d C=%d)", Ca, C);
     CTX_REQUIRE(gn_shape_ok(B, HW, C, groups), "groupnorm: unsupported B=%d HW=%d C=%d groups=%d", B, HW, C, groups);
     if (const int plf = gn_one_kernel_lanes(HW, C, groups); plf && (!x2 || Ca % (C / groups) == 0)) {
         const int thr = (C / groups / 8 * plf + 63) / 64 * 64;
         CTX_BOOL_GO(x32, X, hipLaunchKernelGGL(k_gn_fused<X>, dim3(groups, B), dim3(thr), 0, stream, x, x2, Ca, (const f16 *)gamma, (const f16 *)beta, HW, C,
-                                               groups, plf, eps, silu, (f16 *)y, GnSlabs{}));
+                                               groups, plf, eps, silu, (f16 *)y, GnSlabs{}, ps));
         CTX_CHECK_LAUNCH("groupnorm");
         return CTX_OK;
     }
@@ -355,8 +377,8 @@
         (void)hipFuncSetAttribute((const void *)k_gn_stats<true>, hipFuncAttributeMaxDynamicSharedMemorySize, 80 * 1024);
         attr = true;
     }
-    CTX_BOOL_GO(x32, X, hipLaunchKernelGGL(k_gn_stats<X>, dim3(NS, B), dim3(threads), lds, stream, x, x2, Ca, HW, C, groups, NS, PL, part));
-    gn_launch_apply(x, x32, x2, Ca, part, NS, gamma, beta, B, HW, C, groups, eps, silu, y, stream);
+    CTX_BOOL_GO(x32, X, hipLaunchKernelGGL(k_gn_stats<X>, dim3(NS, B), dim3(threads), lds, stream, x, x2, Ca, HW, C, groups, NS, PL, part, ps));
+    gn_launch_apply(x, x32, x2, Ca, part, NS, gamma, beta, B, HW, C, groups, eps, silu, y, stream, ps);
     CTX_CHECK_LAUNCH("groupnorm");
     return CTX_OK;
 }
@@ -364,11 +386,11 @@
 int ctx_groupnorm_two_pass(int HW, int C, int groups) { return gn_one_kernel_lanes(HW, C, groups) == 0; }
 
 int ctx_groupnorm_apply(const void *x, const float *part, int NS, const void *gamma, const void *beta, int B, int HW, int C, int groups, float eps,
-                        int silu, void *y, hipStream_t stream)
+                        int silu, void *y, hipStream_t stream, const PairShare *pair)
 {
     CTX_REQUIRE(x && part && gamma && beta && y, "groupnorm apply: null pointer");
     CTX_REQUIRE(gn_shape_ok(B, HW, C, groups) && NS >= 1 && NS <= GN_MAX_SPLITS, "groupnorm apply: unsupported B=%d HW=%d C=%d groups=%d NS=%d", B, HW, C, groups, NS);
-    gn_launch_apply(x, 0, nullptr, 0, part, NS, gamma, beta, B, HW, C, groups, eps, silu, y, stream);
+    gn_launch_apply(x, 0, nullptr, 0, part, NS, gamma, beta, B, HW, C, groups, eps, silu, y, stream, pair ? *pair : PairShare());
     CTX_CHECK_LAUNCH("groupnorm apply");
     return CTX_OK;
 }
@@ -381,7 +403,7 @@
     CTX_REQUIRE(plf > 0 && (!sl.rowbias || sl.ldrb % 8 == 0), "groupnorm slabs: B=%d HW=%d C=%d groups=%d does not take the one-kernel form", B, HW, C, groups);
     const int thr = (C / groups / 8 * plf + 63) / 64 * 64;
     hipLaunchKernelGGL((k_gn_fused<false, true>), dim3(groups, B), dim3(thr), 0, stream, (const void *)nullptr, (const void *)nullptr, 0, (const f16 *)gamma,
-                       (const f16 *)beta, HW, C, groups, plf, eps, silu, (f16 *)y, sl);
+                       (const f16 *)beta, HW, C, groups, plf, eps, silu, (f16 *)y, sl, PairShare());
     CTX_CHECK_LAUNCH("groupnorm slabs");
     return CTX_OK;
 }
@@ -518,8 +540,9 @@
 template <int KC, int R, bool X32>
 __global__ __launch_bounds__(256) void k_layernorm(const void *__restrict__ x, const f16 *__restrict__ gamma,
                                                    const f16 *__restrict__ beta, int64_t rows, int C, float eps,
-                                                   f16 *__restrict__ y)
-{
+                                                   f16 *__restrict__ y, PairShare ps)
+{
+    if (pair_rows_dead(ps.mism, ps.epoch, ps.rows, blockIdx.x * (4 * R), min((int64_t)(blockIdx.x + 1) * (4 * R), rows) - 1)) return;
     const int lane = threadIdx.x & 63;
     const int c8n = C / 8;
     const int64_t wave = ((int64_t)blockIdx.x * 256 + threadIdx.x) >> 6;
@@ -562,6 +585,11 @@
         }
         float rstd = rsqrtf(wave_sum_dpp(q) / (float)C + eps);
         f16 *yr = y + (row0 + rr) * C;
+        f16 *twin = nullptr;
+        if (!X32 && ps.dup && ps.mism) {
+            const unsigned sb = (unsigned)(row0 + rr) / (unsigned)ps.rows;
+            if (!(sb & 1) && pair_shared(ps.mism, ps.epoch, (int)sb)) twin = (f16 *)const_cast<void *>(x) + (row0 + rr + ps.rows) * C;
+        }
 #pragma unroll
         for (int k = 0; k < KC; ++k) {
             int c8 = lane + 64 * k;
@@ -570,6 +598,7 @@
 #pragma unroll
                 for (int j = 0; j < 8; ++j) o[j] = ln_norm(v[rr][k].get(j), mean, rstd, ga[k][j], be[k][j]);
                 *(f16x8 *)(yr + c8 * 8) = o;
+                if (twin) pair_copy(v[rr][k], twin + c8 * 8);
             }
         }
     }
@@ -577,8 +606,9 @@
 
 template <int KC>
 __global__ __launch_bounds__(256) void k_layernorm_g8(const f16 *__restrict__ x, const f16 *__restrict__ gamma, const f16 *__restrict__ beta,
-                                                      int64_t rows, float eps, f16 *__restrict__ y)
-{
+                                                      int64_t rows, float eps, f16 *__restrict__ y, PairShare ps)
+{
+    if (pair_rows_dead(ps.mism, ps.epoch, ps.rows, blockIdx.x * 32, min((int64_t)(blockIdx.x + 1) * 32, rows) - 1)) return;
     constexpr int C = 64 * KC;
     const int lane = threadIdx.x & 63, s = lane & 7, rw = lane >> 3;
     const int64_t wave = ((int64_t)blockIdx.x * 256 + threadIdx.x) >> 6;
@@ -608,12 +638,18 @@
     const float rstd = rsqrtf(sum8_dpp(q) / (float)C + eps);
     if (!live) return;
     f16 *yr = y + row * C + s * 8;
+    f16 *twin = nullptr;
+    if (ps.dup && ps.mism) {
+        const unsigned sb = (unsigned)row / (unsigned)ps.rows;
+        if (!(sb & 1) && pair_shared(ps.mism, ps.epoch, (int)sb)) twin = const_cast<f16 *>(x) + (row + ps.rows) * C + s * 8;
+    }
 #pragma unroll
     for (int k = 0; k < KC; ++k) {
         f16x8 o;
 #pragma unroll
         for (int j = 0; j < 8; ++j) o[j] = ln_norm(v[k].get(j), mean, rstd, ga[k][j], be[k][j]);
         *(f16x8 *)(yr + k * 64) = o;
+        if (twin) pair_copy(v[k], twin + k * 64);
     }
 }
 
@@ -623,14 +659,18 @@
     return ctx_layernorm_any(x, 0, gamma, beta, rows, C, eps, y, (hipStream_t)stream);
 }
 
-int ctx_layernorm_any(const void *x, int x32, const void *gamma, const void *beta, int64_t rows, int C, float eps, void *y, hipStream_t stream)
+int ctx_layernorm_any(const void *x, int x32, const void *gamma, const void *beta, int64_t rows, int C, float eps, void *y, hipStream_t stream,
+                      const PairShare *pair)
 {
     CTX_REQUIRE(x && gamma && beta && y && rows > 0 && C % 8 == 0 && C <= 2048, "layernorm: unsupported rows=%lld C=%d", (long long)rows, C);
+    CTX_REQUIRE(!pair || !pair->mism || (pair->rows > 0 && rows < (1ll << 31)), "layernorm: pair sharing needs rows per sample and rows < 2^31");
+    const PairShare ps = pair ? *pair : PairShare();
+    CTX_REQUIRE(!(ps.mism && ps.dup) || !x32, "layernorm: the odd sample's copy of the input needs an fp16 input");
     {
         static const int g8 = ctx_env_int("CTX_LN_G8", 1);
         if (g8 && !x32 && C % 64 == 0 && C <= 640 && rows >= 64) {
             const unsigned nb = (unsigned)cdiv64(cdiv64(rows, 8), 4);
-#define LN_G8(KC_) case KC_: hipLaunchKernelGGL(k_layernorm_g8<KC_>, dim3(nb), dim3(256), 0, stream, (const f16 *)x, (const f16 *)gamma, (const f16 *)beta, rows, eps, (f16 *)y); break
+#define LN_G8(KC_) case KC_: hipLaunchKernelGGL(k_layernorm_g8<KC_>, dim3(nb), dim3(256), 0, stream, (const f16 *)x, (const f16 *)gamma, (const f16 *)beta, rows, eps, (f16 *)y, ps); break
             switch (C / 64) {
                 LN_G8(1); LN_G8(2); LN_G8(3); LN_G8(4); LN_G8(5); LN_G8(6); LN_G8(7); LN_G8(8); LN_G8(9); LN_G8(10);
             }
@@ -641,7 +681,7 @@
     }
     const int kc = (C / 8 + 63) / 64;
 #define LN_GO(KC_, R_) CTX_BOOL_GO(x32, X, hipLaunchKernelGGL((k_layernorm<KC_, R_, X>), dim3((unsigned)cdiv64(cdiv64(rows, R_), 4)), dim3(256), 0, stream, x, \
-                                                          (const f16 *)gamma, (const f16 *)beta, rows, C, eps, (f16 *)y))
+                                                          (const f16 *)gamma, (const f16 *)beta, rows, C, eps, (f16 *)y, ps))
     const bool many = rows >= 8192;
     if (kc == 1) { if (many) LN_GO(1, 4); else LN_GO(1, 1); }
     else if (kc == 2) { if (many) LN_GO(2, 2); else LN_GO(2, 1); }
diff --git a/contexture-nerf_amd/csrc/unet.hip b/contexture-nerf_amd/csrc/unet.hip
--- a/contexture-nerf_amd/csrc/unet.hip
+++ b/contexture-nerf_amd/csrc/unet.hip
@@ -1,5 +1,6 @@
 #include "engine.h"
 #include <string.h>
+#include <atomic>
 
 struct ResP {
     int cin, cout;
@@ -47,6 +48,8 @@
     const f16 *add_res = nullptr;
     float add_scale = 1.0f;
     bool res32 = false;
+    int share_mode = 1;
+    int share_ops = 0;
     void *allocS(size_t n) { return alloc(n * (res32 ? 4 : 2)); }
     struct Tap { size_t off; int rows, C; };
     f16 *tap_buf = nullptr;
@@ -62,6 +65,8 @@
         tap_cursor += n;
     }
 };
+
+static int pair_share_env(void);
 
 static void add_resnet(ctx_unet *u, const std::string &p, int cin, int cout, ResP &r)
 {
@@ -125,6 +130,7 @@
         }
     ctx_unet *u = new ctx_unet();
     u->tag = "unet";
+    u->share_mode = pair_share_env();
     u->cfg = *cfg;
     const int n = cfg->n_levels, lpb = cfg->layers_per_block;
     const int *ch = cfg->block_out_channels;
@@ -397,17 +403,20 @@
     u->note(2, 0, 2);
     const Engine::GnTag t = u->gn_tag;
     u->gn_tag = Engine::GnTag();
+    const PairShare *ps = u->pair.mism ? &u->pair : nullptr;
+    if (ps && u->live()) ++u->pair_ops;
     if (t.x && t.x == x && !x2 && !(u->res32 && x_s) && t.B == B && t.HW == HW && t.C == C && t.groups == u->cfg.groups) {
         ++u->gn_from_producer;
-        RUN(ctx_groupnorm_apply(x, (const float *)stats, t.NS, u->W + g, u->W + b, B, HW, C, u->cfg.groups, eps, silu, y, u->s));
+        RUN(ctx_groupnorm_apply(x, (const float *)stats, t.NS, u->W + g, u->W + b, B, HW, C, u->cfg.groups, eps, silu, y, u->s, ps));
         return;
     }
-    RUN(ctx_groupnorm_any(x, (u->res32 && x_s) ? 1 : 0, u->W + g, u->W + b, B, HW, C, u->cfg.groups, eps, silu, y, stats, u->s, x2, Ca));
+    RUN(ctx_groupnorm_any(x, (u->res32 && x_s) ? 1 : 0, u->W + g, u->W + b, B, HW, C, u->cfg.groups, eps, silu, y, stats, u->s, x2, Ca, ps));
 }
 static void op_ln(ctx_unet *u, const void *x, size_t g, size_t b, int64_t rows, int C, f16 *y)
 {
     u->note(2, 0);
-    RUN(ctx_layernorm_any(x, u->res32 ? 1 : 0, u->W + g, u->W + b, rows, C, 1e-5f, y, u->s));
+    if (u->pair.mism && u->live()) ++u->pair_ops;
+    RUN(ctx_layernorm_any(x, u->res32 ? 1 : 0, u->W + g, u->W + b, rows, C, 1e-5f, y, u->s, u->pair.mism ? &u->pair : nullptr));
 }
 static const f16 *op_as16(ctx_unet *u, const void *x, size_t n)
 {
@@ -420,7 +429,8 @@
 static void op_attn(ctx_unet *u, const f16 *Q, const f16 *K, const f16 *V, int B, int Sq, int Skv, int heads, int qs, int kvs, f16 *O)
 {
     u->note(1, 4.0 * B * heads * (double)Sq * Skv * 64);
-    RUN(ctx_attention_core(Q, K, V, B, Sq, Skv, heads, qs, kvs, 0.125f, O, heads * 64, u->s));
+    if (u->pair.mism && u->live()) ++u->pair_ops;
+    RUN(ctx_attention_core(Q, K, V, B, Sq, Skv, heads, qs, kvs, 0.125f, O, heads * 64, u->s, u->pair.mism ? &u->pair : nullptr));
 }
 
 struct FwdCtx {
@@ -509,11 +519,15 @@
     const int B = f.B, S = H * W, M = B * S, C = t.C, cd = u->cfg.cross_attention_dim;
     size_t mark = u->top;
     f16 *g = u->allocH((size_t)M * C);
+    u->pair.dup = u->pair.mism != nullptr;
     op_gn(u, x, t.ng, t.nb, B, S, C, 1e-6f, 0, g, f.gn_stats);
+    u->pair.dup = 0;
     void *h0 = u->allocS((size_t)M * C);
     op_gemm(u, g, t.piw, t.pib, true, nullptr, M, C, C, h0, 0, false, true);
     f16 *l = g;
+    u->pair.dup = u->pair.mism != nullptr;
     op_ln(u, h0, t.l1g, t.l1b, M, C, l);
+    u->pair.dup = 0;
     f16 *a = nullptr;
     if (u->ref_mode == 2) {
         if (u->ref_k >= (int)u->ref_slots.size() || u->ref_slots[u->ref_k].C != C ||
@@ -549,6 +563,7 @@
         a = u->allocH((size_t)M * C);
         op_attn(u, qkv, qkv + C, qkv + 2 * C, B, S, S, t.heads, 3 * C, 3 * C, a);
     }
+    u->pair = PairShare();
     void *h1 = u->allocS((size_t)M * C);
     op_gemm(u, a, t.o1w, t.o1b, true, h0, M, C, C, h1, 0, true, true);
     op_ln(u, h1, t.l2g, t.l2b, M, C, l);
@@ -581,8 +596,19 @@
     if (u->ref_mode == 1) u->ref_slots.clear();
     FwdCtx f; f.B = B; f.L = L;
     f.gn_stats = u->alloc((size_t)ctx_groupnorm_ws_bytes(B, c.groups));
+    int *mism = (int *)u->alloc((size_t)((B + 1) / 2) * sizeof(int));
+    const bool share = u->share_mode != 0 && B >= 2 && !u->res32 && !u->is_controlnet && !u->add_res && u->ref_mode == 0 && u->down[0].has_attn &&
+                       (int64_t)B * H * W < (1ll << 31);
+    PairShare shared;
+    if (!u->dry) u->share_ops = 0;
     f16 *te0 = u->allocH((size_t)B * ch[0]);
-    u->note(2, 0); RUN(ctx_time_embed_core(timestep, B, ch[0], te0, u->s));
+    u->note(2, 0);
+    if (share) {
+        static std::atomic<int> epochs{0};
+        const int epoch = (epochs.fetch_add(1) & 0x3fffffff) + 1;
+        RUN(ctx_time_embed_pairs_core(timestep, B, ch[0], te0, sample, (int64_t)c.in_channels * H * W, mism, epoch, u->share_mode == 2, u->s));
+        if (u->live()) { shared.mism = mism; shared.epoch = epoch; shared.rows = H * W; }
+    } else RUN(ctx_time_embed_core(timestep, B, ch[0], te0, u->s));
     f16 *te1 = u->allocH((size_t)B * u->temb_dim);
     u->note(2, 2.0 * B * ch[0] * u->temb_dim); RUN(ctx_gemv_core(te0, u->W + u->t1w, u->W + u->t1b, B, u->temb_dim, ch[0], 0, 1, te1, u->s));
     f16 *te2 = u->allocH((size_t)B * u->temb_dim);
@@ -606,7 +632,10 @@
     {
         size_t m0 = u->top;
         f16 *x16 = u->res32 ? u->allocH((size_t)B * h * w * ch[0]) : (f16 *)x;
-        u->note(2, 2.0 * B * h * w * ch[0] * c.in_channels * 9); RUN(ctx_conv_in_core(sample, u->W + u->ciw, u->W + u->cib, B, c.in_channels, h, w, ch[0], x16, u->s));
+        u->pair = shared; u->pair.dup = shared.mism != nullptr;
+        if (u->pair.mism && u->live()) ++u->pair_ops;
+        u->note(2, 2.0 * B * h * w * ch[0] * c.in_channels * 9); RUN(ctx_conv_in_core(sample, u->W + u->ciw, u->W + u->cib, B, c.in_channels, h, w, ch[0], x16, u->s, u->pair.mism ? &u->pair : nullptr));
+        u->pair.dup = 0;
         if (u->res32) { u->note(2, 0); RUN(ctx_f16_to_f32_core(x16, (int64_t)B * h * w * ch[0], (float *)x, u->s)); u->top = m0; }
     }
 
@@ -744,6 +773,7 @@
     op_gn(u, x, u->cng, u->cnb, B, h * w, cur, c.norm_eps, 1, y, f.gn_stats);
     u->note(2, 2.0 * B * h * w * cur * c.out_channels * 9);
     RUN(ctx_conv_out_core(y, u->W + u->cow, u->W + u->cob, B, h, w, cur, c.out_channels, out, u->s));
+    if (!u->dry) u->share_ops = u->pair_ops;
     return engine_finish(u, "unet_forward");
 }
 
@@ -881,6 +911,19 @@
     return CTX_OK;
 }
 
+static int pair_share_env(void)
+{
+    static const int m = ctx_env_int("CTX_CFG_SHARE", 1);
+    return m >= 0 && m <= 2 ? m : 1;
+}
+extern "C" int32_t ctx_unet_set_pair_share(ctx_unet_t *u, int32_t mode)
+{
+    CTX_REQUIRE(u && mode >= 0 && mode <= 2, "unet_set_pair_share: mode %d (0 off, 1 automatic, 2 forced)", mode);
+    u->share_mode = mode;
+    return CTX_OK;
+}
+extern "C" int32_t ctx_unet_pair_share_ops(const ctx_unet_t *u) { return u ? u->share_ops : -1; }
+
 extern "C" int32_t ctx_unet_gn_epilogue_counts(const ctx_unet_t *u, int64_t *from_producer, int64_t *from_slabs)
 {
     CTX_REQUIRE(u && from_producer && from_slabs, "unet_gn_epilogue_counts: bad args");
diff --git a/contexture-nerf_amd/unet.py b/contexture-nerf_amd/unet.py
--- a/contexture-nerf_amd/unet.py
+++ b/contexture-nerf_amd/unet.py
@@ -44,8 +44,11 @@
     def _init_state(self, src=None):
         self.in_channels = self.config['in_channels']
         self._res32 = False
+        self._pair_share = None
         if src is not None and src._res32:
             self.set_residual_fp32(True)
+        if src is not None and src._pair_share is not None:
+            self.set_pair_share(src._pair_share)
 
     def load_state_dict(self, sd, strict=True):
         missing = [n for n in self._names if n not in sd]
@@ -103,6 +106,14 @@
         self._res32 = bool(on)
         self._ws_key = None
         return self
+
+    def set_pair_share(self, mode=1):
+        L.check(self._lib.ctx_unet_set_pair_share(self._h, int(mode)))
+        self._pair_share = int(mode)
+        return self
+
+    def pair_share_ops(self):
+        return int(self._lib.ctx_unet_pair_share_ops(self._h))
 
     def forward_ref(self, sample, timestep, encoder_hidden_states, mode, bank=None, ref_row0=0):
         m = {'w': 1, 'r': 2}.get(mode)
diff --git a/include/ctx_nerf.h b/include/ctx_nerf.h
--- a/include/ctx_nerf.h
+++ b/include/ctx_nerf.h
@@ -253,6 +253,8 @@
 int32_t ctx_unet_set_residual_fp32(ctx_unet_t *u, int32_t on);
 int32_t ctx_unet_stats(const ctx_unet_t *u, int32_t klass, int64_t *launches, double *flops);
 int32_t ctx_unet_gn_epilogue_counts(const ctx_unet_t *u, int64_t *from_producer, int64_t *from_slabs);
+int32_t ctx_unet_set_pair_share(ctx_unet_t *u, int32_t mode);
+int32_t ctx_unet_pair_share_ops(const ctx_unet_t *u);
 int32_t ctx_unet_set_taps(ctx_unet_t *u, void *buf, int64_t capacity);
 int32_t ctx_unet_tap_count(const ctx_unet_t *u);
 int32_t ctx_unet_tap_info(const ctx_unet_t *u, int32_t i, int64_t *offset, int32_t *rows, int32_t *channels);
@@ -322,6 +324,8 @@
 int32_t ctx_gemv_f16(const void *x, const void *w, const void *bias, int32_t Bm, int32_t N, int32_t K, int32_t silu_in, int32_t silu_out,
                      void *out, ctx_stream_t stream);
 int32_t ctx_time_embed_f16(const float *t, int32_t B, int32_t dim, void *out, ctx_stream_t stream);
+int32_t ctx_time_embed_pairs_f16(const float *t, int32_t B, int32_t dim, void *out, const float *sample, int64_t per, void *mism,
+                                 int32_t epoch, int32_t forced, ctx_stream_t stream);
 int32_t ctx_transpose_v_f16(const void *v, int32_t B, int32_t S, int32_t ld, int32_t heads, int32_t Sp, void *vt, ctx_stream_t stream);
 int32_t ctx_concat_f16(const void *a, const void *b, int64_t M, int32_t Ca, int32_t Cb, void *y, ctx_stream_t stream);
 int32_t ctx_concat_f32(const float *a, const float *b, int64_t M, int32_t Ca, int32_t Cb, float *y, ctx_stream_t stream);
```

Result: no change. 121.5 steps/s, median of 6 (+0.6%).
